# lmcinnes/enstop

Hardware: AMD Instinct MI355X
Metric: EM iterations/sec (higher is better)
Workload: dtype f32; 1 GPU; 1M x 100k, 100M nnz; corpus=independent Zipf tokens (SURVEY 8d), nnz=100435863, k=64, schedule=fused, parallelism=single fit

## Files before the change

enstop_amd/_lib.py:

```python
import ctypes as C
import os

import numpy as np

_HERE = os.path.dirname(os.path.abspath(__file__))
LIB_PATH = os.environ.get("ENSTOP_AMD_LIB", os.path.join(_HERE, "libplsa_hip.so"))

PLSA_FUSED = 1
PLSA_TRACE_LL = 4
PLSA_SW_LL_ONLY = 8
PLSA_STOP_NO_ZERO_ARM = 16
PLSA_SHARDED = 64
PLSA_GRAPH = 128
PLSA_REFERENCE_SUMS = 256
PLSA_REFERENCE_LL = 512

_i32p = np.ctypeslib.ndpointer(np.int32, flags="C_CONTIGUOUS")
_i64p = np.ctypeslib.ndpointer(np.int64, flags="C_CONTIGUOUS")
_f32p = np.ctypeslib.ndpointer(np.float32, flags="C_CONTIGUOUS")
_f64p = np.ctypeslib.ndpointer(np.float64, flags="C_CONTIGUOUS")
_ctx = C.c_void_p
_i64 = C.c_int64
_i32 = C.c_int32
_vp = C.c_void_p

SIGNATURES = {
    "plsa_device_count": (C.c_int, [C.POINTER(C.c_int)]),
    "plsa_hw_queues": (C.c_int, []),
    "plsa_create": (C.c_int, [C.c_int, C.POINTER(_ctx)]),
    "plsa_destroy": (None, [_ctx]),
    "plsa_last_error": (C.c_char_p, [_ctx]),
    "plsa_synchronize": (C.c_int, [_ctx]),
    "plsa_device_info": (C.c_int, [_ctx, C.c_char_p, C.c_char_p, C.POINTER(C.c_int), C.POINTER(_i64)]),
    "plsa_upload_csr": (C.c_int, [_ctx, _i32p, _i32p, _f32p, _i64, _i64, _i64]),
    "plsa_bootstrap": (C.c_int, [_ctx, _vp, _i64]),
    "plsa_active_shape": (C.c_int, [_ctx, C.POINTER(_i64), C.POINTER(_i64), C.POINTER(_i64)]),
    "plsa_download_active_csr": (C.c_int, [_ctx, _i32p, _i32p, _f32p]),
    "plsa_set_factors": (C.c_int, [_ctx, _vp, _vp, _i64, _i64, _i32]),
    "plsa_get_factors": (C.c_int, [_ctx, _vp, _vp]),
    "plsa_init_factors_device": (C.c_int, [_ctx, _i32, C.c_uint64]),
    "plsa_init_factors_mt19937": (C.c_int, [_ctx, _i32, np.ctypeslib.ndpointer(np.uint32, flags="C_CONTIGUOUS")]),
    "plsa_mt_marginals": (C.c_int, [_ctx, np.ctypeslib.ndpointer(np.float64, flags="C_CONTIGUOUS"), _i32]),
    "plsa_refit_init_mt19937": (C.c_int, [_ctx, C.c_void_p, _i64, _i32,
                                          np.ctypeslib.ndpointer(np.uint32, flags="C_CONTIGUOUS")]),
    "plsa_copy_components_to_device": (C.c_int, [_ctx, _vp]),
    "plsa_set_arithmetic": (C.c_int, [_ctx, _i32]),
    "plsa_e_step": (C.c_int, [_ctx, C.c_float, _vp]),
    "plsa_set_p": (C.c_int, [_ctx, _f32p]),
    "plsa_m_step": (C.c_int, [_ctx, _vp, _i32, _vp, _vp]),
    "plsa_log_likelihood": (C.c_int, [_ctx, _vp, C.POINTER(C.c_double)]),
    "plsa_fit": (C.c_int, [_ctx, _vp, _i32, _i32, C.c_double, C.c_float, _i32, C.POINTER(_i32), _vp,
                           C.POINTER(_i32)]),
    "plsa_refit": (C.c_int, [_ctx, _vp, _i32, _i32, C.c_double, C.c_float, _i32, C.POINTER(_i32), _vp,
                             C.POINTER(_i32)]),
    "plsa_em_accumulate": (C.c_int, [_ctx, _vp, C.c_float, _vp]),
    "plsa_em_accumulate_materialised": (C.c_int, [_ctx, _vp, C.c_float, _vp]),
    "plsa_p_reserve": (C.c_int, [_ctx, C.c_int64, C.POINTER(C.c_void_p)]),
    "plsa_p_borrow": (C.c_int, [_ctx, C.c_void_p, C.c_int64]),
    "plsa_em_finish": (C.c_int, [_ctx]),
    "plsa_set_sample_weight": (C.c_int, [_ctx, _vp]),
    "plsa_comm_last_error": (C.c_int, [_ctx, C.c_char_p, _i64]),
    "plsa_accumulator_device": (C.c_int, [_ctx, C.POINTER(C.c_void_p), C.POINTER(_i64)]),
    "plsa_accumulator_get": (C.c_int, [_ctx, _f32p]),
    "plsa_accumulator_set": (C.c_int, [_ctx, _f32p]),
    "plsa_comm_unique_id": (C.c_int, [C.c_void_p]),
    "plsa_comm_init": (C.c_int, [_ctx, C.c_char_p, _i32, _i32]),
    "plsa_comm_destroy": (C.c_int, [_ctx]),
    "plsa_comm_info": (C.c_int, [_ctx, C.POINTER(_i32), C.POINTER(_i32)]),
    "plsa_comm_barrier": (C.c_int, [_ctx]),
    "plsa_stack_reserve": (C.c_int, [_ctx, C.c_int64, C.c_int64, C.c_int32, C.POINTER(C.c_void_p)]),
    "plsa_comm_allgather_stack": (C.c_int, [_ctx, C.c_int64, C.c_int64, C.c_int32, C.POINTER(C.POINTER(C.c_float))]),
    "plsa_comm_allgather_stack_to": (C.c_int, [_ctx, _i64, _i64, _i32, _f32p]),
    "plsa_comm_allgather_host": (C.c_int, [_ctx, _vp, _i64, _vp]),
    "plsa_comm_allreduce_f64": (C.c_int, [_ctx, _f64p, _i64, _i32]),
    "plsa_comm_broadcast_host": (C.c_int, [_ctx, _vp, _i64, _i32]),
    "plsa_allreduce_accumulator": (C.c_int, [_ctx]),
    "plsa_reference_chain_info": (C.c_int, [_ctx, C.POINTER(_i64), C.POINTER(_i64), C.POINTER(_i32)]),
    "plsa_placement_info": (C.c_int, [_ctx, C.POINTER(_i32), C.POINTER(C.c_double), C.POINTER(C.c_double)]),
    "plsa_schedule_info": (C.c_int, [_ctx, C.POINTER(_i32), C.POINTER(C.c_double), C.POINTER(_i32), C.POINTER(_i32),
                                     C.POINTER(C.c_int64)]),
    "plsa_packed_info": (C.c_int, [_ctx, C.POINTER(_i32), C.POINTER(_i32)]),
    "plsa_pass_info": (C.c_int, [_ctx, _i32p, _i32p, _i32p]),
    "plsa_fit_info": (C.c_int, [_ctx, _i32p]),
    "plsa_release_scratch": (C.c_int, [_ctx]),
    "plsa_timing_enable": (C.c_int, [_ctx, _i32]),
    "plsa_timing_reset": (C.c_int, [_ctx]),
    "plsa_timing_get": (C.c_int, [_ctx, C.c_char_p, C.POINTER(C.c_double), C.POINTER(_i64)]),
    "plsa_timing_report": (C.c_int, [_ctx, C.c_char_p, _i64]),
    "plsa_measure_stream_bandwidth": (C.c_int, [_ctx, _i64, _i32, _i32, C.POINTER(C.c_double)]),
    "plsa_all_pairs_hellinger": (C.c_int, [_ctx, C.c_void_p, _i64, _i64, _f64p]),
    "plsa_all_pairs_kl": (C.c_int, [_ctx, C.c_void_p, _i64, _i64, _f64p]),
    "plsa_cluster_representatives": (C.c_int, [_ctx, C.c_void_p, _i64, _i64, _i32p, _vp, _i32, _f32p]),
    "plsa_host_normalize_rows": (None, [_f64p, _i64, _i64]),
    "plsa_host_mt19937_jump": (C.c_int, [C.POINTER(C.c_uint32), _i32]),
    "plsa_generate_synthetic": (C.c_int, [_ctx, _i64, _i64, _i64, C.c_double, C.c_uint64,
                                          C.POINTER(_i64)]),
    "plsa_generate_synthetic_topics": (C.c_int, [_ctx, _i64, _i64, _i64, C.c_double, C.c_uint64, _i32, C.c_double,
                                                 C.c_double, C.POINTER(_i64)]),
    "plsa_synthetic_dominant_topics": (C.c_int, [_ctx, _i32p]),
}

_members = C.c_void_p
MEMBERS_MAX = 64
MEMBER_SIGNATURES = {
    "plsa_members_create": (C.c_int, [_ctx, _i32, C.POINTER(_members)]),
    "plsa_members_destroy": (None, [_members]),
    "plsa_members_capacity": (C.c_int, [_ctx, _i32, C.POINTER(_i32)]),
    "plsa_members_prepare": (C.c_int, [_members, _i32, _vp, _i64, _i32, _vp, _vp, _vp]),
    "plsa_members_fit": (C.c_int, [_members, _i32, _i32, _i32, C.c_double, C.c_float, _i32, _i32p, _vp, _i32, _i32p,
                                   C.POINTER(_i32)]),
    "plsa_members_copy_components": (C.c_int, [_members, _i32, C.c_void_p]),
    "plsa_members_context": (C.c_int, [_members, _i32, C.POINTER(_ctx)]),
    "plsa_members_info": (C.c_int, [_members, _i32, _i32p]),
    "plsa_members_last_ll": (C.c_int, [_members, _i32, C.POINTER(C.c_double)]),
    "plsa_members_release": (C.c_int, [_members]),
}

METRIC_SIGNATURES = {
    "plsa_codocument_counts": (C.c_int, [_ctx, _i32p, _i64, _i32, _i32, _i64p, _i64p]),
}

_lib = None
HW_QUEUES = {"set_by": None, "hip_mapped_before_load": None}


def _default_hw_queues():
    want = os.environ.get("ENSTOP_AMD_HW_QUEUES", "8").strip()
    if "GPU_MAX_HW_QUEUES" in os.environ:
        HW_QUEUES["set_by"] = "user"
        return
    try:
        n_queues = int(want)
    except ValueError:
        raise ValueError("ENSTOP_AMD_HW_QUEUES=%r: expected a positive integer (hardware queues to ask the HIP runtime for) "
                         "or 0 to leave the runtime's default" % (want,)) from None
    if n_queues <= 0:
        HW_QUEUES["set_by"] = "opt-out"
        return
    try:
        with open("/proc/self/maps") as f:
            HW_QUEUES["hip_mapped_before_load"] = "libamdhip64" in f.read()
    except OSError:
        pass
    os.environ["GPU_MAX_HW_QUEUES"] = str(n_queues)
    HW_QUEUES["set_by"] = "enstop_amd"


def hw_queues():
    return dict(HW_QUEUES, value=int(load().plsa_hw_queues()))


def load():
    global _lib
    if _lib is not None:
        return _lib
    if not os.path.exists(LIB_PATH):
        raise ImportError(
            "enstop_amd: %s not found -- build the HIP extension first "
            "(python -m enstop_amd.build). There is no CPU fallback." % LIB_PATH)
    _default_hw_queues()
    lib = C.CDLL(LIB_PATH, mode=C.RTLD_GLOBAL)
    for name, (res, args) in list(SIGNATURES.items()) + list(MEMBER_SIGNATURES.items()) + list(METRIC_SIGNATURES.items()):
        fn = getattr(lib, name)
        fn.restype = res
        fn.argtypes = args
    _lib = lib
    return lib


def ptr(a):
    return None if a is None else a.ctypes.data
```

enstop_amd/csrc/plsa_hip.hip:

```cpp
#include <hip/hip_runtime.h>
#include <hipcub/hipcub.hpp>
#include <rccl/rccl.h>

#include <algorithm>
#include <cmath>
#include <cstdarg>
#include <cstdio>
#include <cstdlib>
#include <cstring>
#include <memory>
#include <mutex>
#include <string>
#include <thread>
#include <type_traits>
#include <vector>

#include "../../include/plsa_hip.h"
#include "../../include/plsa_hip_diag.h"
#include "../../include/plsa_hip_members.h"
#include "../../include/plsa_hip_metrics.h"
#include "mt_jump.hpp"
#include "plsa_kernels.hpp"
#include "plsa_member_kernels.hpp"
#include "plsa_metric_kernels.hpp"
#include "plsa_ref_kernels.hpp"
#include "plsa_synth.hpp"

using plsa::i64;

namespace {

thread_local std::string g_err;


struct DevBuf {
    void *p = nullptr;
    size_t cap = 0;
    bool borrowed = false;
    DevBuf() = default;
    DevBuf(DevBuf &&o) noexcept { swap(o); }
    DevBuf &operator=(DevBuf &&o) noexcept { DevBuf(std::move(o)).swap(*this); return *this; }
    void swap(DevBuf &o) noexcept { std::swap(p, o.p); std::swap(cap, o.cap); std::swap(borrowed, o.borrowed); }
    ~DevBuf() { if (p && !borrowed) (void)hipFree(p); }
    void release() { if (!borrowed) *this = DevBuf(); }
    void borrow(void *q, size_t bytes) { *this = DevBuf(); p = q; cap = q ? bytes : 0; borrowed = q != nullptr; }
    template <class T> T *as() const { return reinterpret_cast<T *>(p); }
};

template <class H, hipError_t (*Destroy)(H)>
struct Handle {
    H h = nullptr;
    Handle() = default;
    Handle(Handle &&o) noexcept { std::swap(h, o.h); }
    Handle &operator=(Handle &&o) noexcept { Handle(std::move(o)).swap(*this); return *this; }
    void swap(Handle &o) noexcept { std::swap(h, o.h); }
    ~Handle() { if (h) (void)Destroy(h); }
    operator H() const { return h; }
};
using Stream = Handle<hipStream_t, hipStreamDestroy>;
using Event = Handle<hipEvent_t, hipEventDestroy>;

struct HostFree { void operator()(void *p) const { (void)hipHostFree(p); } };
template <class T> using Pinned = std::unique_ptr<T[], HostFree>;
template <class T> hipError_t host_alloc(Pinned<T> &h, size_t count) {
    h.reset();
    void *q = nullptr;
    const hipError_t e = hipHostMalloc(&q, sizeof(T) * count, hipHostMallocDefault);
    h.reset(static_cast<T *>(q));
    return e;
}

template <class T> struct Derived {
    bool valid = false;
    void invalidate() { valid = false; }
    void drop() { static_cast<T &>(*this) = T{}; }
};

struct Timed {
    int name_id;
    Event a, b;
};

}

struct plsa_ctx {
    int device = 0;
    Stream stream;
    Stream stream2;
    hipStream_t ls = nullptr;
    Event ev_fork, ev_join;
    Event ev_row, ev_tail;
    bool overlap = true;
    double overlap_full_limit = 2e9;
    std::string err;
    hipDeviceProp_t prop;
    int grid_cap = 2048;

    i64 bn = 0, bm = 0, bnnz = 0;
    DevBuf b_indptr, b_col, b_val;
    bool active_is_base = true;
    i64 n = 0, m = 0, nnz = 0;
    DevBuf a_indptr, a_col, a_val;
    const int *indptr = nullptr, *col = nullptr;
    const float *val = nullptr;
    struct RowIndex : Derived<RowIndex> { DevBuf ids; } rowidx;

    struct Csc : Derived<Csc> {
        DevBuf colptr, row, val, pos, item_first, item_col, item_start, item_end, item_order, heavy_cols;
        DevBuf item_rec;
        DevBuf xcd_lo;
        bool balanced = false;
        int seg = 256, n_heavy = 0;
        i64 n_items = 0;
    } csc;
    int seg_override = 0, struct_lpn = 0;
    int struct_row_lpn = 0;
    DevBuf partial;
    bool use_item_order = true, xcd_split = true;
    bool packed = true;
    struct PackedStream : Derived<PackedStream> { DevBuf buf; bool ok = false; } pk_csr, pk_csc;
    DevBuf pk_count;
    int chunks_per_lane = 2;
    int row_lpn = 1, row_ch = 1;
    bool row_shape_8x2 = true;
    bool p_lent = false;
    int e_rows = -1;
    int mt_streams = 256;
    i64 mt_min_blocks = 4096;
    int heavy_items = 32;

    bool force_wide = false;
    struct RowItems : Derived<RowItems> {
        DevBuf first, row, start;
        bool use = false;
        int seg = 64;
        i64 n = 0;
    } ritems;
    int rseg_override = 0, ritems_mode = -1;
    DevBuf rpartial;

    struct EItems : Derived<EItems> { DevBuf row, start; int seg = 0; i64 n = 0; } eitems;
    int eseg_override = -1;

    bool sort_rows = true;
    struct RowOrder : Derived<RowOrder> {
        DevBuf ids;
        int range = 0;
    } roworder;
    i64 syn_n = 0; int syn_k0 = 0; double syn_alpha = 0.0; uint64_t syn_seed = 0;
    bool row_xcd = false;

    int k = 0, kp = 0, lpn = 1, ch = 1;
    DevBuf U[3], Vt[3], Vacc;
    bool rot3 = false;
    int speculate = -1;
    Event ev_ll;
    int cu = 0, cv = 0;
    i64 fac_n = 0, fac_m = 0;
    DevBuf P;
    struct PState : Derived<PState> {} p_state;
    bool ref_sums = false, ref_ll = false;
    DevBuf ref_terms;
    int ref_chain_mode = 0;
    bool ref_pairs_off = false;
    DevBuf ref_csum, ref_pairs, ref_exps, ref_pairs2, ref_exps2, ref_stats, ref_ll_neg;
    struct RefTileSums : Derived<RefTileSums> {
        DevBuf sums;
        const float *sw = nullptr;
        int tj = 0;
    } ref_tsum;
    const float *ref_e_sw = nullptr;
    bool ref_e_no_sums = false;
    struct RefHeavy : Derived<RefHeavy> { DevBuf cols; int n = 0, min = 0; } ref_heavy;
    Pinned<unsigned long long> h_ref_stats;
    Event ev_ref_stats;
    bool ref_stats_pending = false;
    unsigned long long ref_slow_total = 0, ref_chunks_total = 0;
    int placement_candidates = 4, placement_tried = 0;
    double placement_gbps[2] = {0.0, 0.0};
    size_t p_shift = 0;

    DevBuf sw, ll_partials, ll_out, colsum_partials, norm_pwz, norm_pdz, tmp0, tmp1, tmp2, cubtmp;
    DevBuf mt_seq;
    bool mt_chain = false;
    DevBuf mt_words, mt_state, mt_fin, mt_poly;
    Pinned<double> h_ll;

    DevBuf colsum_rows, colsum_rows2;
    DevBuf metric_mask, metric_small;
    DevBuf t_end;
    bool pipeline = true;
    bool graph = false;
    int order_band = -1;
    int balance = -1;
    bool bal_have_frac = false;
    double bal_frac[9] = {0, 0, 0, 0, 0, 0, 0, 0, 0};
    int bal_lo[9] = {0, 0, 0, 0, 0, 0, 0, 0, 0};
    i64 bal_chunks = -1;
    int bal_launches = 0;
    double bal_end_us[8] = {0, 0, 0, 0, 0, 0, 0, 0};
    int small_grid = 0;
    int colsum_rows_used = 0;
    struct FitInfo {
        int fused = 0, pipelined = 0, speculated = 0, graph_launches = 0;
        int tail = 0;
        int two_stage = 0;
        int xcd_split = 0;
    } fit_info;

    ncclComm_t comm = nullptr;
    int comm_rank = 0, comm_world = 1;
    bool sharded = false;
    bool sw_resident = false;
    i64 sw_n = 0;
    DevBuf sw_res;
    DevBuf comm_send, comm_recv, comm_small, comm_stack;
    Pinned<float> comm_host;
    size_t comm_host_cap = 0;

    bool timing = false;
    std::vector<std::string> names;
    std::vector<Timed> timed;
    std::vector<Event> pool;
    std::vector<double> acc_ms;
    std::vector<i64> acc_n;
};

namespace {

inline float *p_base(plsa_ctx *c) { return reinterpret_cast<float *>(reinterpret_cast<char *>(c->P.p) + c->p_shift); }

int fail(plsa_ctx *c, const char *fmt, ...) {
    char buf[512];
    va_list ap;
    va_start(ap, fmt);
    vsnprintf(buf, sizeof buf, fmt, ap);
    va_end(ap);
    if (c) c->err = buf; else g_err = buf;
    return 1;
}

#define HIPCHK(c, expr)                                                                            \
    do {                                                                                           \
        hipError_t e_ = (expr);                                                                    \
        if (e_ != hipSuccess)                                                                      \
            return fail((c), "%s failed: %s (%s:%d)", #expr, hipGetErrorString(e_), __FILE__,      \
                        __LINE__);                                                                 \
    } while (0)

#define CHK(expr)                                                                                  \
    do {                                                                                           \
        int r_ = (expr);                                                                           \
        if (r_) return r_;                                                                         \
    } while (0)

#define NCCLCHK(c, expr)                                                                           \
    do {                                                                                           \
        ncclResult_t n_ = (expr);                                                                  \
        if (n_ != ncclSuccess)                                                                     \
            return fail((c), "%s failed: %s (%s:%d)", #expr, ncclGetErrorString(n_), __FILE__,     \
                        __LINE__);                                                                 \
    } while (0)

int grid_for(plsa_ctx *c, i64 work_items, int items_per_block);
bool g_contig = false;

int ensure(plsa_ctx *c, DevBuf &b, size_t bytes) {
// ... 248 lines not shown
    if (c->row_lpn == 8 && c->row_ch == 2 && c->kp == 64) {
        if (wide) fn(plsa::Shape<8, 2, false, true>{}); else fn(plsa::Shape<8, 2, true>{});
        return 0;
    }
    return dispatch_shape_gather(c, wide, fn);
}

int launch_check(plsa_ctx *c, const char *what) {
    hipError_t e = hipGetLastError();
    if (e != hipSuccess) return fail(c, "launch of %s failed: %s", what, hipGetErrorString(e));
    return 0;
}

inline int out_u(const plsa_ctx *c) { return c->rot3 ? (c->cu + 1) % 3 : 1 - c->cu; }
inline int out_v(const plsa_ctx *c) { return c->rot3 ? (c->cv + 1) % 3 : 1 - c->cv; }

int grid_for(plsa_ctx *c, i64 work_items, int items_per_block) {
    i64 need = (work_items + items_per_block - 1) / items_per_block;
    if (need < 1) need = 1;
    return (int)std::min<i64>(need, c->grid_cap);
}

void set_active_pointers(plsa_ctx *c) {
    if (c->active_is_base) {
        c->indptr = c->b_indptr.as<int>(); c->col = c->b_col.as<int>(); c->val = c->b_val.as<float>();
        c->n = c->bn; c->m = c->bm; c->nnz = c->bnnz;
    } else {
        c->indptr = c->a_indptr.as<int>(); c->col = c->a_col.as<int>(); c->val = c->a_val.as<float>();
    }
    c->rowidx.invalidate(); c->csc.invalidate(); c->pk_csr.invalidate(); c->pk_csc.invalidate(); c->roworder.invalidate();
    c->ritems.invalidate(); c->eitems.invalidate(); c->p_state.invalidate(); c->ref_heavy.invalidate(); c->ref_tsum.invalidate();
    c->ref_pairs_off = false;
}

int ensure_rowidx(plsa_ctx *c) {
    if (c->rowidx.valid) return 0;
    CHK(ensure(c, c->rowidx.ids, sizeof(int) * (size_t)c->nnz));
    if (c->n > 0) {
        Scope s(c, "k_expand_rows");
        hipLaunchKernelGGL(plsa::k_expand_rows, dim3(grid_for(c, c->n, 4)), dim3(256), 0, c->stream,
                           c->indptr, (int)c->n, c->rowidx.ids.as<int>());
    }
    CHK(launch_check(c, "k_expand_rows"));
    c->rowidx.valid = true;
    return 0;
}

int row_xcd_range(const plsa_ctx *c) {
    const i64 gpb = 256 / std::max(1, c->row_lpn);
    if (!c->row_xcd || c->n < 64 * gpb) return 0;
    return (int)(((c->n + gpb - 1) / gpb + 7) / 8 * gpb);
}

int ensure_roworder(plsa_ctx *c, const int **out) {
    *out = nullptr;
    if (!c->sort_rows) return 0;
    const int range = row_xcd_range(c);
    if (!c->roworder.valid || c->roworder.range != range) {
        c->roworder.range = range;
        const i64 n = c->n;
        CHK(ensure(c, c->roworder.ids, sizeof(int) * (size_t)n));
        CHK(ensure(c, c->tmp0, sizeof(int) * (size_t)n * 2));
        CHK(ensure(c, c->tmp1, sizeof(int) * (size_t)n));
        int *len = c->tmp0.as<int>(), *len_sorted = c->tmp0.as<int>() + n, *ids = c->tmp1.as<int>();
        hipLaunchKernelGGL(plsa::k_row_lengths, dim3((unsigned)((n + 255) / 256)), dim3(256), 0, c->stream,
                           c->indptr, (int)n, len, ids, range);
        CHK(launch_check(c, "k_row_lengths"));
        size_t bytes = 0;
        HIPCHK(c, hipcub::DeviceRadixSort::SortPairsDescending(nullptr, bytes, len, len_sorted, ids,
                                                               c->roworder.ids.as<int>(), (int)n, 0, 32, c->stream));
        CHK(ensure(c, c->cubtmp, bytes));
        HIPCHK(c, hipcub::DeviceRadixSort::SortPairsDescending(c->cubtmp.p, bytes, len, len_sorted, ids,
                                                               c->roworder.ids.as<int>(), (int)n, 0, 32, c->stream));
        c->roworder.valid = true;
    }
    *out = c->roworder.ids.as<int>();
    return 0;
}

int exclusive_sum_int(plsa_ctx *c, const int *in, int *out, i64 count);

int ensure_ritems(plsa_ctx *c) {
    if (c->ritems.valid) return 0;
    const i64 n = c->n;
    const i64 group_slots = (i64)c->prop.multiProcessorCount * 32 * (64 / std::max(1, c->row_lpn));
    const double avg = (double)c->nnz / (double)std::max<i64>(n, 1);
    const int rseg_decide = c->rseg_override ? c->rseg_override : 64;
    c->ritems.use = c->ritems_mode == 1 || (c->ritems_mode < 0 && n < 2 * group_slots && avg > 2.0 * rseg_decide);
    if (c->rseg_override) c->ritems.seg = c->rseg_override;
    else {
        const i64 per_slot = c->nnz / std::max<i64>(group_slots, 1);
        int r = 16;
        while (r * 2 <= per_slot && r < 64) r *= 2;
        c->ritems.seg = r;
    }
    c->ritems.n = 0;
    if (c->ritems.use) {
        CHK(ensure(c, c->ritems.first, sizeof(int) * (size_t)(n + 1)));
        CHK(ensure(c, c->tmp0, sizeof(int) * (size_t)(n + 1)));
        HIPCHK(c, hipMemsetAsync(c->tmp0.p, 0, sizeof(int) * (size_t)(n + 1), c->stream));
        hipLaunchKernelGGL(plsa::k_item_counts, dim3((unsigned)((n + 255) / 256)), dim3(256), 0, c->stream,
                           c->indptr, (int)n, c->ritems.seg, c->tmp0.as<int>());
        CHK(exclusive_sum_int(c, c->tmp0.as<int>(), c->ritems.first.as<int>(), n + 1));
        int cnt = 0;
        HIPCHK(c, hipMemcpyAsync(&cnt, c->ritems.first.as<int>() + n, sizeof(int), hipMemcpyDeviceToHost, c->stream));
        HIPCHK(c, hipStreamSynchronize(c->stream));
        c->ritems.n = cnt;
        CHK(ensure(c, c->ritems.row, sizeof(int) * (size_t)std::max(cnt, 1)));
        CHK(ensure(c, c->ritems.start, sizeof(int) * (size_t)std::max(cnt, 1)));
        hipLaunchKernelGGL(plsa::k_ritem_fill, dim3((unsigned)((n + 255) / 256)), dim3(256), 0, c->stream,
                           c->indptr, c->ritems.first.as<int>(), (int)n, c->ritems.seg, c->ritems.row.as<int>(),
                           c->ritems.start.as<int>());
        CHK(launch_check(c, "k_ritem_fill"));
    }
    c->ritems.valid = true;
    return 0;
}

int ensure_eitems(plsa_ctx *c, int eseg) {
    if (c->eitems.valid && c->eitems.seg == eseg) return 0;
    const i64 n = c->n;
    c->eitems.seg = eseg;
    c->eitems.n = 0;
    if (eseg > 0) {
        CHK(ensure(c, c->tmp0, sizeof(int) * (size_t)(n + 1)));
        CHK(ensure(c, c->tmp1, sizeof(int) * (size_t)(n + 1)));
        HIPCHK(c, hipMemsetAsync(c->tmp0.p, 0, sizeof(int) * (size_t)(n + 1), c->stream));
        hipLaunchKernelGGL(plsa::k_item_counts, dim3((unsigned)((n + 255) / 256)), dim3(256), 0, c->stream,
                           c->indptr, (int)n, eseg, c->tmp0.as<int>());
        CHK(exclusive_sum_int(c, c->tmp0.as<int>(), c->tmp1.as<int>(), n + 1));
        int cnt = 0;
        HIPCHK(c, hipMemcpyAsync(&cnt, c->tmp1.as<int>() + n, sizeof(int), hipMemcpyDeviceToHost, c->stream));
        HIPCHK(c, hipStreamSynchronize(c->stream));
        c->eitems.n = cnt;
        CHK(ensure(c, c->eitems.row, sizeof(int) * (size_t)std::max(cnt, 1)));
        CHK(ensure(c, c->eitems.start, sizeof(int) * (size_t)std::max(cnt, 1)));
        hipLaunchKernelGGL(plsa::k_ritem_fill, dim3((unsigned)((n + 255) / 256)), dim3(256), 0, c->stream,
                           c->indptr, c->tmp1.as<int>(), (int)n, eseg, c->eitems.row.as<int>(), c->eitems.start.as<int>());
        CHK(launch_check(c, "k_ritem_fill"));
        HIPCHK(c, hipStreamSynchronize(c->stream));
    }
    c->eitems.valid = true;
    return 0;
}

int exclusive_sum_int(plsa_ctx *c, const int *in, int *out, i64 count) {
    size_t bytes = 0;
    HIPCHK(c, hipcub::DeviceScan::ExclusiveSum(nullptr, bytes, in, out, (int)count, c->stream));
    CHK(ensure(c, c->cubtmp, bytes));
    HIPCHK(c, hipcub::DeviceScan::ExclusiveSum(c->cubtmp.p, bytes, in, out, (int)count, c->stream));
    return 0;
}

int ensure_csc(plsa_ctx *c) {
    if (c->csc.valid) return 0;
    CHK(ensure_rowidx(c));
    {
        const i64 slots = (i64)c->prop.multiProcessorCount * 32 * (64 / std::max(1, c->lpn));
        i64 want = c->nnz / std::max<i64>(slots + slots / 4, 1);
        int seg = 16;
        const int cap = 64;
        while (seg * 2 <= want && seg < cap) seg *= 2;
        c->csc.seg = c->seg_override ? c->seg_override : seg;
    }
    const i64 nnz = c->nnz, m = c->m;
    CHK(ensure(c, c->csc.colptr, sizeof(int) * (size_t)(m + 1)));
    CHK(ensure(c, c->csc.row, sizeof(int) * (size_t)nnz));
    CHK(ensure(c, c->csc.val, sizeof(float) * (size_t)nnz));
    CHK(ensure(c, c->csc.pos, sizeof(int) * (size_t)nnz));
    CHK(ensure(c, c->tmp0, sizeof(int) * (size_t)std::max<i64>(nnz, m + 1)));
    CHK(ensure(c, c->tmp1, sizeof(int) * (size_t)nnz));
    const bool pack = c->packed && nnz > 0 && c->n <= plsa::PACK_MAX_IDS;
    c->pk_csc.invalidate();
    c->pk_csc.ok = false;
    if (pack) {
        CHK(ensure(c, c->pk_csc.buf, sizeof(unsigned) * (size_t)nnz));
        CHK(ensure(c, c->pk_count, sizeof(unsigned long long)));
        HIPCHK(c, hipMemsetAsync(c->pk_count.p, 0, sizeof(unsigned long long), c->stream));
    }
    if (nnz > 0) {
        hipLaunchKernelGGL(plsa::k_iota, dim3(grid_for(c, nnz, 256)), dim3(256), 0, c->stream,
                           c->tmp1.as<int>(), nnz);
        int bits = 1;
        while (((i64)1 << bits) < m) ++bits;
        size_t bytes = 0;
        HIPCHK(c, hipcub::DeviceRadixSort::SortPairs(nullptr, bytes, c->col, c->tmp0.as<int>(),
                                                     c->tmp1.as<int>(), c->csc.pos.as<int>(), nnz, 0,
                                                     bits, c->stream));
        CHK(ensure(c, c->cubtmp, bytes));
        HIPCHK(c, hipcub::DeviceRadixSort::SortPairs(c->cubtmp.p, bytes, c->col, c->tmp0.as<int>(),
                                                     c->tmp1.as<int>(), c->csc.pos.as<int>(), nnz, 0,
                                                     bits, c->stream));
        hipLaunchKernelGGL(plsa::k_colptr_from_sorted, dim3((unsigned)((m + 256) / 256)), dim3(256), 0, c->stream,
                           c->tmp0.as<int>(), nnz, (int)m, c->csc.colptr.as<int>());
        hipLaunchKernelGGL(plsa::k_csc_gather, dim3(grid_for(c, nnz, 256)), dim3(256), 0, c->stream,
                           c->csc.pos.as<int>(), c->rowidx.ids.as<int>(), c->val, nnz,
                           c->csc.row.as<int>(), c->csc.val.as<float>(), pack ? c->pk_csc.buf.as<unsigned>() : nullptr,
                           pack ? c->pk_count.as<unsigned long long>() : nullptr);
        CHK(launch_check(c, "k_csc_gather"));
    } else {
        HIPCHK(c, hipMemsetAsync(c->csc.colptr.p, 0, sizeof(int) * (size_t)(m + 1), c->stream));
    }
    CHK(ensure(c, c->csc.item_first, sizeof(int) * (size_t)(m + 1)));
    HIPCHK(c, hipMemsetAsync(c->tmp0.p, 0, sizeof(int) * (size_t)(m + 1), c->stream));
    hipLaunchKernelGGL(plsa::k_col_item_counts, dim3((unsigned)((m + 255) / 256)), dim3(256), 0, c->stream,
                       c->csc.colptr.as<int>(), (int)m, c->csc.seg, c->tmp0.as<int>());
    CHK(exclusive_sum_int(c, c->tmp0.as<int>(), c->csc.item_first.as<int>(), m + 1));
    int n_items = 0;
    HIPCHK(c, hipMemcpyAsync(&n_items, c->csc.item_first.as<int>() + m, sizeof(int), hipMemcpyDeviceToHost,
                             c->stream));
    HIPCHK(c, hipStreamSynchronize(c->stream));
    c->csc.n_items = n_items;
    const size_t ni = (size_t)std::max<i64>(n_items, 1);
    CHK(ensure(c, c->csc.item_col, sizeof(int) * ni));
    CHK(ensure(c, c->csc.item_start, sizeof(int) * ni));
    CHK(ensure(c, c->csc.item_end, sizeof(int) * ni));
    CHK(ensure(c, c->csc.item_order, sizeof(int) * ni));
    CHK(ensure(c, c->tmp2, sizeof(unsigned long long) * ni * 2));
    CHK(ensure(c, c->tmp1, sizeof(int) * ni));
    unsigned long long *d_key = c->tmp2.as<unsigned long long>();
    const int band_bytes = (c->kp >= 64 ? 2048 : 512) << 10;
    const int band = c->order_band >= 0 ? c->order_band : std::max(64, band_bytes / (c->kp > 0 ? c->kp * 4 : 256));
    int len_bits = 1;
    while (((i64)1 << len_bits) <= c->n) ++len_bits;
    int key_bits = len_bits;
    if (band > 0) { i64 n_bands = c->n / band + 1; int bb = 1; while (((i64)1 << bb) < n_bands) ++bb; key_bits = len_bits + bb; }
    if (n_items > 0)
        hipLaunchKernelGGL(plsa::k_item_fill, dim3((unsigned)((n_items + 255) / 256)), dim3(256), 0, c->stream,
                           c->csc.colptr.as<int>(), c->csc.item_first.as<int>(), (int)m, c->csc.seg, c->csc.row.as<int>(),
                           c->csc.item_col.as<int>(), c->csc.item_start.as<int>(), c->csc.item_end.as<int>(), band, len_bits, d_key,
                           c->tmp1.as<int>(), n_items);
    CHK(launch_check(c, "k_item_fill"));
    if (n_items > 0) {
        size_t bytes = 0;
        HIPCHK(c, hipcub::DeviceRadixSort::SortPairs(nullptr, bytes, d_key, d_key + ni,
                                                     c->tmp1.as<int>(), c->csc.item_order.as<int>(), n_items, 0, key_bits, c->stream));
        CHK(ensure(c, c->cubtmp, bytes));
        HIPCHK(c, hipcub::DeviceRadixSort::SortPairs(c->cubtmp.p, bytes, d_key, d_key + ni,
                                                     c->tmp1.as<int>(), c->csc.item_order.as<int>(), n_items, 0, key_bits, c->stream));
    }
    CHK(ensure(c, c->csc.item_rec, sizeof(int4) * ni));
    if (n_items > 0) {
        hipLaunchKernelGGL(plsa::k_item_records, dim3((unsigned)((n_items + 255) / 256)), dim3(256), 0, c->stream,
                           c->use_item_order ? c->csc.item_order.as<int>() : nullptr, c->csc.item_col.as<int>(),
                           c->csc.item_start.as<int>(), c->csc.item_end.as<int>(), (i64)n_items, c->csc.item_rec.as<int4>());
        CHK(launch_check(c, "k_item_records"));
    }
    c->csc.balanced = false;
    CHK(ensure(c, c->csc.heavy_cols, sizeof(int) * (size_t)(m + 1)));
    HIPCHK(c, hipMemsetAsync(c->csc.heavy_cols.as<int>() + m, 0, sizeof(int), c->stream));
    hipLaunchKernelGGL(plsa::k_heavy_list, dim3((unsigned)((m + 255) / 256)), dim3(256), 0, c->stream,
                       c->csc.item_first.as<int>(), (int)m, c->heavy_items, c->csc.heavy_cols.as<int>(),
                       c->csc.heavy_cols.as<int>() + m);
    CHK(launch_check(c, "k_heavy_list"));
    HIPCHK(c, hipMemcpyAsync(&c->csc.n_heavy, c->csc.heavy_cols.as<int>() + m, sizeof(int), hipMemcpyDeviceToHost, c->stream));
    unsigned long long escaped = 0;
    if (pack) HIPCHK(c, hipMemcpyAsync(&escaped, c->pk_count.p, sizeof escaped, hipMemcpyDeviceToHost, c->stream));
    HIPCHK(c, hipStreamSynchronize(c->stream));
    c->csc.valid = true;
    c->pk_csc.valid = c->packed;
    c->pk_csc.ok = pack && escaped * 16 <= (unsigned long long)nnz;
    if (!c->pk_csc.ok) c->pk_csc.buf.release();
    return 0;
}

int build_packed(plsa_ctx *c, DevBuf &out, const int *ids, const float *vals, i64 id_range, bool *ok) {
    *ok = false;
    const i64 nnz = c->nnz;
    if (nnz <= 0 || id_range > plsa::PACK_MAX_IDS) { out.release(); return 0; }
    CHK(ensure(c, out, sizeof(unsigned) * (size_t)nnz));
    CHK(ensure(c, c->pk_count, sizeof(unsigned long long)));
    HIPCHK(c, hipMemsetAsync(c->pk_count.p, 0, sizeof(unsigned long long), c->stream));
    hipLaunchKernelGGL(plsa::k_pack_entries, dim3(grid_for(c, nnz, 256)), dim3(256), 0, c->stream,
                       ids, vals, nnz, out.as<unsigned>(), c->pk_count.as<unsigned long long>());
    CHK(launch_check(c, "k_pack_entries"));
    unsigned long long escaped = 0;
    HIPCHK(c, hipMemcpyAsync(&escaped, c->pk_count.p, sizeof escaped, hipMemcpyDeviceToHost, c->stream));
    HIPCHK(c, hipStreamSynchronize(c->stream));
    *ok = escaped * 16 <= (unsigned long long)nnz;
    if (!*ok) out.release();
    return 0;
}

int ensure_packed_csr(plsa_ctx *c) {
    if (!c->packed || c->pk_csr.valid) return 0;
    CHK(build_packed(c, c->pk_csr.buf, c->col, c->val, c->m, &c->pk_csr.ok));
    c->pk_csr.valid = true;
    return 0;
}

int ensure_packed_csc(plsa_ctx *c) {
    CHK(ensure_csc(c));
    if (!c->packed || c->pk_csc.valid) return 0;
    CHK(build_packed(c, c->pk_csc.buf, c->csc.row.as<int>(), c->csc.val.as<float>(), c->n, &c->pk_csc.ok));
    c->pk_csc.valid = true;
    return 0;
}

int upload_sw(plsa_ctx *c, const float *sw, const float **d_sw) {
    *d_sw = nullptr;
    if (!sw) {
        if (c->sw_resident) {
            if (c->sw_n != c->n) return fail(c, "resident sample weights were set for %lld documents, the active matrix has %lld",
                                              (long long)c->sw_n, (long long)c->n);
            *d_sw = c->sw_res.as<float>();
        }
        return 0;
    }
    CHK(ensure(c, c->sw, sizeof(float) * (size_t)c->n));
    HIPCHK(c, hipMemcpyAsync(c->sw.p, sw, sizeof(float) * (size_t)c->n, hipMemcpyHostToDevice, c->stream));
    HIPCHK(c, hipStreamSynchronize(c->stream));
    *d_sw = c->sw.as<float>();
    return 0;
}

void set_shape(plsa_ctx *c, int k) {
    const int kp = (k + 3) / 4 * 4;
    c->k = k; c->kp = kp;
    const int prev_lpn = c->struct_lpn, prev_row_lpn = c->struct_row_lpn;
    int lpn = 1;
    while (lpn < kp / 4 && lpn < 64) lpn *= 2;
    if (lpn >= 32 && lpn * 4 >= kp && c->chunks_per_lane == 2) lpn /= 2;
    c->lpn = lpn;
    c->ch = (kp / 4 + lpn - 1) / lpn;
    if (c->ch == 3) c->ch = 4;
    c->row_lpn = c->lpn; c->row_ch = c->ch;
    if (c->row_shape_8x2 && c->lpn == 16 && c->ch == 1 && kp == 64) { c->row_lpn = 8; c->row_ch = 2; }
    if (c->row_lpn != prev_row_lpn) {
        c->ritems.invalidate();
        c->struct_row_lpn = c->row_lpn;
    }
    if (lpn != prev_lpn) {
        c->eitems.invalidate();
        if (!c->seg_override) c->csc.invalidate();
        c->struct_lpn = lpn;
    }
}

int need_factors(plsa_ctx *c) {
    if (c->k <= 0 || !c->U[0].p || !c->Vt[0].p) return fail(c, "factors not set (call plsa_set_factors)");
    if (c->n <= 0) return fail(c, "no corpus uploaded");
    if (c->fac_n != c->n || c->fac_m != c->m)
        return fail(c, "factors were set for a %lld x %lld matrix but the active matrix is %lld x %lld "
                       "(call plsa_set_factors after plsa_upload_csr / plsa_bootstrap)",
                    (long long)c->fac_n, (long long)c->fac_m, (long long)c->n, (long long)c->m);
    return 0;
}

int run_ref_e_step(plsa_ctx *c, float thresh);
int run_ref_norm_pwz(plsa_ctx *c, const float *d_sw);
int ensure_ref_heavy(plsa_ctx *c);
bool ref_pairs_now(const plsa_ctx *c);
int run_ref_m_step(plsa_ctx *c, const float *d_sw, bool update_v, float *d_norm_pdz);
int run_ref_loglik(plsa_ctx *c, const float *d_sw, double *out);

int run_e_step(plsa_ctx *c, float thresh) {
    c->ref_tsum.invalidate();
    {
        const size_t need = sizeof(float) * (size_t)(c->nnz + 64) * (size_t)c->kp;
        size_t free_b = 0, total_b = 0;
        if (!c->P.borrowed && c->P.cap < need && hipMemGetInfo(&free_b, &total_b) == hipSuccess && free_b + c->P.cap < need)
            return fail(c, c->ref_sums ? "the reference arithmetic (PLSA_REFERENCE_SUMS) stores P(z|w,d) like the reference does: %.1f GB needed, "
                                         "%.1f GB of HBM free -- at this size only the default arithmetic is available"
                                       : "materialising P(z|w,d) needs %.1f GB but only %.1f GB of HBM are free; use the fused "
                           "schedule (PLSA_FUSED), which never stores it, or tile the documents (plsa_em_accumulate_materialised)", need / 1e9, (free_b + c->P.cap) / 1e9);
    }
    if (c->P.borrowed || c->p_lent) {
        const size_t need = sizeof(float) * (size_t)(c->nnz + 64) * (size_t)c->kp;
        if (c->P.cap < need)
            return fail(c, c->P.borrowed ? "the borrowed P(z|w,d) buffer holds %.2f GB, this matrix needs %.2f GB (plsa_p_borrow)"
                                         : "the P(z|w,d) buffer lent out by plsa_p_reserve holds %.2f GB, this matrix needs %.2f GB: it cannot "
                                           "grow while other contexts hold its address (end the loans, then plsa_release_scratch)",
                        c->P.cap / 1e9, need / 1e9);
        c->p_shift = 0;
    } else
    {
        const char *s1 = getenv("PLSA_P_SLACK_MB"), *s2 = getenv("PLSA_P_OFFSET_KB");
        const size_t slack = s1 ? (size_t)atoll(s1) << 20 : 0;
        c->p_shift = s2 ? (size_t)atoll(s2) * 1024 : 0;
        CHK(ensure_best_placement(c, c->P, sizeof(float) * (size_t)(c->nnz + 64) * (size_t)c->kp + std::max(slack, c->p_shift),
                                  c->placement_candidates, c->placement_gbps, &c->placement_tried));
    }
    if (c->ref_sums) return run_ref_e_step(c, thresh);
    bool e_rows = c->e_rows < 0 ? (double)c->nnz * c->kp >= 1e8 : c->e_rows != 0;
    if (e_rows) {
        const int eseg = c->eseg_override >= 0 ? c->eseg_override : (c->lpn >= 16 ? 64 : (c->lpn == 8 ? 8 : 16));
        CHK(ensure_eitems(c, eseg));
        const bool items = eseg > 0 && c->eitems.n > 0;
        const int grid = grid_for(c, items ? c->eitems.n : c->n, 256 / c->lpn);
        const int *order = nullptr;
        if (!items) CHK(ensure_roworder(c, &order));
        CHK(dispatch_shape(c, [&](auto S) {
            Scope s(c, "k_e_step");
            auto go = [&](auto TN) {
                hipLaunchKernelGGL((plsa::k_e_step_rows<decltype(S), decltype(TN)::value>), dim3(grid), dim3(256), 0, c->stream,
                                   c->indptr, c->col, (int)c->n, order, c->U[c->cu].as<float>(), c->Vt[c->cv].as<float>(),
                                   p_base(c), c->kp, thresh, items ? c->eitems.row.as<int>() : nullptr,
                                   items ? c->eitems.start.as<int>() : nullptr, eseg, c->eitems.n);
            };
            if (thresh < plsa::TINY_THRESH) go(std::true_type{}); else go(std::false_type{});
        }));
    } else {
        CHK(ensure_rowidx(c));
        const i64 tiles = (c->nnz + 63) / 64;
        const int grid = grid_for(c, tiles, 4);
        CHK(dispatch_shape(c, [&](auto S) {
            Scope s(c, "k_e_step");
            auto go = [&](auto TN) {
                hipLaunchKernelGGL((plsa::k_e_step<decltype(S), decltype(TN)::value>), dim3(grid), dim3(256), 0, c->stream,
                                   c->rowidx.ids.as<int>(), c->col, c->nnz, c->U[c->cu].as<float>(),
                                   c->Vt[c->cv].as<float>(), p_base(c), c->kp, thresh);
            };
            if (thresh < plsa::TINY_THRESH) go(std::true_type{}); else go(std::false_type{});
        }));
    }
    CHK(launch_check(c, "k_e_step"));
    c->p_state.valid = true;
    return 0;
}

int run_row_pass(plsa_ctx *c, bool from_p, bool want_ll, const float *d_sw, float thresh,
                 float *d_norm_pdz, int *ll_blocks) {
    CHK(ensure_ritems(c));
    const bool items = c->ritems.use && c->ritems.n > 0;
    int grid = grid_for(c, items ? c->ritems.n : c->n, 256 / c->row_lpn);
    const int *order = nullptr;
    const int gpb_row = 256 / c->row_lpn;
    const bool xcd_rows = !items && !from_p && c->sort_rows && row_xcd_range(c) > 0;
    if (xcd_rows) grid = (int)(((c->n + gpb_row - 1) / gpb_row + 7) / 8 * 8);
    if (!items) CHK(ensure_roworder(c, &order));
    if (items) CHK(ensure(c, c->rpartial, sizeof(float) * (size_t)c->ritems.n * c->kp));
    const int *ri_row = items ? c->ritems.row.as<int>() : nullptr;
    const int *ri_start = items ? c->ritems.start.as<int>() : nullptr;
    float *rpart = items ? c->rpartial.as<float>() : nullptr;
    const int rseg = c->ritems.seg;
    const i64 n_ritems = c->ritems.n;
    if (want_ll) CHK(ensure(c, c->ll_partials, sizeof(double) * (size_t)grid));
    if (!from_p) CHK(ensure_packed_csr(c));
    const bool packed = !from_p && c->packed && c->pk_csr.ok;
    CHK(dispatch_shape_row(c, [&](auto S) {
        using Sh = decltype(S);
        const int *ip = c->indptr, *cl = packed ? c->pk_csr.buf.as<int>() : c->col;
        const float *vl = c->val, *U = c->U[c->cu].as<float>(), *Vt = c->Vt[c->cv].as<float>();
        const float *P = p_base(c);
        float *Un = c->U[out_u(c)].as<float>();
        double *llp = c->ll_partials.as<double>();
        const int n = (int)c->n, kp = c->kp;
        auto launch = [&](auto SS, auto FP, auto LL, auto TN, const char *name) {
            Scope s(c, name);
            hipLaunchKernelGGL((plsa::k_row_pass<decltype(SS), decltype(FP)::value, decltype(LL)::value, decltype(TN)::value>),
                               dim3(grid), dim3(256), 0, c->ls, ip, cl, vl, n, order, U, Vt, P, Un,
                               d_sw, d_norm_pdz, kp, thresh, llp, ri_row, ri_start, rseg, n_ritems, rpart, xcd_rows ? 1 : 0);
        };
        auto go = [&](auto FP, auto LL, auto TN, const char *name) {
            if constexpr (!decltype(FP)::value) {
                if (packed) { launch(plsa::Packed<Sh>{}, FP, LL, TN, name); return; }
            }
            launch(Sh{}, FP, LL, TN, name);
        };
        using T = std::true_type;
        using F = std::false_type;
        const bool tiny = thresh < plsa::TINY_THRESH;
        if (from_p) go(T{}, F{}, F{}, "k_row_pass<P>");
        else if (want_ll) { if (tiny) go(F{}, T{}, T{}, "k_row_pass<fused,LL>"); else go(F{}, T{}, F{}, "k_row_pass<fused,LL>"); }
        else { if (tiny) go(F{}, F{}, T{}, "k_row_pass<fused>"); else go(F{}, F{}, F{}, "k_row_pass<fused>"); }
        if (items) {
            Scope s(c, "k_row_reduce");
            hipLaunchKernelGGL((plsa::k_row_reduce<Sh>), dim3(grid_for(c, c->n, 256 / Sh::LPN)), dim3(256), 0, c->ls,
                               c->ritems.first.as<int>(), n, rpart, Un, d_norm_pdz, kp);
        }
    }));
    CHK(launch_check(c, "k_row_pass"));
    if (ll_blocks) *ll_blocks = grid;
    return 0;
}

void balance_set_lo(plsa_ctx *c, int n_chunks) {
    c->bal_lo[0] = 0;
    for (int x = 1; x < 8; ++x) {
        int v = (int)(c->bal_frac[x] * n_chunks + 0.5);
        c->bal_lo[x] = std::min(n_chunks, std::max(c->bal_lo[x - 1], v));
    }
    c->bal_lo[8] = n_chunks;
    c->bal_chunks = n_chunks;
}

int col_grid(plsa_ctx *c, int n_chunks, bool split) {
    i64 g = n_chunks;
    if (split) {
        int longest = 1;
        for (int x = 0; x < 8; ++x) longest = std::max(longest, c->bal_lo[x + 1] - c->bal_lo[x]);
        g = 8 * (i64)longest;
    }
    return (int)std::max<i64>(1, std::min<i64>(g, (i64)1 << 22));
}

template <class Launch>
int ensure_balance(plsa_ctx *c, int n_chunks, bool split, Launch &&launch) {
    if (c->csc.balanced && c->bal_chunks == n_chunks) return 0;
    CHK(ensure(c, c->csc.xcd_lo, sizeof(int) * 16));
    const bool warm = c->bal_have_frac;
    if (!warm) for (int x = 0; x <= 8; ++x) c->bal_frac[x] = x / 8.0;
    balance_set_lo(c, n_chunks);
    HIPCHK(c, hipMemcpyAsync(c->csc.xcd_lo.p, c->bal_lo, sizeof(int) * 9, hipMemcpyHostToDevice, c->ls));
    c->bal_launches = 0;
    const bool small_grid_active = c->small_grid > 0 && (double)c->nnz * c->kp < c->overlap_full_limit;
    const bool tune = split && n_chunks >= 64 && !small_grid_active &&
                      (c->balance > 0 || (c->balance < 0 && (double)c->nnz * c->kp >= 1e8));
    if (tune) {
        const size_t cap = (size_t)8 * (size_t)n_chunks + 16;
        CHK(ensure(c, c->t_end, sizeof(unsigned long long) * cap));
        std::vector<unsigned long long> te;
        const int max_launches = warm ? 1 : 8;
        if (!warm) CHK(launch(false));
        double best_spread = 1e300, best_frac[9];
        for (int x = 0; x <= 8; ++x) best_frac[x] = c->bal_frac[x];
        for (int it = 0; it < max_launches; ++it) {
            const int grid = col_grid(c, n_chunks, split);
            te.assign((size_t)grid + 1, 0);
            HIPCHK(c, hipMemsetAsync(c->t_end.p, 0, sizeof(unsigned long long) * ((size_t)grid + 1), c->ls));
            CHK(launch(true));
            HIPCHK(c, hipMemcpyAsync(te.data(), c->t_end.p, sizeof(unsigned long long) * ((size_t)grid + 1),
                                     hipMemcpyDeviceToHost, c->ls));
            HIPCHK(c, hipStreamSynchronize(c->ls));
            c->bal_launches++;
            unsigned long long t0 = ~0ull, last[8] = {0, 0, 0, 0, 0, 0, 0, 0};
            for (int b = 0; b <= grid; ++b) if (te[b]) t0 = std::min(t0, te[b]);
            for (int b = 0; b < grid; ++b) last[b & 7] = std::max(last[b & 7], te[b]);
            double T[8], mean = 0.0, lo_t = 1e300, hi_t = 0.0;
            for (int x = 0; x < 8; ++x) {
                T[x] = std::max(1.0, (double)(last[x] - t0) / 100.0);
                c->bal_end_us[x] = T[x];
                mean += T[x] / 8.0; lo_t = std::min(lo_t, T[x]); hi_t = std::max(hi_t, T[x]);
            }
            const double spread = (hi_t - lo_t) / mean;
            if (spread < best_spread) {
                best_spread = spread;
                for (int x = 0; x <= 8; ++x) best_frac[x] = c->bal_frac[x];
            }
            if (spread <= 0.02) break;
            if (it == max_launches - 1 && !warm) {
                for (int x = 0; x <= 8; ++x) c->bal_frac[x] = best_frac[x];
                balance_set_lo(c, n_chunks);
                HIPCHK(c, hipMemcpyAsync(c->csc.xcd_lo.p, c->bal_lo, sizeof(int) * 9, hipMemcpyHostToDevice, c->ls));
                break;
            }
            double size[8], tot = 0.0;
            for (int x = 0; x < 8; ++x) {
                size[x] = std::max(1e-6, (c->bal_frac[x + 1] - c->bal_frac[x]) * (1.0 + 0.8 * (mean / T[x] - 1.0)));
                tot += size[x];
            }
            double acc = 0.0;
            for (int x = 0; x < 8; ++x) { acc += size[x]; c->bal_frac[x + 1] = acc / tot; }
            c->bal_frac[8] = 1.0;
            balance_set_lo(c, n_chunks);
            HIPCHK(c, hipMemcpyAsync(c->csc.xcd_lo.p, c->bal_lo, sizeof(int) * 9, hipMemcpyHostToDevice, c->ls));
        }
        c->bal_have_frac = true;
    }
    c->csc.balanced = true;
    return 0;
}

int run_col_pass(plsa_ctx *c, bool from_p, const float *d_sw, float thresh, int parts = 3) {
    CHK(from_p ? ensure_csc(c) : ensure_packed_csc(c));
    const bool packed = !from_p && c->packed && c->pk_csc.ok;
    CHK(ensure(c, c->partial, sizeof(float) * (size_t)std::max<i64>(c->csc.n_items, 1) * c->kp));
    int rc = 0;
    CHK(dispatch_shape_gather(c, table_is_wide(c, c->n), [&](auto S) {
        using Sh = decltype(S);
        constexpr int LPN = Sh::LPN, GPB = 256 / LPN;
        const i64 n_visit = c->csc.n_items;
        const int n_chunks = (int)((n_visit + GPB - 1) / GPB);
        const int grid2 = grid_for(c, c->m, GPB);
        const bool u_fits_l2 = (double)c->n * c->kp * 4.0 <= 2.0 * 1024 * 1024;
        const int xcd_split = (c->xcd_split && n_chunks >= 64 && !u_fits_l2) ? 1 : 0;
        if (parts & 1) {
            c->fit_info.xcd_split = xcd_split;
            rc = ensure(c, c->colsum_rows, sizeof(double) * (size_t)std::max(n_chunks, 1) * c->kp);
            if (rc) return;
            const size_t smem = sizeof(double) * (size_t)GPB * c->kp;
            auto launch = [&](bool timed) -> int {
                int grid = col_grid(c, n_chunks, xcd_split != 0);
                if (c->small_grid > 0 && (double)c->nnz * c->kp < c->overlap_full_limit)
                    grid = std::min(grid, c->small_grid * c->prop.multiProcessorCount);
                Scope s(c, from_p ? "k_col_pass<P>" : "k_col_pass<fused>");
                const int4 *rec = c->csc.item_rec.as<int4>();
                const int *lo = c->csc.xcd_lo.as<int>(), *cp = c->csc.pos.as<int>();
                const int *cr = packed ? c->pk_csc.buf.as<int>() : c->csc.row.as<int>();
                const float *cvl = c->csc.val.as<float>(), *U = c->U[c->cu].as<float>(), *Vt = c->Vt[c->cv].as<float>();
                float *part = c->partial.as<float>();
                double *sums = c->colsum_rows.as<double>();
                unsigned long long *te = c->t_end.as<unsigned long long>();
                const int kp = c->kp;
                auto run = [&](auto SS, auto FP, auto TM, auto TN) {
                    hipLaunchKernelGGL((plsa::k_col_pass<decltype(SS), decltype(FP)::value, decltype(TM)::value, decltype(TN)::value>),
                                       dim3(grid), dim3(256), smem, c->ls, rec, n_visit, lo, cr, cvl, cp, U, Vt, p_base(c), d_sw,
                                       part, kp, thresh, xcd_split, sums, te);
                };
                auto go = [&](auto FP, auto TM, auto TN) {
                    if constexpr (!decltype(FP)::value) {
                        if (packed) { run(plsa::Packed<Sh>{}, FP, TM, TN); return; }
                    }
                    run(Sh{}, FP, TM, TN);
                };
                using T = std::true_type;
                using F = std::false_type;
                const bool tiny = !from_p && thresh < plsa::TINY_THRESH;
                if (from_p) { if (timed) go(T{}, T{}, F{}); else go(T{}, F{}, F{}); }
                else if (tiny) { if (timed) go(F{}, T{}, T{}); else go(F{}, F{}, T{}); }
                else { if (timed) go(F{}, T{}, F{}); else go(F{}, F{}, F{}); }
                return launch_check(c, "k_col_pass");
            };
            rc = ensure_balance(c, n_chunks, xcd_split != 0, launch);
            if (rc) return;
            rc = launch(false);
            if (rc) return;
            c->colsum_rows_used = n_chunks;
        }
        if (parts & 2) {
            Scope s(c, "k_col_reduce");
            hipLaunchKernelGGL((plsa::k_col_reduce<Sh>), dim3(grid2 + c->csc.n_heavy), dim3(256),
                               (256 / LPN) * c->kp * sizeof(float), c->ls,
                               c->csc.item_first.as<int>(), (int)c->m, c->heavy_items, c->csc.heavy_cols.as<int>(), c->csc.n_heavy,
                               c->partial.as<float>(), c->Vacc.as<float>(), c->kp);
        }
    }));
    if (rc) return rc;
    CHK(launch_check(c, "k_col_pass"));
    return 0;
}

int run_v_normalise(plsa_ctx *c) {
    if (c->sharded && c->comm) {
        Scope s(c, "rccl_allreduce_accumulator");
        NCCLCHK(c, ncclAllReduce(c->Vacc.p, c->Vacc.p, (size_t)c->m * c->kp, ncclFloat, ncclSum, c->comm, c->ls));
    }
    const int nb = (int)std::min<i64>(plsa::NORM_BLOCKS, std::max<i64>(1, c->m));
    CHK(ensure(c, c->colsum_partials, sizeof(double) * (size_t)nb * c->kp));
    {
        Scope s(c, "k_colsum_partial");
        hipLaunchKernelGGL(plsa::k_colsum_partial, dim3(nb), dim3(256), 256 * sizeof(double), c->ls,
                           c->Vacc.as<float>(), (int)c->m, c->kp, c->colsum_partials.as<double>());
    }
    CHK(ensure(c, c->norm_pwz, sizeof(float) * (size_t)c->kp));
    {
        Scope s(c, "k_colsum_final");
        hipLaunchKernelGGL(plsa::k_colsum_final, dim3(1), dim3(256), 0, c->ls,
                           c->colsum_partials.as<double>(), nb, c->kp, c->norm_pwz.as<float>());
    }
    {
        Scope s(c, "k_v_normalise");
        const i64 total4 = c->m * c->kp / 4;
        hipLaunchKernelGGL(plsa::k_v_normalise, dim3(grid_for(c, total4, 256)), dim3(256),
                           c->kp * sizeof(float), c->ls, c->Vacc.as<float>(),
                           c->Vt[out_v(c)].as<float>(), (int)c->m, c->kp, c->norm_pwz.as<float>());
    }
    CHK(launch_check(c, "k_v_normalise"));
    return 0;
}

int run_col_tail(plsa_ctx *c) {
    if (c->sharded) {
        c->fit_info.tail = 2;
        c->fit_info.two_stage = 0;
        CHK(run_col_pass(c, false, nullptr, 0.f, 2));
        return run_v_normalise(c);
    }
    c->fit_info.tail = 1;
    c->fit_info.two_stage = c->colsum_rows_used > 2048;
    const int rows = c->colsum_rows_used;
    if (rows <= 0) return fail(c, "internal: column tail without a column pass");
    CHK(ensure(c, c->norm_pwz, sizeof(float) * (size_t)c->kp));
    const double *rows_in = c->colsum_rows.as<double>();
    int n_rows = rows;
    if (rows > 2048) {
        const int nb = std::max(64, std::min(1024, rows / 64));
        CHK(ensure(c, c->colsum_rows2, sizeof(double) * (size_t)nb * c->kp));
        Scope s(c, "k_norm_reduce");
        hipLaunchKernelGGL(plsa::k_norm_reduce, dim3(nb), dim3(256), 0, c->ls, rows_in, rows, c->kp,
                           c->colsum_rows2.as<double>());
        rows_in = c->colsum_rows2.as<double>();
        n_rows = nb;
    }
    {
        Scope s(c, "k_colsum_final");
        hipLaunchKernelGGL(plsa::k_colsum_final, dim3(1), dim3(256), 0, c->ls, rows_in, n_rows, c->kp,
                           c->norm_pwz.as<float>());
    }
    CHK(dispatch_shape(c, [&](auto S) {
        using Sh = decltype(S);
        constexpr int GPB = 256 / Sh::LPN;
        const int grid2 = grid_for(c, c->m, GPB);
        Scope s(c, "k_col_reduce_norm");
        hipLaunchKernelGGL((plsa::k_col_reduce_norm<Sh>), dim3(grid2 + c->csc.n_heavy), dim3(256),
                           sizeof(float) * (size_t)(GPB + 1) * c->kp, c->ls, c->csc.item_first.as<int>(), (int)c->m,
                           c->heavy_items, c->csc.heavy_cols.as<int>(), c->csc.n_heavy, c->partial.as<float>(),
                           c->norm_pwz.as<float>(), c->Vt[out_v(c)].as<float>(), c->kp);
    }));
    return launch_check(c, "k_col_reduce_norm");
}

int finish_ll(plsa_ctx *c, int blocks, double *out) {
    CHK(ensure(c, c->ll_out, sizeof(double)));
    {
        Scope s(c, "k_ll_final");
        hipLaunchKernelGGL(plsa::k_ll_final, dim3(1), dim3(256), 0, c->stream,
                           c->ll_partials.as<double>(), blocks, c->ll_out.as<double>());
    }
    CHK(launch_check(c, "k_ll_final"));
    if (c->sharded && c->comm)
        NCCLCHK(c, ncclAllReduce(c->ll_out.p, c->ll_out.p, 1, ncclDouble, ncclSum, c->comm, c->stream));
    HIPCHK(c, hipMemcpyAsync(c->h_ll.get(), c->ll_out.p, sizeof(double), hipMemcpyDeviceToHost, c->stream));
    if (!out) return hipEventRecord(c->ev_ll, c->stream) == hipSuccess ? 0 : fail(c, "event record failed");
    HIPCHK(c, hipStreamSynchronize(c->stream));
    *out = c->h_ll[0];
    return 0;
}

int wait_ll(plsa_ctx *c, double *out) {
    HIPCHK(c, hipEventSynchronize(c->ev_ll));
    *out = c->h_ll[0];
    return 0;
}

int run_loglik(plsa_ctx *c, const float *d_sw, double *out) {
    if (c->ref_ll) return run_ref_loglik(c, d_sw, out);
    const int grid = grid_for(c, c->n, 256 / c->lpn);
    const int *order = nullptr;
    CHK(ensure_roworder(c, &order));
    CHK(ensure(c, c->ll_partials, sizeof(double) * (size_t)grid));
    CHK(dispatch_shape(c, [&](auto S) {
        Scope s(c, "k_loglik");
        hipLaunchKernelGGL((plsa::k_loglik<decltype(S)>), dim3(grid), dim3(256), 0, c->stream, c->indptr,
                           c->col, c->val, (int)c->n, order, c->U[c->cu].as<float>(),
                           c->Vt[c->cv].as<float>(), d_sw, c->kp, c->ll_partials.as<double>());
    }));
    CHK(launch_check(c, "k_loglik"));
    return finish_ll(c, grid, out);
}

int run_m_step_from_p(plsa_ctx *c, const float *d_sw, bool update_v, float *d_norm_pdz) {
    if (!c->p_state.valid) return fail(c, "plsa_m_step: no P(z|w,d) on the device (run plsa_e_step or plsa_set_p)");
    if (c->ref_sums) return run_ref_m_step(c, d_sw, update_v, d_norm_pdz);
    CHK(run_row_pass(c, true, false, nullptr, 0.f, d_norm_pdz, nullptr));
    if (update_v) {
        CHK(run_col_pass(c, true, d_sw, 0.f, 1));
        CHK(run_col_tail(c));
    }
    c->cu ^= 1;
    if (update_v) c->cv ^= 1;
    return 0;
}

template <class Fn>
int dispatch_ref_group(plsa_ctx *c, Fn &&fn) {
    using std::integral_constant;
    const int kp = c->kp;
    if (kp <= 8) fn(integral_constant<int, 8>{}, integral_constant<int, 1>{});
    else if (kp <= 16) fn(integral_constant<int, 16>{}, integral_constant<int, 1>{});
    else if (kp <= 32) fn(integral_constant<int, 32>{}, integral_constant<int, 1>{});
    else if (kp <= 64) fn(integral_constant<int, 64>{}, integral_constant<int, 1>{});
    else if (kp <= 128) fn(integral_constant<int, 64>{}, integral_constant<int, 2>{});
    else if (kp <= 256) fn(integral_constant<int, 64>{}, integral_constant<int, 4>{});
    else if (kp <= 512) fn(integral_constant<int, 64>{}, integral_constant<int, 8>{});
    else if (kp <= 1024) fn(integral_constant<int, 64>{}, integral_constant<int, 16>{});
    else return fail(c, "unsupported topic count k=%d (max 1024)", c->k);
    return 0;
}

int run_ref_e_step(plsa_ctx *c, float thresh) {
    CHK(ensure_rowidx(c));
    static const bool tiled = [] { const char *e = getenv("PLSA_REF_E_TILED"); return !e || atoi(e) != 0; }();
    if (tiled && c->nnz > 0) {
        Scope s(c, "k_ref_e_step");
        const int kp = c->kp;
        const char *fe = getenv("PLSA_REF_FUSE_SUMS");
        const bool fuse = (!fe || atoi(fe) != 0) && ref_pairs_now(c) && !c->ref_e_no_sums;
        int rc_alloc = 0;
        auto go = [&](auto NZ) {
            constexpr int nz = decltype(NZ)::value;
            const i64 tiles = (c->nnz + 64 / nz - 1) / (64 / nz);
            if (fuse && (rc_alloc = ensure(c, c->ref_tsum.sums, sizeof(float) * (size_t)tiles * kp)) == 0) {
                hipLaunchKernelGGL((plsa::ref::k_ref_e_step_tiled<nz, true>), dim3(grid_for(c, tiles, 2)), dim3(128),
                                   sizeof(float) * 2 * (64 / nz) * (size_t)(kp + 1), c->stream, c->rowidx.ids.as<int>(), c->col, c->nnz,
                                   c->U[c->cu].as<float>(), c->Vt[c->cv].as<float>(), p_base(c), kp, thresh, c->val, c->ref_e_sw,
                                   c->ref_tsum.sums.as<float>());
                c->ref_tsum.valid = true; c->ref_tsum.sw = c->ref_e_sw; c->ref_tsum.tj = 64 / nz;
            } else if (!rc_alloc) {
                hipLaunchKernelGGL((plsa::ref::k_ref_e_step_tiled<nz, false>), dim3(grid_for(c, tiles, 2)), dim3(128),
                                   sizeof(float) * 2 * (64 / nz) * (size_t)(kp + 1), c->stream, c->rowidx.ids.as<int>(), c->col, c->nnz,
                                   c->U[c->cu].as<float>(), c->Vt[c->cv].as<float>(), p_base(c), kp, thresh, nullptr, nullptr, nullptr);
            }
        };
        using std::integral_constant;
        if (kp <= 64) go(integral_constant<int, 1>{});
        else if (kp <= 128) go(integral_constant<int, 2>{});
        else if (kp <= 256) go(integral_constant<int, 4>{});
        else if (kp <= 512) go(integral_constant<int, 8>{});
        else go(integral_constant<int, 16>{});
        if (rc_alloc) return rc_alloc;
    } else {
        Scope s(c, "k_ref_e_step");
        hipLaunchKernelGGL(plsa::ref::k_ref_e_step, dim3(grid_for(c, c->nnz, 256)), dim3(256), 0, c->stream,
                           c->rowidx.ids.as<int>(), c->col, c->nnz, c->U[c->cu].as<float>(), c->Vt[c->cv].as<float>(),
                           p_base(c), c->kp, thresh);
    }
    CHK(launch_check(c, "k_ref_e_step"));
    c->p_state.valid = true;
    return 0;
}

int ensure_ref_heavy(plsa_ctx *c) {
    if (c->ref_heavy.valid) return 0;
    const char *e = getenv("PLSA_REF_HEAVY_MIN");
    c->ref_heavy.min = e ? atoi(e) : 2048;
    c->ref_heavy.n = 0;
    if (c->ref_heavy.min > 0 && c->nnz > 0) {
        CHK(ensure(c, c->ref_heavy.cols, sizeof(int) * (size_t)(c->m + 1)));
        HIPCHK(c, hipMemsetAsync(c->ref_heavy.cols.p, 0, sizeof(int), c->stream));
        hipLaunchKernelGGL(plsa::ref::k_ref_heavy_cols, dim3((unsigned)((c->m + 255) / 256)), dim3(256), 0, c->stream,
                           c->csc.colptr.as<int>(), (int)c->m, c->ref_heavy.min, c->ref_heavy.cols.as<int>() + 1, c->ref_heavy.cols.as<int>());
        CHK(launch_check(c, "k_ref_heavy_cols"));
        int n = 0;
        HIPCHK(c, hipMemcpyAsync(&n, c->ref_heavy.cols.p, sizeof(int), hipMemcpyDeviceToHost, c->stream));
        HIPCHK(c, hipStreamSynchronize(c->stream));
        c->ref_heavy.n = n;
    }
    c->ref_heavy.valid = true;
    return 0;
}

int run_ref_pair_chain(plsa_ctx *c, int kind, const float *P, int kp, const float *d_sw, float *out, unsigned long long *stats) {
    const int *ri = c->rowidx.ids.as<int>();
    const bool ll = kind == plsa::ref::PAIR_NEG_TERMS;
    bool two = true;
    if (const char *e = getenv("PLSA_REF_LEVELS")) two = atoi(e) != 1;
    int L = !two && c->nnz >= plsa::ref::PAIR_L_LARGE_FROM ? plsa::ref::PAIR_L_LARGE : plsa::ref::PAIR_L_SMALL;
    if (const char *e = getenv("PLSA_REF_CHUNK")) { const int v = atoi(e); if (v >= 64 && v <= 4096 && v % 64 == 0) L = v; }
    const i64 n_chunks = (c->nnz + L - 1) / L;
    const i64 n_groups = (n_chunks + plsa::ref::PAIR_R - 1) / plsa::ref::PAIR_R;
    if (two) {
        CHK(ensure(c, c->ref_pairs2, sizeof(uint4) * (size_t)n_groups * kp));
        CHK(ensure(c, c->ref_exps2, sizeof(unsigned) * (size_t)n_groups * kp));
    }
    const i64 n_super = (n_chunks + plsa::ref::PAIR_SC - 1) / plsa::ref::PAIR_SC, n_pad = n_super * plsa::ref::PAIR_SC;
    CHK(ensure(c, c->ref_csum, sizeof(double) * (size_t)n_pad * kp));
    CHK(ensure(c, c->ref_pairs, sizeof(uint4) * (size_t)n_chunks * kp));
    CHK(ensure(c, c->ref_exps, sizeof(unsigned) * (size_t)n_chunks * kp));
    const int grid = grid_for(c, n_super, 4);
// ... 100 lines not shown
    unsigned long long *stats = c->ref_stats.as<unsigned long long>();
    HIPCHK(c, hipMemsetAsync(stats, 0, 16, c->ls));
    CHK(run_ref_pair_chain(c, d_sw ? plsa::ref::PAIR_WEIGHTED : plsa::ref::PAIR_PLAIN, p_base(c), kp, d_sw, out, stats));
    CHK(launch_check(c, "k_ref_pair_walk"));
    if (!c->ref_stats_pending) {
        HIPCHK(c, hipMemcpyAsync(c->h_ref_stats.get(), stats, 16, hipMemcpyDeviceToHost, c->ls));
        HIPCHK(c, hipEventRecord(c->ev_ref_stats, c->ls));
        c->ref_stats_pending = true;
    }
    return 0;
}

int run_ref_m_step(plsa_ctx *c, const float *d_sw, bool update_v, float *d_norm_pdz) {
    if (c->sharded) return fail(c, "the reference arithmetic has no doc-sharded form (norm_pwz is ONE chain over all non-zeros)");
    const int *order = nullptr;
    CHK(ensure_roworder(c, &order));
    int heavy_min = INT32_MAX;
    if (update_v) {
        CHK(ensure_csc(c));
        CHK(ensure_rowidx(c));
        CHK(ensure_ref_heavy(c));
        if (c->ref_heavy.n > 0) heavy_min = c->ref_heavy.min;
        CHK(ensure(c, c->norm_pwz, sizeof(float) * (size_t)c->kp));
        HIPCHK(c, hipEventRecord(c->ev_fork, c->stream));
        HIPCHK(c, hipStreamWaitEvent(c->stream2, c->ev_fork, 0));
        {
            LaunchOn on2(c, c->stream2);
            CHK(run_ref_norm_pwz(c, d_sw));
        }
        CHK(launch_check(c, "k_ref_norm_chain"));
        HIPCHK(c, hipEventRecord(c->ev_join, c->stream2));
    }
    const char *row_tiled_env = getenv("PLSA_REF_ROW_TILED");
    const bool row_tiled = row_tiled_env ? atoi(row_tiled_env) != 0 : c->n >= 300000;
    CHK(dispatch_ref_group(c, [&](auto G, auto NZ) {
        constexpr int g = decltype(G)::value, nz = decltype(NZ)::value;
        if (row_tiled) {
            Scope s(c, "k_ref_row_pass");
            constexpr int tj = 64 / nz;
            hipLaunchKernelGGL((plsa::ref::k_ref_row_pass_tiled<nz>), dim3(grid_for(c, (c->n + tj - 1) / tj, 2)), dim3(128),
                               sizeof(float) * 2 * tj * (size_t)(c->kp + 1), c->stream, c->indptr, c->val, (int)c->n, order,
                               p_base(c), c->U[out_u(c)].as<float>(), d_norm_pdz, c->kp);
        } else {
            Scope s(c, "k_ref_row_pass");
            hipLaunchKernelGGL((plsa::ref::k_ref_row_pass<g, nz>), dim3(grid_for(c, c->n, 256 / g)), dim3(256),
                               sizeof(float) * (size_t)(256 / g) * c->kp, c->stream, c->indptr, c->val, (int)c->n, order,
                               p_base(c), c->U[out_u(c)].as<float>(), d_norm_pdz, c->kp);
        }
        if (update_v) {
            Scope s(c, "k_ref_col_pass");
            hipLaunchKernelGGL((plsa::ref::k_ref_col_pass<g, nz>), dim3(grid_for(c, c->m, 256 / g)), dim3(256), 0, c->stream,
                               c->csc.colptr.as<int>(), c->csc.row.as<int>(), c->csc.val.as<float>(), c->csc.pos.as<int>(),
                               (int)c->m, p_base(c), d_sw, c->Vacc.as<float>(), c->kp, heavy_min);
        }
    }));
    if (update_v && c->ref_heavy.n > 0) {
        Scope s(c, "k_ref_col_heavy");
        const int kp = c->kp;
        auto go = [&](auto NZ) {
            constexpr int nz = decltype(NZ)::value;
            if (d_sw)
                hipLaunchKernelGGL((plsa::ref::k_ref_norm_chain<nz, true, true>), dim3(c->ref_heavy.n), dim3(plsa::ref::CHAIN_THREADS), 0,
                                   c->stream, c->csc.row.as<int>(), c->csc.val.as<float>(), (i64)0, p_base(c), d_sw, kp, c->Vacc.as<float>(),
                                   c->csc.pos.as<int>(), c->ref_heavy.cols.as<int>() + 1, c->csc.colptr.as<int>());
            else
                hipLaunchKernelGGL((plsa::ref::k_ref_norm_chain<nz, false, true>), dim3(c->ref_heavy.n), dim3(plsa::ref::CHAIN_THREADS), 0,
                                   c->stream, c->csc.row.as<int>(), c->csc.val.as<float>(), (i64)0, p_base(c), d_sw, kp, c->Vacc.as<float>(),
                                   c->csc.pos.as<int>(), c->ref_heavy.cols.as<int>() + 1, c->csc.colptr.as<int>());
        };
        using std::integral_constant;
        if (kp <= 64) go(integral_constant<int, 1>{});
        else if (kp <= 128) go(integral_constant<int, 2>{});
        else if (kp <= 256) go(integral_constant<int, 4>{});
        else if (kp <= 512) go(integral_constant<int, 8>{});
        else go(integral_constant<int, 16>{});
    }
    CHK(launch_check(c, "k_ref_row_pass / k_ref_col_pass"));
    if (update_v) {
        HIPCHK(c, hipStreamWaitEvent(c->stream, c->ev_join, 0));
        Scope s(c, "k_v_normalise");
        const i64 total4 = c->m * c->kp / 4;
        hipLaunchKernelGGL(plsa::k_v_normalise, dim3(grid_for(c, total4, 256)), dim3(256), c->kp * sizeof(float), c->stream,
                           c->Vacc.as<float>(), c->Vt[out_v(c)].as<float>(), (int)c->m, c->kp, c->norm_pwz.as<float>());
        CHK(launch_check(c, "k_v_normalise"));
    }
    c->cu ^= 1;
    if (update_v) c->cv ^= 1;
    return 0;
}

int run_ref_loglik(plsa_ctx *c, const float *d_sw, double *out) {
    if (c->sharded) return fail(c, "the reference arithmetic has no doc-sharded form");
    CHK(ensure_rowidx(c));
    CHK(ensure(c, c->ref_terms, sizeof(float) * (size_t)std::max<i64>(c->nnz, 1)));
    CHK(ensure(c, c->ll_out, sizeof(double)));
    {
        Scope s(c, "k_ref_ll_terms");
        hipLaunchKernelGGL(plsa::ref::k_ref_ll_terms, dim3(grid_for(c, c->nnz, 256)), dim3(256), 0, c->stream,
                           c->rowidx.ids.as<int>(), c->col, c->val, c->nnz, c->U[c->cu].as<float>(), c->Vt[c->cv].as<float>(),
                           d_sw, c->kp, c->ref_terms.as<float>());
    }
    if (ref_pairs_now(c)) {
        CHK(ensure(c, c->ref_stats, 32));
        CHK(ensure(c, c->ref_ll_neg, sizeof(float)));
        unsigned long long *stats = c->ref_stats.as<unsigned long long>();
        CHK(run_ref_pair_chain(c, plsa::ref::PAIR_NEG_TERMS, c->ref_terms.as<float>(), 1, nullptr, c->ref_ll_neg.as<float>(), stats + 2));
        hipLaunchKernelGGL(plsa::ref::k_ref_ll_from_walk, dim3(1), dim3(1), 0, c->stream, c->ref_ll_neg.as<float>(), c->ll_out.as<double>());
    } else {
        Scope s(c, "k_ref_ll_chain");
        hipLaunchKernelGGL(plsa::ref::k_ref_ll_chain, dim3(1), dim3(64), 0, c->stream, c->ref_terms.as<float>(), c->nnz,
                           c->ll_out.as<double>());
    }
    CHK(launch_check(c, "k_ref_ll_chain"));
    HIPCHK(c, hipMemcpyAsync(c->h_ll.get(), c->ll_out.p, sizeof(double), hipMemcpyDeviceToHost, c->stream));
    HIPCHK(c, hipStreamSynchronize(c->stream));
    *out = c->h_ll[0];
    return 0;
}

struct ArithmeticScope {
    plsa_ctx *c;
    bool sums, ll;
    ArithmeticScope(plsa_ctx *c_, int flags) : c(c_), sums(c_->ref_sums), ll(c_->ref_ll) {
        if (flags & PLSA_REFERENCE_SUMS) c->ref_sums = true;
        if (flags & PLSA_REFERENCE_LL) c->ref_ll = true;
    }
    ~ArithmeticScope() { c->ref_sums = sums; c->ref_ll = ll; }
};

bool stop_test(float cur, float &prev, double tol, bool zero_arm = true) {
    const float change = fabsf(cur - prev);
    if ((zero_arm && change == 0.0f) || (double)(change / fabsf(cur)) < tol) return true;
    prev = cur;
    return false;
}

void read_knobs(plsa_ctx *c) {
    if (const char *s = getenv("PLSA_OVERLAP")) c->overlap = atoi(s) != 0;
    if (const char *s = getenv("PLSA_OVERLAP_FULL_LIMIT")) c->overlap_full_limit = atof(s);
    if (const char *s = getenv("PLSA_ROW_ITEMS")) c->ritems_mode = atoi(s);
    if (const char *s = getenv("PLSA_PACKED")) c->packed = atoi(s) != 0;
    if (const char *s = getenv("PLSA_ROW_SEG")) c->rseg_override = std::max(1, atoi(s));
    int mult = 128;
    if (const char *s = getenv("PLSA_GRID_MULT")) mult = std::max(1, atoi(s));
    c->grid_cap = c->prop.multiProcessorCount * mult;
    if (const char *s = getenv("PLSA_CONTIG")) g_contig = atoi(s) != 0;
    if (const char *s = getenv("PLSA_PLACEMENT_CANDIDATES")) c->placement_candidates = std::max(1, atoi(s));
    if (const char *s = getenv("PLSA_COL_SEG")) c->seg_override = std::max(1, atoi(s));
    if (const char *s = getenv("PLSA_HEAVY_ITEMS")) c->heavy_items = std::max(1, atoi(s));
    if (const char *s = getenv("PLSA_SORT_ROWS")) c->sort_rows = atoi(s) != 0;
    if (const char *s = getenv("PLSA_ROW_XCD")) c->row_xcd = atoi(s) != 0;
    if (const char *s = getenv("PLSA_ITEM_ORDER")) c->use_item_order = atoi(s) != 0;
    if (const char *s = getenv("PLSA_XCD_SPLIT")) c->xcd_split = atoi(s) != 0;
    if (const char *s = getenv("PLSA_BALANCE")) c->balance = atoi(s);
    if (const char *s = getenv("PLSA_ORDER_BAND")) c->order_band = atoi(s);
    if (const char *s = getenv("PLSA_GRAPH")) c->graph = atoi(s) != 0;
    if (const char *s = getenv("PLSA_PIPELINE")) c->pipeline = atoi(s) != 0;
    if (const char *s = getenv("PLSA_CHUNKS_PER_LANE")) c->chunks_per_lane = atoi(s);
    if (const char *s = getenv("PLSA_E_ROWS")) c->e_rows = atoi(s);
    if (const char *s = getenv("PLSA_E_SEG")) c->eseg_override = atoi(s);
    if (const char *s = getenv("PLSA_MT_STREAMS")) c->mt_streams = std::max(1, std::min(4096, atoi(s)));
    if (const char *s = getenv("PLSA_MT_MIN_BLOCKS")) c->mt_min_blocks = std::max(1, atoi(s));
    if (const char *s = getenv("PLSA_SMALL_GRID")) c->small_grid = std::max(0, atoi(s));
    if (const char *s = getenv("PLSA_ROW_SHAPE")) c->row_shape_8x2 = atoi(s) != 0;
    if (const char *s = getenv("PLSA_FORCE_WIDE")) c->force_wide = atoi(s) != 0;
    if (const char *s = getenv("PLSA_MT_CHAIN")) c->mt_chain = atoi(s) != 0;
    if (const char *s = getenv("PLSA_SPECULATE")) c->speculate = atoi(s);
    if (const char *s = getenv("PLSA_REF_CHAIN"))
        c->ref_chain_mode = !strcmp(s, "pairs") ? 1 : (!strcmp(s, "serial") ? 2 : 0);
}

}

extern "C" {

int plsa_device_count(int *count) {
    hipError_t e = hipGetDeviceCount(count);
    if (e != hipSuccess) { *count = 0; return fail(nullptr, "hipGetDeviceCount: %s", hipGetErrorString(e)); }
    return 0;
}

const char *plsa_last_error(const plsa_ctx *ctx) { return ctx ? ctx->err.c_str() : g_err.c_str(); }

int plsa_create(int device, plsa_ctx **out) {
    *out = nullptr;
    int cnt = 0;
    hipError_t e = hipGetDeviceCount(&cnt);
    if (e != hipSuccess || cnt <= 0)
        return fail(nullptr, "no HIP device available (%s)", hipGetErrorString(e));
    if (device < 0 || device >= cnt) return fail(nullptr, "device %d out of range [0,%d)", device, cnt);
    std::unique_ptr<plsa_ctx> owner(new plsa_ctx());
    plsa_ctx *c = owner.get();
    c->device = device;
    if (hipSetDevice(device) != hipSuccess || hipGetDeviceProperties(&c->prop, device) != hipSuccess)
        return fail(nullptr, "hipSetDevice(%d) failed", device);
    if (strncmp(c->prop.gcnArchName, "gfx950", 6) != 0)
        return fail(nullptr, "libplsa_hip is built for gfx950 (MI355X) only; device %d is %s", device,
                    c->prop.gcnArchName);
    int prio_lo = 0, prio_hi = 0;
    (void)hipDeviceGetStreamPriorityRange(&prio_lo, &prio_hi);
    const char *prio_env = getenv("PLSA_TAIL_PRIORITY");
    const bool tail_prio = !prio_env || atoi(prio_env) != 0;
    if (hipStreamCreateWithFlags(&c->stream.h, hipStreamNonBlocking) != hipSuccess ||
        (tail_prio ? hipStreamCreateWithPriority(&c->stream2.h, hipStreamNonBlocking, prio_hi)
                   : hipStreamCreateWithFlags(&c->stream2.h, hipStreamNonBlocking)) != hipSuccess ||
        hipEventCreateWithFlags(&c->ev_fork.h, hipEventDisableTiming) != hipSuccess ||
        hipEventCreateWithFlags(&c->ev_join.h, hipEventDisableTiming) != hipSuccess ||
        hipEventCreateWithFlags(&c->ev_row.h, hipEventDisableTiming) != hipSuccess ||
        hipEventCreateWithFlags(&c->ev_tail.h, hipEventDisableTiming) != hipSuccess ||
        hipEventCreateWithFlags(&c->ev_ll.h, hipEventDisableTiming) != hipSuccess ||
        host_alloc(c->h_ll, 2) != hipSuccess)
        return fail(nullptr, "stream / pinned buffer creation failed");
    c->ls = c->stream;
    read_knobs(c);
    *out = owner.release();
    return 0;
}

void plsa_destroy(plsa_ctx *c) {
    if (!c) return;
    (void)hipSetDevice(c->device);
    (void)hipStreamSynchronize(c->stream);
    if (c->comm) (void)ncclCommDestroy(c->comm);
    delete c;
}

int plsa_synchronize(plsa_ctx *c) {
    HIPCHK(c, hipSetDevice(c->device));
    HIPCHK(c, hipStreamSynchronize(c->stream));
    return 0;
}

int plsa_hw_queues(void) {
    const char *s = getenv("GPU_MAX_HW_QUEUES");
    return s && atoi(s) > 0 ? atoi(s) : 4;
}

int plsa_device_info(plsa_ctx *c, char *name64, char *arch64, int *cus, int64_t *hbm_bytes) {
    if (name64) { strncpy(name64, c->prop.name, 63); name64[63] = 0; }
    if (arch64) { strncpy(arch64, c->prop.gcnArchName, 63); arch64[63] = 0; }
    if (cus) *cus = c->prop.multiProcessorCount;
    if (hbm_bytes) *hbm_bytes = (int64_t)c->prop.totalGlobalMem;
    return 0;
}

int plsa_upload_csr(plsa_ctx *c, const int32_t *indptr, const int32_t *indices, const float *data,
                    int64_t n, int64_t m, int64_t nnz) {
    HIPCHK(c, hipSetDevice(c->device));
    if (n <= 0 || m <= 0 || nnz < 0) return fail(c, "plsa_upload_csr: bad shape n=%lld m=%lld nnz=%lld",
                                                 (long long)n, (long long)m, (long long)nnz);
    if (n >= INT32_MAX || m >= INT32_MAX || nnz >= INT32_MAX)
        return fail(c, "plsa_upload_csr: n, m and nnz must each be < 2^31");
    if (indptr[0] != 0 || indptr[n] != nnz) return fail(c, "plsa_upload_csr: indptr[0] != 0 or indptr[n] != nnz");
    CHK(ensure(c, c->b_indptr, sizeof(int) * (size_t)(n + 1)));
    CHK(ensure(c, c->b_col, sizeof(int) * (size_t)nnz));
    CHK(ensure(c, c->b_val, sizeof(float) * (size_t)nnz));
    HIPCHK(c, hipMemcpyAsync(c->b_indptr.p, indptr, sizeof(int) * (size_t)(n + 1), hipMemcpyHostToDevice, c->stream));
    if (nnz) {
        CHK(copy_to_device(c, c->b_col.p, indices, sizeof(int) * (size_t)nnz));
        CHK(copy_to_device(c, c->b_val.p, data, sizeof(float) * (size_t)nnz));
    }
    CHK(ensure(c, c->tmp2, 16));
    int bad = 0;
    HIPCHK(c, hipMemsetAsync(c->tmp2.p, 0, sizeof(int), c->stream));
    hipLaunchKernelGGL(plsa::k_validate_csr, dim3(grid_for(c, std::max<i64>(n, nnz), 256)), dim3(256), 0, c->stream,
                       c->b_indptr.as<int>(), c->b_col.as<int>(), (i64)n, (i64)m, (i64)nnz, c->tmp2.as<int>());
    CHK(launch_check(c, "k_validate_csr"));
    HIPCHK(c, hipMemcpyAsync(&bad, c->tmp2.p, sizeof(int), hipMemcpyDeviceToHost, c->stream));
    HIPCHK(c, hipStreamSynchronize(c->stream));
    if (bad) {
        c->bn = c->bm = c->bnnz = 0;
        c->n = c->m = c->nnz = 0;
        c->active_is_base = true;
        return fail(c, "plsa_upload_csr: %s%s%s", (bad & 1) ? "indptr is not non-decreasing within [0, nnz]" : "",
                    bad == 3 ? "; " : "", (bad & 2) ? "column index outside [0, m)" : "");
    }
    c->bn = n; c->bm = m; c->bnnz = nnz;
    c->syn_n = 0;
    c->active_is_base = true;
    set_active_pointers(c);
    return 0;
}

int plsa_bootstrap(plsa_ctx *c, const int64_t *idx, int64_t n_out) {
    HIPCHK(c, hipSetDevice(c->device));
    if (c->bn <= 0) return fail(c, "plsa_bootstrap: no corpus uploaded");
    if (!idx) {
        c->active_is_base = true;
        set_active_pointers(c);
        return 0;
    }
    if (n_out <= 0 || n_out >= INT32_MAX) return fail(c, "plsa_bootstrap: bad n_out");
    CHK(ensure(c, c->tmp0, sizeof(i64) * (size_t)n_out));
    CHK(ensure(c, c->tmp1, sizeof(i64) * (size_t)(n_out + 1)));
    CHK(ensure(c, c->tmp2, sizeof(i64) * (size_t)(n_out + 1) + 16));
    i64 *d_idx = c->tmp0.as<i64>();
    int *d_len = c->tmp1.as<int>();
    i64 *d_ptr = c->tmp2.as<i64>();
    int *d_bad = reinterpret_cast<int *>(d_ptr + n_out + 1);
    HIPCHK(c, hipMemcpyAsync(d_idx, idx, sizeof(i64) * (size_t)n_out, hipMemcpyHostToDevice, c->stream));
    HIPCHK(c, hipMemsetAsync(d_bad, 0, sizeof(int), c->stream));
    HIPCHK(c, hipMemsetAsync(d_len, 0, sizeof(int) * (size_t)(n_out + 1), c->stream));
    hipLaunchKernelGGL(plsa::k_boot_lengths, dim3((unsigned)((n_out + 255) / 256)), dim3(256), 0, c->stream,
                       c->b_indptr.as<int>(), d_idx, (i64)n_out, c->bn, d_len, d_bad);
    CHK(launch_check(c, "k_boot_lengths"));
    {
// ... 756 lines not shown
    HIPCHK(c, hipSetDevice(c->device));
    if (c->comm) {
        HIPCHK(c, hipStreamSynchronize(c->stream));
        HIPCHK(c, hipStreamSynchronize(c->stream2));
        NCCLCHK(c, ncclCommDestroy(c->comm));
        c->comm = nullptr;
    }
    c->comm_rank = 0; c->comm_world = 1;
    return 0;
}

int plsa_comm_info(plsa_ctx *c, int32_t *rank, int32_t *world) {
    if (rank) *rank = c->comm_rank;
    if (world) *world = c->comm_world;
    return 0;
}

int plsa_comm_barrier(plsa_ctx *c) {
    HIPCHK(c, hipSetDevice(c->device));
    if (c->comm) {
        HIPCHK(c, hipMemsetAsync(c->comm_small.p, 0, sizeof(int), c->stream));
        NCCLCHK(c, ncclAllReduce(c->comm_small.p, c->comm_small.p, 1, ncclInt32, ncclSum, c->comm, c->stream));
    }
    HIPCHK(c, hipStreamSynchronize(c->stream));
    return 0;
}

int plsa_stack_reserve(plsa_ctx *c, int64_t slots, int64_t m, int32_t k, void **base_device) {
    HIPCHK(c, hipSetDevice(c->device));
    if (slots < 1 || m < 1 || k < 1 || !base_device) return fail(c, "plsa_stack_reserve: bad arguments");
    CHK(ensure(c, c->comm_stack, sizeof(float) * (size_t)slots * (size_t)k * (size_t)m));
    *base_device = c->comm_stack.p;
    return 0;
}

static int allgather_stack_impl(plsa_ctx *c, int64_t slots, int64_t m, int32_t k, float *dst, float **host_view) {
    HIPCHK(c, hipSetDevice(c->device));
    if (slots < 1 || m < 1 || k < 1 || (!dst && !host_view)) return fail(c, "plsa_comm_allgather_stack: bad arguments");
    const size_t km = (size_t)k * (size_t)m, world = (size_t)c->comm_world;
    if (c->comm_stack.cap < sizeof(float) * (size_t)slots * km)
        return fail(c, "plsa_comm_allgather_stack: no stack of %lld slots reserved (plsa_stack_reserve)", (long long)slots);
    const size_t bytes = sizeof(float) * (size_t)slots * km * world;
    if (!dst && c->comm_host_cap < bytes) {
        c->comm_host_cap = 0;
        HIPCHK(c, host_alloc(c->comm_host, bytes / sizeof(float)));
        c->comm_host_cap = bytes;
    }
    const float *src = c->comm_stack.as<float>();
    if (c->comm) {
        CHK(ensure(c, c->comm_recv, bytes));
        Scope s(c, "rccl_allgather_stack");
        NCCLCHK(c, ncclGroupStart());
        for (int64_t sl = 0; sl < slots; ++sl)
            NCCLCHK(c, ncclAllGather(c->comm_stack.as<float>() + (size_t)sl * km,
                                     c->comm_recv.as<float>() + (size_t)sl * world * km, km, ncclFloat, c->comm, c->stream));
        NCCLCHK(c, ncclGroupEnd());
        src = c->comm_recv.as<float>();
    }
    float *to = dst ? dst : c->comm_host.get();
    HIPCHK(c, hipMemcpyAsync(to, src, bytes, hipMemcpyDeviceToHost, c->stream));
    HIPCHK(c, hipStreamSynchronize(c->stream));
    if (host_view) *host_view = to;
    return 0;
}

int plsa_comm_allgather_stack(plsa_ctx *c, int64_t slots, int64_t m, int32_t k, float **host) {
    return allgather_stack_impl(c, slots, m, k, nullptr, host);
}

int plsa_comm_allgather_stack_to(plsa_ctx *c, int64_t slots, int64_t m, int32_t k, float *dst) {
    if (!dst) return fail(c, "plsa_comm_allgather_stack_to: dst is NULL");
    return allgather_stack_impl(c, slots, m, k, dst, nullptr);
}

int plsa_comm_allgather_host(plsa_ctx *c, const void *send, int64_t bytes, void *recv) {
    HIPCHK(c, hipSetDevice(c->device));
    if (!send || !recv || bytes <= 0) return fail(c, "plsa_comm_allgather_host: bad arguments");
    if (!c->comm) { memmove(recv, send, (size_t)bytes); return 0; }
    CHK(ensure(c, c->comm_send, (size_t)bytes));
    CHK(ensure(c, c->comm_recv, (size_t)bytes * (size_t)c->comm_world));
    HIPCHK(c, hipMemcpyAsync(c->comm_send.p, send, (size_t)bytes, hipMemcpyHostToDevice, c->stream));
    NCCLCHK(c, ncclAllGather(c->comm_send.p, c->comm_recv.p, (size_t)bytes, ncclUint8, c->comm, c->stream));
    HIPCHK(c, hipMemcpyAsync(recv, c->comm_recv.p, (size_t)bytes * (size_t)c->comm_world, hipMemcpyDeviceToHost, c->stream));
    HIPCHK(c, hipStreamSynchronize(c->stream));
    return 0;
}

int plsa_comm_allreduce_f64(plsa_ctx *c, double *inout, int64_t count, int32_t op) {
    HIPCHK(c, hipSetDevice(c->device));
    if (!inout || count <= 0 || (op != 0 && op != 1)) return fail(c, "plsa_comm_allreduce_f64: bad arguments");
    if (!c->comm) return 0;
    CHK(ensure(c, c->comm_send, sizeof(double) * (size_t)count));
    HIPCHK(c, hipMemcpyAsync(c->comm_send.p, inout, sizeof(double) * (size_t)count, hipMemcpyHostToDevice, c->stream));
    NCCLCHK(c, ncclAllReduce(c->comm_send.p, c->comm_send.p, (size_t)count, ncclDouble, op == 0 ? ncclSum : ncclMax,
                             c->comm, c->stream));
    HIPCHK(c, hipMemcpyAsync(inout, c->comm_send.p, sizeof(double) * (size_t)count, hipMemcpyDeviceToHost, c->stream));
    HIPCHK(c, hipStreamSynchronize(c->stream));
    return 0;
}

int plsa_comm_broadcast_host(plsa_ctx *c, void *buf, int64_t bytes, int32_t root) {
    HIPCHK(c, hipSetDevice(c->device));
    if (!buf || bytes <= 0 || root < 0 || root >= c->comm_world) return fail(c, "plsa_comm_broadcast_host: bad arguments");
    if (!c->comm) return 0;
    CHK(ensure(c, c->comm_send, (size_t)bytes));
    if (c->comm_rank == root)
        HIPCHK(c, hipMemcpyAsync(c->comm_send.p, buf, (size_t)bytes, hipMemcpyHostToDevice, c->stream));
    NCCLCHK(c, ncclBroadcast(c->comm_send.p, c->comm_send.p, (size_t)bytes, ncclUint8, root, c->comm, c->stream));
    HIPCHK(c, hipMemcpyAsync(buf, c->comm_send.p, (size_t)bytes, hipMemcpyDeviceToHost, c->stream));
    HIPCHK(c, hipStreamSynchronize(c->stream));
    return 0;
}

int plsa_allreduce_accumulator(plsa_ctx *c) {
    HIPCHK(c, hipSetDevice(c->device));
    CHK(need_factors(c));
    if (!c->comm) return 0;
    NCCLCHK(c, ncclAllReduce(c->Vacc.p, c->Vacc.p, (size_t)c->m * c->kp, ncclFloat, ncclSum, c->comm, c->stream));
    return 0;
}

int plsa_reference_chain_info(plsa_ctx *c, int64_t *slow_chunks, int64_t *chunks, int32_t *serial_now) {
    HIPCHK(c, hipSetDevice(c->device));
    HIPCHK(c, hipStreamSynchronize(c->stream));
    HIPCHK(c, hipStreamSynchronize(c->stream2));
    if (c->ref_stats_pending) {
        c->ref_stats_pending = false;
        c->ref_slow_total += c->h_ref_stats[0]; c->ref_chunks_total += c->h_ref_stats[1];
        if (c->ref_chain_mode == 0 && c->h_ref_stats[1] > 0 && c->h_ref_stats[0] * 4 > c->h_ref_stats[1]) c->ref_pairs_off = true;
    }
    if (slow_chunks) *slow_chunks = (int64_t)c->ref_slow_total;
    if (chunks) *chunks = (int64_t)c->ref_chunks_total;
    if (serial_now) *serial_now = (c->ref_chain_mode == 2 || (c->ref_chain_mode == 0 && c->ref_pairs_off)) ? 1 : 0;
    return 0;
}

int plsa_placement_info(plsa_ctx *c, int32_t *candidates, double *best_gbps, double *worst_gbps) {
    if (candidates) *candidates = c->placement_tried;
    if (best_gbps) *best_gbps = c->placement_gbps[0];
    if (worst_gbps) *worst_gbps = c->placement_gbps[1];
    return 0;
}

int plsa_schedule_info(plsa_ctx *c, int32_t *xcd_lo, double *xcd_end_us, int32_t *timed_launches, int32_t *item_len,
                       int64_t *n_items) {
    if (xcd_lo) for (int x = 0; x <= 8; ++x) xcd_lo[x] = c->csc.balanced ? c->bal_lo[x] : 0;
    if (xcd_end_us) for (int x = 0; x < 8; ++x) xcd_end_us[x] = c->bal_launches > 0 ? c->bal_end_us[x] : 0.0;
    if (timed_launches) *timed_launches = c->bal_launches;
    if (item_len) *item_len = c->csc.valid ? c->csc.seg : 0;
    if (n_items) *n_items = c->csc.valid ? c->csc.n_items : 0;
    return 0;
}

int plsa_packed_info(plsa_ctx *c, int32_t *csr, int32_t *csc) {
    if (csr) *csr = !c->packed ? 0 : (c->pk_csr.valid ? (c->pk_csr.ok ? 1 : 0) : -1);
    if (csc) *csc = !c->packed ? 0 : (c->csc.valid && c->pk_csc.valid ? (c->pk_csc.ok ? 1 : 0) : -1);
    return 0;
}

int plsa_pass_info(plsa_ctx *c, int32_t *col, int32_t *row, int32_t *wide) {
    if (c->k <= 0) return fail(c, "plsa_pass_info: factors not set (call plsa_set_factors)");
    if (col) { col[0] = c->lpn; col[1] = c->ch; col[2] = c->kp == 4 * c->lpn * c->ch; }
    if (row) { row[0] = c->row_lpn; row[1] = c->row_ch; row[2] = c->kp == 4 * c->row_lpn * c->row_ch; }
    if (wide) { wide[0] = table_is_wide(c, c->m); wide[1] = table_is_wide(c, c->n); }
    return 0;
}

int plsa_fit_info(plsa_ctx *c, int32_t *info) {
    if (!info) return fail(c, "plsa_fit_info: NULL argument");
    const plsa_ctx::FitInfo &f = c->fit_info;
    info[0] = f.fused; info[1] = f.pipelined; info[2] = f.speculated; info[3] = f.graph_launches;
    info[4] = f.tail; info[5] = f.two_stage; info[6] = f.xcd_split;
    return 0;
}

int plsa_release_scratch(plsa_ctx *c) {
    HIPCHK(c, hipSetDevice(c->device));
    HIPCHK(c, hipStreamSynchronize(c->stream));
    c->P.release();
    c->p_lent = false;
    c->p_state.drop();
    c->p_shift = 0;
    c->ref_heavy.drop(); c->ref_tsum.drop(); c->pk_csr.drop(); c->pk_csc.drop();
    for (DevBuf *b : {&c->ref_terms, &c->ref_csum, &c->ref_pairs, &c->ref_exps, &c->ref_ll_neg, &c->ref_pairs2, &c->ref_exps2,
                      &c->partial, &c->tmp0, &c->tmp1, &c->tmp2, &c->cubtmp, &c->pk_count,
                      &c->mt_words, &c->mt_state, &c->mt_fin, &c->mt_poly, &c->mt_seq,
                      &c->comm_stack, &c->comm_recv, &c->comm_send, &c->metric_mask, &c->metric_small})
        b->release();
    return 0;
}

int plsa_timing_enable(plsa_ctx *c, int32_t on) {
    if (!on) CHK(timing_flush(c));
    c->timing = on != 0;
    return 0;
}

int plsa_timing_reset(plsa_ctx *c) {
    CHK(timing_flush(c));
    std::fill(c->acc_ms.begin(), c->acc_ms.end(), 0.0);
    std::fill(c->acc_n.begin(), c->acc_n.end(), 0);
    return 0;
}

int plsa_timing_get(plsa_ctx *c, const char *prefix, double *total_ms, int64_t *launches) {
    CHK(timing_flush(c));
    double t = 0.0;
    i64 n = 0;
    const size_t pl = strlen(prefix);
    for (size_t i = 0; i < c->names.size(); ++i)
        if (c->names[i].compare(0, pl, prefix) == 0) { t += c->acc_ms[i]; n += c->acc_n[i]; }
    if (total_ms) *total_ms = t;
    if (launches) *launches = n;
    return 0;
}

int plsa_timing_report(plsa_ctx *c, char *buf, int64_t cap) {
    CHK(timing_flush(c));
    std::string s;
    char line[256];
    for (size_t i = 0; i < c->names.size(); ++i) {
        if (!c->acc_n[i]) continue;
        snprintf(line, sizeof line, "%s %lld %.6f\n", c->names[i].c_str(), (long long)c->acc_n[i], c->acc_ms[i]);
        s += line;
    }
    if (cap > 0) { strncpy(buf, s.c_str(), (size_t)cap - 1); buf[cap - 1] = 0; }
    return 0;
}

int plsa_measure_stream_bandwidth(plsa_ctx *c, int64_t bytes, int32_t kind, int32_t reps, double *gbps) {
    HIPCHK(c, hipSetDevice(c->device));
    if (bytes < (1 << 20) || reps < 1 || kind < 0 || kind > 6) return fail(c, "plsa_measure_stream_bandwidth: bad arguments");
    DevBuf a, b;
    const i64 n4 = bytes / 16;
    CHK(ensure(c, a, (size_t)n4 * 16));
    if (kind == 2) CHK(ensure(c, b, (size_t)n4 * 16));
    Event e0, e1;
    (void)hipEventCreate(&e0.h); (void)hipEventCreate(&e1.h);
    const int grid = grid_for(c, n4, 256);
    for (int r = -1; r < reps; ++r) {
        if (r == 0) (void)hipEventRecord(e0, c->stream);
        if (kind == 0) hipLaunchKernelGGL((plsa::k_probe_fill<true>), dim3(grid), dim3(256), 0, c->stream, a.as<float>(), n4);
        else if (kind == 1) hipLaunchKernelGGL((plsa::k_probe_fill<false>), dim3(grid), dim3(256), 0, c->stream, a.as<float>(), n4);
        else if (kind >= 4) hipLaunchKernelGGL(plsa::k_probe_fill_tiled, dim3(grid_for(c, n4, 256 * (kind == 4 ? 16 : kind == 5 ? 4 : 64))), dim3(256), 0, c->stream, a.as<float>(), n4, kind == 4 ? 16 : kind == 5 ? 4 : 64);
        else if (kind == 3) hipLaunchKernelGGL(plsa::k_probe_read, dim3(grid), dim3(256), 0, c->stream, a.as<float>(), a.as<float>(), n4);
        else hipLaunchKernelGGL(plsa::k_probe_copy, dim3(grid), dim3(256), 0, c->stream, a.as<float>(), b.as<float>(), n4);
    }
    (void)hipEventRecord(e1, c->stream);
    hipError_t e = hipStreamSynchronize(c->stream);
    float ms = 0.f;
    (void)hipEventElapsedTime(&ms, e0, e1);
    if (e != hipSuccess) return fail(c, "stream probe failed: %s", hipGetErrorString(e));
    const double moved = (double)n4 * 16.0 * (kind == 2 ? 2.0 : 1.0) * reps;
    *gbps = moved / 1e9 / (ms / 1e3);
    return 0;
}

void plsa_host_normalize_rows(double *a, int64_t rows, int64_t cols) {
    for (int64_t i = 0; i < rows; ++i) {
        double *r = a + i * cols;
        double marginal = 0.0;
        for (int64_t j = 0; j < cols; ++j) marginal += r[j];
        if (marginal > 0.0)
            for (int64_t j = 0; j < cols; ++j) r[j] /= marginal;
    }
}

int plsa_all_pairs_hellinger(plsa_ctx *c, const float *topics, int64_t t, int64_t m, double *D) {
    HIPCHK(c, hipSetDevice(c->device));
    if (!topics || !D || t <= 0 || m <= 0 || t > 65536) return fail(c, "plsa_all_pairs_hellinger: bad arguments");
    const int nt = (int)((t + plsa::HELL_TILE - 1) / plsa::HELL_TILE);
    std::vector<int> ti, tj;
    for (int i = 0; i < nt; ++i) for (int j = i; j < nt; ++j) { ti.push_back(i); tj.push_back(j); }
    int slices = (int)std::max<i64>(1, std::min<i64>(64, (4 * (i64)c->prop.multiProcessorCount + (i64)ti.size() - 1) / (i64)ti.size()));
    i64 slice = ((m + slices - 1) / slices + plsa::HELL_KSTEP - 1) / plsa::HELL_KSTEP * plsa::HELL_KSTEP;
    slices = (int)((m + slice - 1) / slice);
    DevBuf R, l1, part, dD, dt;
    CHK(ensure(c, R, sizeof(float) * (size_t)t * m));
    CHK(ensure(c, l1, sizeof(double) * (size_t)t));
    CHK(ensure(c, part, sizeof(double) * (size_t)slices * t * t));
    CHK(ensure(c, dD, sizeof(double) * (size_t)t * t));
    CHK(ensure(c, dt, sizeof(int) * 2 * ti.size()));
    hipError_t e = hipMemcpyAsync(R.p, topics, sizeof(float) * (size_t)t * m, hipMemcpyHostToDevice, c->stream);
    if (e == hipSuccess) e = hipMemcpyAsync(dt.p, ti.data(), sizeof(int) * ti.size(), hipMemcpyHostToDevice, c->stream);
    if (e == hipSuccess) e = hipMemcpyAsync(dt.as<int>() + ti.size(), tj.data(), sizeof(int) * tj.size(), hipMemcpyHostToDevice, c->stream);
    if (e == hipSuccess) {
        hipLaunchKernelGGL(plsa::k_hell_prepare, dim3((unsigned)t), dim3(256), 0, c->stream, R.as<float>(), (int)t, (i64)m, l1.as<double>());
        { Scope s(c, "k_hell_gram");
          hipLaunchKernelGGL(plsa::k_hell_gram, dim3((unsigned)ti.size(), (unsigned)slices), dim3(256), 0, c->stream,
                             R.as<float>(), (int)t, (i64)m, slice, dt.as<int>(), dt.as<int>() + ti.size(), part.as<double>()); }
        hipLaunchKernelGGL(plsa::k_hell_finish, dim3((unsigned)((t * t + 255) / 256)), dim3(256), 0, c->stream,
                           part.as<double>(), slices, (int)t, l1.as<double>(), dD.as<double>());
        e = hipGetLastError();
    }
    if (e == hipSuccess) e = hipMemcpyAsync(D, dD.p, sizeof(double) * (size_t)t * t, hipMemcpyDeviceToHost, c->stream);
    if (e == hipSuccess) e = hipStreamSynchronize(c->stream);
    if (e != hipSuccess) return fail(c, "plsa_all_pairs_hellinger: %s", hipGetErrorString(e));
    return 0;
}

int plsa_codocument_counts(plsa_ctx *c, const int32_t *words, int64_t sets, int32_t nw, int32_t max_sets_per_pass,
                           int64_t *co, int64_t *positive) {
    if (!c) return fail(c, "plsa_codocument_counts: ctx is NULL");
    HIPCHK(c, hipSetDevice(c->device));
    if (nw < 2 || nw > plsa::METRIC_MAX_WORDS)
        return fail(c, "plsa_codocument_counts: nw=%d outside [2,%d]", nw, plsa::METRIC_MAX_WORDS);
// ... 267 lines not shown
```

enstop_amd/csrc/plsa_kernels.hpp:

```cpp
#pragma once
#include <hip/hip_runtime.h>
#include <stdint.h>

#ifndef PLSA_UNR
#define PLSA_UNR 4
#endif
#ifndef PLSA_NT_STREAMS
#define PLSA_NT_STREAMS 0
#endif
#ifndef PLSA_UNR_E
#define PLSA_UNR_E 16
#endif
#ifndef PLSA_WAVES
#define PLSA_WAVES 1
#endif
#ifndef PLSA_UNR_COL
#define PLSA_UNR_COL 8
#endif
#ifndef PLSA_WAVES_COL
#define PLSA_WAVES_COL PLSA_WAVES
#endif

namespace plsa {

// ... 408 lines not shown
                                                float *__restrict__ U_new,
                                                float *__restrict__ norm_pdz_out, int kp_rt, unsigned block, unsigned nblocks) {
    constexpr int LPN = S::LPN, CH = S::CH;
    constexpr int GPB = 256 / LPN;
    const int kp = S::kp(kp_rt);
    const int li = threadIdx.x % LPN;
    const int gid = threadIdx.x / LPN;
    for (i64 d = (i64)block * GPB + gid; d < n; d += (i64)nblocks * GPB) {
        const int i0 = ritem_first[d], i1 = ritem_first[d + 1];
        float4 acc[CH];
#pragma unroll
        for (int j = 0; j < CH; ++j) acc[j] = zero4();
        for (int it = i0; it < i1; ++it) {
            float4 p[CH];
            load_row<S, true>(rpartial + (i64)it * kp, li, kp, p);
#pragma unroll
            for (int j = 0; j < CH; ++j) {
                acc[j].x += p[j].x; acc[j].y += p[j].y; acc[j].z += p[j].z; acc[j].w += p[j].w;
            }
        }
        float part = 0.f;
#pragma unroll
        for (int j = 0; j < CH; ++j) part += hsum(acc[j]);
        const float rown = group_sum<LPN>(part);
        if (norm_pdz_out && li == 0) norm_pdz_out[d] = rown;
#pragma unroll
        for (int j = 0; j < CH; ++j) {
            if (S::ok(li, j, kp)) {
                float4 o = acc[j];
                if (rown > 0.f) { o.x /= rown; o.y /= rown; o.z /= rown; o.w /= rown; }
                st4(U_new + d * kp + S::c4(li, j), o);
            }
        }
    }
}

template <class S>
__global__ __launch_bounds__(256) void k_row_reduce(const int *__restrict__ ritem_first, int n,
                                                    const float *__restrict__ rpartial,
                                                    float *__restrict__ U_new,
                                                    float *__restrict__ norm_pdz_out, int kp_rt) {
    row_reduce_body<S>(ritem_first, n, rpartial, U_new, norm_pdz_out, kp_rt, blockIdx.x, gridDim.x);
}

__global__ void k_ritem_fill(const int *__restrict__ indptr, const int *__restrict__ ritem_first, int n,
                             int seg, int *__restrict__ ritem_row, int *__restrict__ ritem_start) {
    const i64 d = (i64)blockIdx.x * blockDim.x + threadIdx.x;
    if (d < n) {
        const int i0 = ritem_first[d], i1 = ritem_first[d + 1];
        for (int i = i0; i < i1; ++i) {
            ritem_row[i] = (int)d;
            ritem_start[i] = indptr[d] + (i - i0) * seg;
        }
    }
}

template <class S, int THREADS = 256>
__device__ __forceinline__ void block_colsum(const float4 (&csum)[S::CH], int li, int gid, int kp,
                                             double *sred , double *__restrict__ out_row) {
    constexpr int GPB = THREADS / S::LPN;
#pragma unroll
    for (int j = 0; j < S::CH; ++j) {
        if (S::ok(li, j, kp)) {
            double *p = sred + gid * kp + S::c4(li, j);
            p[0] = (double)csum[j].x; p[1] = (double)csum[j].y; p[2] = (double)csum[j].z; p[3] = (double)csum[j].w;
        }
    }
    __syncthreads();
    for (int z = threadIdx.x; z < kp; z += THREADS) {
        double t = 0.0;
        for (int g = 0; g < GPB; ++g) t += sred[g * kp + z];
        out_row[z] = t;
    }
}

template <class S, bool FROM_P, int UN, bool TINY>
__device__ __forceinline__ void col_batch(int s0, int d_l, float x_l, int p_l, int li, int kp, float thresh,
                                          const float *__restrict__ U, const float *__restrict__ P,
                                          const float4 (&vt)[S::CH], float4 (&acc)[S::CH]) {
    constexpr int LPN = S::LPN, CH = S::CH;
    constexpr bool OWNER = !FROM_P && UN >= 4;
    float4 a[UN][CH];
    float x[UN];
#pragma unroll
    for (int q = 0; q < UN; ++q) {
        if (!OWNER) x[q] = __shfl(x_l, s0 + q, LPN);
        if (FROM_P) {
            const int pos = __shfl(p_l, s0 + q, LPN);
            load_row<S, false>(P + (i64)pos * kp, li, kp, a[q]);
        } else {
            const int d = __shfl(d_l, s0 + q, LPN);
            gather_row<S>(U, d, li, kp, a[q]);
        }
    }
    if (OWNER) {
        float nmine = 0.f;
#pragma unroll
        for (int q = 0; q < UN; ++q) {
            float unth;
            float norm = group_sum<LPN>(products<CH, false>(a[q], vt, thresh, a[q], unth));
            rescue_tiny(TINY, norm, a[q]);
            nmine = (li == s0 + q) ? norm : nmine;
        }
        const float xs_mine = x_l * inv_norm(nmine);
#pragma unroll
        for (int q = 0; q < UN; ++q) {
            const float xs = __shfl(xs_mine, s0 + q, LPN);
#pragma unroll
            for (int j = 0; j < CH; ++j) {
                acc[j].x += xs * a[q][j].x; acc[j].y += xs * a[q][j].y;
                acc[j].z += xs * a[q][j].z; acc[j].w += xs * a[q][j].w;
            }
        }
        return;
    }
#pragma unroll
    for (int q = 0; q < UN; ++q) {
        float4 pz[CH];
        if (FROM_P) {
#pragma unroll
            for (int j = 0; j < CH; ++j) pz[j] = S::ok(li, j, kp) ? a[q][j] : zero4();
        } else {
            float unth;
            float norm = group_sum<LPN>(products<CH, false>(a[q], vt, thresh, pz, unth));
            rescue_tiny(TINY, norm, pz);
            x[q] *= inv_norm(norm);
        }
#pragma unroll
        for (int j = 0; j < CH; ++j) {
            acc[j].x += x[q] * pz[j].x; acc[j].y += x[q] * pz[j].y;
            acc[j].z += x[q] * pz[j].z; acc[j].w += x[q] * pz[j].w;
        }
    }
}

template <class S, bool FROM_P, bool TIMED, bool TINY>
__device__ __forceinline__ void col_pass_body(const int4 *__restrict__ item_rec, i64 n_items,
                                                  const int *__restrict__ xcd_lo,
                                                  const int *__restrict__ csc_row,
                                                  const float *__restrict__ csc_val,
                                                  const int *__restrict__ csc_pos,
                                                  const float *__restrict__ U,
                                                  const float *__restrict__ Vt,
                                                  const float *__restrict__ P,
                                                  const float *__restrict__ sw,
                                                  float *__restrict__ partial, int kp_rt, float thresh,
                                                  int xcd_split, double *__restrict__ chunk_sums,
                                                  unsigned long long *__restrict__ t_end, double *scol , unsigned block, unsigned nblocks) {
    constexpr int LPN = S::LPN, CH = S::CH, UNR = S::UNR_COL;
    constexpr int GPB = 256 / LPN;
    const int kp = S::kp(kp_rt);
    const int li = threadIdx.x % LPN;
    const int gid = threadIdx.x / LPN;
    const int n_chunks = (int)((n_items + GPB - 1) / GPB);
    const int xcd = xcd_split ? (int)(block & 7) : 0;
    const int nq = xcd_split ? (int)((nblocks + 7 - xcd) / 8) : (int)nblocks;
    const int q = xcd_split ? (int)(block >> 3) : (int)block;
    const int c_lo = xcd_split ? xcd_lo[xcd] : 0, c_hi = xcd_split ? xcd_lo[xcd + 1] : n_chunks;
    if (TIMED && block == 0 && threadIdx.x == 0) t_end[nblocks] = wall_clock64();
    for (int chunk = c_lo + q; chunk < c_hi; chunk += nq) {
        const i64 io = (i64)chunk * GPB + gid;
        float4 acc[CH];
#pragma unroll
        for (int j = 0; j < CH; ++j) acc[j] = zero4();
        if (io < n_items) {
            const int4 rec = item_rec[io];
            const int w = rec.x, j0 = rec.y, j1 = rec.z;
            float4 vt[CH];
            load_row<S, true, PLSA_NT_STREAMS>(Vt + (i64)w * kp, li, kp, vt);
            int d_n = (j0 + li < j1) ? ldi(csc_row + j0 + li) : 0;
            float x_n = (!S::PACKED && j0 + li < j1) ? ldf(csc_val + j0 + li) : 0.f;
            int p_n = (FROM_P && j0 + li < j1) ? ldi(csc_pos + j0 + li) : 0;
            for (int jb = j0; jb < j1; jb += LPN) {
                int d_l = d_n;
                const int p_l = p_n;
                float x_l = x_n;
                if (S::PACKED) unpack_entry(d_l, x_l, csc_val, jb + li, j1);
                const int jn = jb + LPN + li;
                d_n = jn < j1 ? ldi(csc_row + jn) : 0;
                if (!S::PACKED) x_n = jn < j1 ? ldf(csc_val + jn) : 0.f;
                if (FROM_P) p_n = jn < j1 ? ldi(csc_pos + jn) : 0;
                if (sw) x_l *= sw[d_l];
                const int cnt = min(LPN, j1 - jb);
                int s0 = 0;
                for (; s0 + UNR <= cnt; s0 += UNR)
                    col_batch<S, FROM_P, UNR, TINY>(s0, d_l, x_l, p_l, li, kp, thresh, U, P, vt, acc);
                constexpr int TAIL = (UNR >= 2 && LPN >= 2) ? 2 : 1;
                for (; s0 < cnt; s0 += TAIL)
                    col_batch<S, FROM_P, TAIL, TINY>(s0, d_l, x_l, p_l, li, kp, thresh, U, P, vt, acc);
            }
#pragma unroll
            for (int j = 0; j < CH; ++j)
                if (S::ok(li, j, kp)) st4(partial + (i64)rec.w * kp + S::c4(li, j), acc[j]);
        }
        block_colsum<S>(acc, li, gid, kp, scol, chunk_sums + (i64)chunk * kp);
        __syncthreads();
    }
    if (TIMED && threadIdx.x == 0) t_end[block] = wall_clock64();
}

template <class S, bool FROM_P, bool TIMED, bool TINY = false>
__global__ __launch_bounds__(256, PLSA_WAVES_COL) void k_col_pass(const int4 *__restrict__ item_rec, i64 n_items,
                                                  const int *__restrict__ xcd_lo,
                                                  const int *__restrict__ csc_row,
                                                  const float *__restrict__ csc_val,
                                                  const int *__restrict__ csc_pos,
                                                  const float *__restrict__ U,
                                                  const float *__restrict__ Vt,
                                                  const float *__restrict__ P,
                                                  const float *__restrict__ sw,
                                                  float *__restrict__ partial, int kp_rt, float thresh,
                                                  int xcd_split, double *__restrict__ chunk_sums,
                                                  unsigned long long *__restrict__ t_end) {
    extern __shared__ double scol[];
    col_pass_body<S, FROM_P, TIMED, TINY>(item_rec, n_items, xcd_lo, csc_row, csc_val, csc_pos, U, Vt, P, sw, partial, kp_rt, thresh,
                                          xcd_split, chunk_sums, t_end, scol, blockIdx.x, gridDim.x);
}

__global__ void k_item_records(const int *__restrict__ item_order, const int *__restrict__ item_col,
                               const int *__restrict__ item_start, const int *__restrict__ item_end, i64 n_items,
                               int4 *__restrict__ rec) {
    const i64 io = (i64)blockIdx.x * blockDim.x + threadIdx.x;
    if (io < n_items) {
        const int it = item_order ? item_order[io] : (int)io;
        rec[io] = make_int4(item_col[it], item_start[it], item_end[it], it);
    }
}

__device__ __forceinline__ float div_pos(float v, float n) { return n > 0.f ? v / n : v; }

template <class S, bool NORMALISE>
__device__ __forceinline__ void col_reduce_body(const int *__restrict__ item_first, int m, int heavy_items,
                                                const int *__restrict__ heavy_cols, int n_heavy,
                                                const float *__restrict__ partial, float *__restrict__ Vt_new,
                                                int kp, int block, int nblocks, float *sacc ,
                                                const float *snorm ) {
    constexpr int LPN = S::LPN, CH = S::CH;
    constexpr int GPB = 256 / LPN;
    const int li = threadIdx.x % LPN;
    const int gid = threadIdx.x / LPN;
    float4 acc[CH];
    for (int h = block; h < n_heavy; h += nblocks) {
        const int c = heavy_cols[h];
        const int i0 = item_first[c], i1 = item_first[c + 1];
#pragma unroll
        for (int j = 0; j < CH; ++j) acc[j] = zero4();
        constexpr int B = 4;
        for (int it = i0 + gid; it < i1; it += GPB * B) {
            float4 p[B][CH];
#pragma unroll
            for (int u = 0; u < B; ++u) {
                const int iu = it + u * GPB;
                if (iu < i1) {
                    load_row<S, true>(partial + (i64)iu * kp, li, kp, p[u]);
                } else {
#pragma unroll
                    for (int j = 0; j < CH; ++j) p[u][j] = zero4();
                }
            }
#pragma unroll
            for (int u = 0; u < B; ++u)
#pragma unroll
                for (int j = 0; j < CH; ++j) {
                    acc[j].x += p[u][j].x; acc[j].y += p[u][j].y; acc[j].z += p[u][j].z; acc[j].w += p[u][j].w;
                }
        }
#pragma unroll
        for (int j = 0; j < CH; ++j)
            if (S::ok(li, j, kp)) st4(sacc + gid * kp + S::c4(li, j), acc[j]);
        __syncthreads();
        for (int z = threadIdx.x; z < kp; z += 256) {
            float t = 0.f;
            for (int g = 0; g < GPB; ++g) t += sacc[g * kp + z];
            Vt_new[(i64)c * kp + z] = NORMALISE ? div_pos(t, snorm[z]) : t;
        }
        __syncthreads();
    }
    for (i64 c = (i64)block * GPB + gid; c < m; c += (i64)nblocks * GPB) {
        const int i0 = item_first[c], i1 = item_first[c + 1];
        if (i1 - i0 > heavy_items) continue;
#pragma unroll
        for (int j = 0; j < CH; ++j) acc[j] = zero4();
        int it = i0;
        for (; it + 4 <= i1; it += 4) {
            float4 p[4][CH];
#pragma unroll
            for (int u = 0; u < 4; ++u) load_row<S, true>(partial + (i64)(it + u) * kp, li, kp, p[u]);
#pragma unroll
            for (int u = 0; u < 4; ++u)
#pragma unroll
                for (int j = 0; j < CH; ++j) {
                    acc[j].x += p[u][j].x; acc[j].y += p[u][j].y; acc[j].z += p[u][j].z; acc[j].w += p[u][j].w;
                }
        }
        for (; it < i1; ++it) {
            float4 p[CH];
            load_row<S, true>(partial + (i64)it * kp, li, kp, p);
#pragma unroll
            for (int j = 0; j < CH; ++j) {
                acc[j].x += p[j].x; acc[j].y += p[j].y; acc[j].z += p[j].z; acc[j].w += p[j].w;
            }
        }
#pragma unroll
        for (int j = 0; j < CH; ++j) {
            if (S::ok(li, j, kp)) {
                float4 o = acc[j];
                if (NORMALISE) {
                    const float *nn = snorm + S::c4(li, j);
                    o.x = div_pos(o.x, nn[0]); o.y = div_pos(o.y, nn[1]); o.z = div_pos(o.z, nn[2]); o.w = div_pos(o.w, nn[3]);
                }
                st4(Vt_new + c * kp + S::c4(li, j), o);
            }
        }
    }
}

template <class S>
__global__ __launch_bounds__(256) void k_col_reduce(const int *__restrict__ item_first, int m,
                                                    int heavy_items, const int *__restrict__ heavy_cols,
                                                    int n_heavy, const float *__restrict__ partial,
                                                    float *__restrict__ Vt_new, int kp_rt) {
    extern __shared__ float sacc[];
    col_reduce_body<S, false>(item_first, m, heavy_items, heavy_cols, n_heavy, partial, Vt_new, S::kp(kp_rt),
                              (int)blockIdx.x, (int)gridDim.x, sacc, nullptr);
}

template <class S>
__global__ __launch_bounds__(256) void k_col_reduce_norm(const int *__restrict__ item_first, int m,
                                                         int heavy_items, const int *__restrict__ heavy_cols,
                                                         int n_heavy, const float *__restrict__ partial,
                                                         const float *__restrict__ norm_pwz,
                                                         float *__restrict__ Vt_out, int kp_rt) {
    extern __shared__ float sdyn[];
    const int kp = S::kp(kp_rt);
    constexpr int GPB = 256 / S::LPN;
    float *snorm = sdyn + GPB * kp;
    for (int z = threadIdx.x; z < kp; z += 256) snorm[z] = norm_pwz[z];
    __syncthreads();
    col_reduce_body<S, true>(item_first, m, heavy_items, heavy_cols, n_heavy, partial, Vt_out, kp,
                             (int)blockIdx.x, (int)gridDim.x, sdyn, snorm);
}

__global__ void k_heavy_list(const int *__restrict__ item_first, int m, int heavy_items,
                             int *__restrict__ heavy_cols, int *__restrict__ n_heavy) {
    const i64 c = (i64)blockIdx.x * blockDim.x + threadIdx.x;
    if (c < m && item_first[c + 1] - item_first[c] > heavy_items)
        heavy_cols[atomicAdd(n_heavy, 1)] = (int)c;
}

constexpr int NORM_BLOCKS = 256;

__device__ __forceinline__ void colsum_slab_body(const float *__restrict__ Vt_new, int m, int kp, int slab,
                                                 int n_slabs, double *__restrict__ partials, double *sred ) {
    const i64 per = ((i64)m + n_slabs - 1) / n_slabs;
    const i64 w0 = (i64)slab * per, w1 = min((i64)m, w0 + per);
    for (int zb = 0; zb < kp; zb += 256) {
        const int span = min(256, kp - zb);
        const int rpp = 256 / span;
        const int z = zb + (int)threadIdx.x % span;
        const int ro = (int)threadIdx.x / span;
        float s = 0.f;
        if (ro < rpp)
            for (i64 w = w0 + ro; w < w1; w += rpp) s += Vt_new[w * kp + z];
        sred[threadIdx.x] = (ro < rpp) ? (double)s : 0.0;
        __syncthreads();
        if ((int)threadIdx.x < span) {
            double tot = 0.0;
            for (int r = 0; r < rpp; ++r) tot += sred[r * span + threadIdx.x];
            partials[(i64)slab * kp + zb + threadIdx.x] = tot;
        }
        __syncthreads();
    }
}

__global__ __launch_bounds__(256) void k_colsum_partial(const float *__restrict__ Vt_new, int m,
                                                        int kp, double *__restrict__ partials) {
    extern __shared__ double sred_dyn[];
    colsum_slab_body(Vt_new, m, kp, (int)blockIdx.x, (int)gridDim.x, partials, sred_dyn);
}

__device__ __forceinline__ void colsum_final_body(const double *__restrict__ partials, int n_partials, int kp,
                                                  float *out, double *sred ) {
    for (int zb = 0; zb < kp; zb += 256) {
        const int span = min(256, kp - zb);
        const int rpp = 256 / span;
        const int z = zb + (int)threadIdx.x % span;
        const int ro = (int)threadIdx.x / span;
        double tot = 0.0;
        if (ro < rpp) {
#pragma unroll 8
            for (int b = ro; b < n_partials; b += rpp) tot += partials[(i64)b * kp + z];
        }
        sred[threadIdx.x] = tot;
        __syncthreads();
        if ((int)threadIdx.x < span) {
            double t2 = 0.0;
            for (int r = 0; r < rpp; ++r) t2 += sred[r * span + threadIdx.x];
            out[zb + threadIdx.x] = (float)t2;
        }
        __syncthreads();
    }
}

__global__ __launch_bounds__(256) void k_colsum_final(const double *__restrict__ partials, int n_partials,
                                                      int kp, float *__restrict__ norm_pwz) {
    __shared__ double sred[256];
    colsum_final_body(partials, n_partials, kp, norm_pwz, sred);
}

__device__ __forceinline__ void norm_reduce_body(const double *__restrict__ in, int rows, int kp,
                                                 double *__restrict__ out, double *sred , unsigned block,
                                                 unsigned nblocks) {
    const i64 per = ((i64)rows + nblocks - 1) / nblocks;
    const i64 r0 = (i64)block * per, r1 = min((i64)rows, r0 + per);
    for (int zb = 0; zb < kp; zb += 256) {
        const int span = min(256, kp - zb);
        const int rpp = 256 / span;
        const int z = zb + (int)threadIdx.x % span;
        const int ro = (int)threadIdx.x / span;
        double s = 0.0;
        if (ro < rpp) {
#pragma unroll 8
            for (i64 r = r0 + ro; r < r1; r += rpp) s += in[r * kp + z];
        }
        sred[threadIdx.x] = (ro < rpp) ? s : 0.0;
        __syncthreads();
        if ((int)threadIdx.x < span) {
            double tot = 0.0;
            for (int r = 0; r < rpp; ++r) tot += sred[r * span + threadIdx.x];
            out[(i64)block * kp + zb + threadIdx.x] = tot;
        }
        __syncthreads();
    }
}

__global__ __launch_bounds__(256) void k_norm_reduce(const double *__restrict__ in, int rows, int kp,
                                                     double *__restrict__ out) {
    __shared__ double sred[256];
    norm_reduce_body(in, rows, kp, out, sred, blockIdx.x, gridDim.x);
}

__device__ __forceinline__ void v_normalise_body(const float *__restrict__ Vt_new, float *__restrict__ Vt, int m,
                                                 int kp, const float *snorm, int block, int nblocks) {
    const i64 total4 = (i64)m * kp / 4;
    const int kq = kp / 4;
    for (i64 i = (i64)block * 256 + threadIdx.x; i < total4; i += (i64)nblocks * 256) {
        const int z4 = (int)(i % kq) * 4;
        float4 v = ld4(Vt_new + i * 4);
        const float n0 = snorm[z4], n1 = snorm[z4 + 1], n2 = snorm[z4 + 2], n3 = snorm[z4 + 3];
        if (n0 > 0.f) v.x /= n0;
        if (n1 > 0.f) v.y /= n1;
        if (n2 > 0.f) v.z /= n2;
        if (n3 > 0.f) v.w /= n3;
        st4(Vt + i * 4, v);
    }
}

__global__ __launch_bounds__(256) void k_v_normalise(const float *__restrict__ Vt_new,
                                                     float *__restrict__ Vt, int m, int kp,
                                                     const float *__restrict__ norm_pwz) {
    extern __shared__ float snorm[];
    for (int z = threadIdx.x; z < kp; z += 256) snorm[z] = norm_pwz[z];
    __syncthreads();
    v_normalise_body(Vt_new, Vt, m, kp, snorm, (int)blockIdx.x, (int)gridDim.x);
}

__device__ __forceinline__ void ll_final_body(const double *__restrict__ partials, int nb, double *__restrict__ out,
                                              double *red ) {
    double s = 0.0;
    for (int i = threadIdx.x; i < nb; i += 256) s += partials[i];
    red[threadIdx.x] = s;
    __syncthreads();
    for (int st = 128; st > 0; st >>= 1) {
        if ((int)threadIdx.x < st) red[threadIdx.x] += red[threadIdx.x + st];
        __syncthreads();
    }
    if (threadIdx.x == 0) out[0] = red[0];
}

__global__ void k_ll_final(const double *__restrict__ partials, int nb, double *__restrict__ out) {
    __shared__ double red[256];
    ll_final_body(partials, nb, out, red);
}

template <class S>
__global__ __launch_bounds__(256, PLSA_WAVES) void k_loglik(const int *__restrict__ indptr,
                                                const int *__restrict__ colidx,
                                                const float *__restrict__ vals, int n,
                                                const int *__restrict__ row_order,
                                                const float *__restrict__ U,
                                                const float *__restrict__ Vt,
                                                const float *__restrict__ sw, int kp_rt,
                                                double *__restrict__ ll_partials) {
    constexpr int LPN = S::LPN, CH = S::CH, UNR = S::UNR;
    constexpr int GPB = 256 / LPN;
    const int kp = S::kp(kp_rt);
    const int li = threadIdx.x % LPN;
    const int gid = threadIdx.x / LPN;
    double ll = 0.0;
// ... 789 lines not shown
```

enstop_amd/csrc/plsa_member_kernels.hpp:

```cpp
#pragma once

#include "plsa_kernels.hpp"

namespace plsa {

constexpr int MEMBERS_MAX = 64;

struct MemberArgs {
    const int4 *item_rec;
    const int *csc_row;
    const float *csc_val;
    float *partial;
    double *chunk_sums;
    i64 n_items;
    double *chunk_sums2;
    float *norm_pwz;
    const int *item_first, *heavy_cols;
    int n_chunks, norm_blocks;
    int m, n_heavy, heavy_items, reduce_grid;
    const int *indptr, *colidx;
    const float *vals;
    const int *row_order, *ritem_row, *ritem_start, *ritem_first;
    float *rpartial;
    double *ll_partials, *ll_out;
    i64 n_ritems;
    int n, rseg, row_grid, row_reduce_grid;
    float *U[2], *Vt[2];
};

__device__ __forceinline__ bool member_live(u64 live, unsigned r) { return (live >> r) & 1ull; }

template <class S, bool WANT_LL, bool TINY>
__global__ __launch_bounds__(256, PLSA_WAVES) void k_row_pass_members(const MemberArgs *__restrict__ args, u64 live, u64 cu,
                                                                      u64 cv, int kp_rt, float thresh) {
    const unsigned r = blockIdx.y;
    if (!member_live(live, r)) return;
    const MemberArgs &a = args[r];
    if (blockIdx.x >= (unsigned)a.row_grid) return;
    const int pu = (int)((cu >> r) & 1ull), pv = (int)((cv >> r) & 1ull);
    row_pass_body<S, false, WANT_LL, TINY>(a.indptr, a.colidx, a.vals, a.n, a.row_order, a.U[pu], a.Vt[pv], nullptr, a.U[1 - pu],
                                           nullptr, nullptr, kp_rt, thresh, a.ll_partials, a.ritem_row, a.ritem_start, a.rseg,
                                           a.n_ritems, a.rpartial, 0, blockIdx.x, (unsigned)a.row_grid);
}

template <class S>
__global__ __launch_bounds__(256) void k_row_reduce_members(const MemberArgs *__restrict__ args, u64 live, u64 cu, int kp_rt) {
    const unsigned r = blockIdx.y;
    if (!member_live(live, r)) return;
    const MemberArgs &a = args[r];
    if (!a.ritem_row || blockIdx.x >= (unsigned)a.row_reduce_grid) return;
    const int pu = (int)((cu >> r) & 1ull);
    row_reduce_body<S>(a.ritem_first, a.n, a.rpartial, a.U[1 - pu], nullptr, kp_rt, blockIdx.x, (unsigned)a.row_reduce_grid);
}

__global__ __launch_bounds__(256) void k_ll_final_members(const MemberArgs *__restrict__ args, u64 live) {
    __shared__ double red[256];
    const unsigned r = blockIdx.x;
    if (!member_live(live, r)) return;
    const MemberArgs &a = args[r];
    ll_final_body(a.ll_partials, a.row_grid, a.ll_out, red);
}

template <class S, bool TINY>
__global__ __launch_bounds__(256, PLSA_WAVES_COL) void k_col_pass_members(const MemberArgs *__restrict__ args, u64 live, u64 cu,
                                                                          u64 cv, int kp_rt, float thresh) {
    extern __shared__ double scol[];
    const unsigned r = blockIdx.y;
    if (!member_live(live, r)) return;
    const MemberArgs &a = args[r];
    if (blockIdx.x >= (unsigned)a.n_chunks) return;
    const int pu = (int)((cu >> r) & 1ull), pv = (int)((cv >> r) & 1ull);
    const unsigned nblocks = min((unsigned)a.n_chunks, gridDim.x);
    col_pass_body<S, false, false, TINY>(a.item_rec, a.n_items, nullptr, a.csc_row, a.csc_val, nullptr, a.U[pu], a.Vt[pv], nullptr,
                                         nullptr, a.partial, kp_rt, thresh, 0, a.chunk_sums, nullptr, scol, blockIdx.x, nblocks);
}

__global__ __launch_bounds__(256) void k_norm_reduce_members(const MemberArgs *__restrict__ args, u64 live, int kp) {
    __shared__ double sred[256];
    const unsigned r = blockIdx.y;
    if (!member_live(live, r)) return;
    const MemberArgs &a = args[r];
    if (blockIdx.x >= (unsigned)a.norm_blocks) return;
    norm_reduce_body(a.chunk_sums, a.n_chunks, kp, a.chunk_sums2, sred, blockIdx.x, (unsigned)a.norm_blocks);
}

__global__ __launch_bounds__(256) void k_colsum_final_members(const MemberArgs *__restrict__ args, u64 live, int kp) {
    __shared__ double sred[256];
    const unsigned r = blockIdx.x;
    if (!member_live(live, r)) return;
    const MemberArgs &a = args[r];
    if (a.norm_blocks > 0) colsum_final_body(a.chunk_sums2, a.norm_blocks, kp, a.norm_pwz, sred);
    else colsum_final_body(a.chunk_sums, a.n_chunks, kp, a.norm_pwz, sred);
}

template <class S>
__global__ __launch_bounds__(256) void k_col_reduce_norm_members(const MemberArgs *__restrict__ args, u64 live, u64 cv,
                                                                 int kp_rt) {
    extern __shared__ float sdyn[];
    const unsigned r = blockIdx.y;
    if (!member_live(live, r)) return;
    const MemberArgs &a = args[r];
    if (blockIdx.x >= (unsigned)a.reduce_grid) return;
    const int kp = S::kp(kp_rt);
    constexpr int GPB = 256 / S::LPN;
    float *snorm = sdyn + GPB * kp;
    for (int z = threadIdx.x; z < kp; z += 256) snorm[z] = a.norm_pwz[z];
    __syncthreads();
    const int pv = (int)((cv >> r) & 1ull);
    col_reduce_body<S, true>(a.item_first, a.m, a.heavy_items, a.heavy_cols, a.n_heavy, a.partial, a.Vt[1 - pv], kp,
                             (int)blockIdx.x, a.reduce_grid, sdyn, snorm);
}

}
```

enstop_amd/csrc/plsa_members.hpp:

```cpp
#pragma once

struct plsa_members {
    struct MemberDelete {
        void operator()(plsa_ctx *m) const {
            if (!m) return;
            m->stream.h = nullptr; m->stream2.h = nullptr;
            delete m;
        }
    };
    using Member = std::unique_ptr<plsa_ctx, MemberDelete>;
    plsa_ctx *leader = nullptr;
    std::vector<Member> ctx;
    std::vector<char> prepared;
    struct Info { int group = -1, group_size = 0, items = 0, rseg = 0, n_chunks = 0, n_heavy = 0, row_grid = 0, norm_blocks = 0; };
    std::vector<Info> info;
    std::vector<double> last_ll;
    DevBuf table, ll_out;
    Pinned<double> h_ll;
};

namespace {

int new_member(plsa_ctx *leader, plsa_members::Member &out) {
    plsa_members::Member m(new plsa_ctx());
    m->device = leader->device;
    m->prop = leader->prop;
    m->stream.h = leader->stream.h;
    m->stream2.h = leader->stream2.h;
    m->ls = m->stream;
    if (hipEventCreateWithFlags(&m->ev_fork.h, hipEventDisableTiming) != hipSuccess ||
        hipEventCreateWithFlags(&m->ev_join.h, hipEventDisableTiming) != hipSuccess ||
        hipEventCreateWithFlags(&m->ev_row.h, hipEventDisableTiming) != hipSuccess ||
        hipEventCreateWithFlags(&m->ev_tail.h, hipEventDisableTiming) != hipSuccess ||
        hipEventCreateWithFlags(&m->ev_ll.h, hipEventDisableTiming) != hipSuccess ||
        host_alloc(m->h_ll, 2) != hipSuccess)
        return fail(leader, "plsa_members: event / pinned buffer creation failed");
    read_knobs(m.get());
    out = std::move(m);
    return 0;
}

struct ScratchLoan {
    plsa_ctx *l, *m;
    void swap_all() {
        for (auto p : {&plsa_ctx::tmp0, &plsa_ctx::tmp1, &plsa_ctx::tmp2, &plsa_ctx::cubtmp, &plsa_ctx::pk_count, &plsa_ctx::mt_words,
                       &plsa_ctx::mt_state, &plsa_ctx::mt_fin, &plsa_ctx::mt_poly, &plsa_ctx::mt_seq})
            (l->*p).swap(m->*p);
    }
    ScratchLoan(plsa_ctx *l_, plsa_ctx *m_) : l(l_), m(m_) { swap_all(); }
    ~ScratchLoan() { swap_all(); }
};

int member_rc(plsa_ctx *leader, plsa_ctx *m, int rc) {
    if (rc) leader->err = m->err;
    return rc;
}

int members_check(plsa_members *b, int32_t member) {
    if (!b) return fail(nullptr, "plsa_members: NULL batch");
    if (member < 0 || member >= (int32_t)b->ctx.size())
        return fail(b->leader, "plsa_members: member %d outside [0, %d)", member, (int)b->ctx.size());
    return 0;
}

int member_args(plsa_ctx *c, double *ll_out, plsa::MemberArgs &a, plsa_members::Info &inf) {
    CHK(ensure_packed_csc(c));
    CHK(ensure_packed_csr(c));
    CHK(ensure_ritems(c));
    const bool items = c->ritems.use && c->ritems.n > 0;
    const int *order = nullptr;
    if (!items) CHK(ensure_roworder(c, &order));
    const int row_grid = grid_for(c, items ? c->ritems.n : c->n, 256 / c->row_lpn);
    if (items) CHK(ensure(c, c->rpartial, sizeof(float) * (size_t)c->ritems.n * c->kp));
    CHK(ensure(c, c->ll_partials, sizeof(double) * (size_t)row_grid));
    CHK(ensure(c, c->partial, sizeof(float) * (size_t)std::max<i64>(c->csc.n_items, 1) * c->kp));
    const int gpb = 256 / c->lpn;
    const int n_chunks = (int)((c->csc.n_items + gpb - 1) / gpb);
    CHK(ensure(c, c->colsum_rows, sizeof(double) * (size_t)std::max(n_chunks, 1) * c->kp));
    CHK(ensure(c, c->norm_pwz, sizeof(float) * (size_t)c->kp));
    int norm_blocks = 0;
    if (n_chunks > 2048) {
        norm_blocks = std::max(64, std::min(1024, n_chunks / 64));
        CHK(ensure(c, c->colsum_rows2, sizeof(double) * (size_t)norm_blocks * c->kp));
    }
    const bool pk_col = c->packed && c->pk_csc.ok, pk_row = c->packed && c->pk_csr.ok;
    a = plsa::MemberArgs{};
    a.item_rec = c->csc.item_rec.as<int4>();
    a.csc_row = pk_col ? c->pk_csc.buf.as<int>() : c->csc.row.as<int>();
    a.csc_val = c->csc.val.as<float>();
    a.partial = c->partial.as<float>();
    a.chunk_sums = c->colsum_rows.as<double>();
    a.n_items = c->csc.n_items;
    a.chunk_sums2 = c->colsum_rows2.as<double>();
    a.norm_pwz = c->norm_pwz.as<float>();
    a.item_first = c->csc.item_first.as<int>();
    a.heavy_cols = c->csc.heavy_cols.as<int>();
    a.n_chunks = n_chunks;
    a.norm_blocks = norm_blocks;
    a.m = (int)c->m;
    a.n_heavy = c->csc.n_heavy;
    a.heavy_items = c->heavy_items;
    a.reduce_grid = grid_for(c, c->m, gpb) + c->csc.n_heavy;
    a.indptr = c->indptr;
    a.colidx = pk_row ? c->pk_csr.buf.as<int>() : c->col;
    a.vals = c->val;
    a.row_order = order;
    a.ritem_row = items ? c->ritems.row.as<int>() : nullptr;
    a.ritem_start = items ? c->ritems.start.as<int>() : nullptr;
    a.ritem_first = items ? c->ritems.first.as<int>() : nullptr;
    a.rpartial = items ? c->rpartial.as<float>() : nullptr;
    a.ll_partials = c->ll_partials.as<double>();
    a.ll_out = ll_out;
    a.n_ritems = c->ritems.n;
    a.n = (int)c->n;
    a.rseg = c->ritems.seg;
    a.row_grid = row_grid;
    a.row_reduce_grid = grid_for(c, c->n, 256 / c->row_lpn);
    for (int i = 0; i < 2; ++i) { a.U[i] = c->U[i].as<float>(); a.Vt[i] = c->Vt[i].as<float>(); }
    inf.items = items; inf.rseg = c->ritems.seg; inf.n_chunks = n_chunks; inf.n_heavy = c->csc.n_heavy;
    inf.row_grid = row_grid; inf.norm_blocks = norm_blocks;
    c->colsum_rows_used = n_chunks;
    return 0;
}

template <class Fn>
int dispatch_narrow_row(plsa_ctx *c, Fn &&fn) {
    if (c->row_lpn == 8 && c->row_ch == 2 && c->kp == 64) { fn(plsa::Shape<8, 2, true>{}); return 0; }
    return dispatch_shape(c, fn);
}

int fit_group(plsa_members *b, const std::vector<int> &who, const std::vector<plsa::MemberArgs> &rows, int n_iter,
              int n_iter_per_test, double tolerance, float thresh, int flags, int32_t *iters_done, float *ll_trace, int ll_cap,
              int32_t *n_ll) {
    plsa_ctx *L = b->leader, *c0 = b->ctx[who[0]].get();
    const int G = (int)who.size();
    const bool trace = flags & PLSA_TRACE_LL, zero_arm = !(flags & PLSA_STOP_NO_ZERO_ARM);
    HIPCHK(L, hipMemcpyAsync(b->table.p, rows.data(), sizeof(plsa::MemberArgs) * (size_t)G, hipMemcpyHostToDevice, L->stream));
    HIPCHK(L, hipStreamSynchronize(L->stream));
    const plsa::MemberArgs *table = b->table.as<plsa::MemberArgs>();
    int row_x = 1, reduce_x = 1, chunks_x = 1, norm_x = 0, rr_x = 0;
    for (const auto &a : rows) {
        row_x = std::max(row_x, a.row_grid);
        reduce_x = std::max(reduce_x, a.reduce_grid);
        chunks_x = std::max(chunks_x, a.n_chunks);
        norm_x = std::max(norm_x, a.norm_blocks);
        if (a.ritem_row) rr_x = std::max(rr_x, a.row_reduce_grid);
    }
    const bool pk_row = c0->packed && c0->pk_csr.ok, pk_col = c0->packed && c0->pk_csc.ok;
    const bool tiny = thresh < plsa::TINY_THRESH;
    const int kp = c0->kp;
    using u64 = unsigned long long;
    u64 live = G == 64 ? ~0ull : ((1ull << G) - 1ull), cu = 0, cv = 0;
    for (int g = 0; g < G; ++g) {
        plsa_ctx *c = b->ctx[who[g]].get();
        if (c->cu) cu |= 1ull << g;
        if (c->cv) cv |= 1ull << g;
    }
    using T = std::true_type;
    using F = std::false_type;
    const bool two_streams = L->overlap;
    hipStream_t col_stream = two_streams ? L->stream2.h : L->stream.h;
    auto row_pass = [&](bool want_ll) -> int {
        CHK(dispatch_narrow_row(c0, [&](auto S) {
            using Sh = decltype(S);
            auto launch = [&](auto SS, auto LL, auto TN) {
                hipLaunchKernelGGL((plsa::k_row_pass_members<decltype(SS), decltype(LL)::value, decltype(TN)::value>),
                                   dim3(row_x, G), dim3(256), 0, L->stream, table, live, cu, cv, kp, thresh);
            };
            auto go = [&](auto LL, auto TN) { if (pk_row) launch(plsa::Packed<Sh>{}, LL, TN); else launch(Sh{}, LL, TN); };
            if (want_ll) { if (tiny) go(T{}, T{}); else go(T{}, F{}); }
            else { if (tiny) go(F{}, T{}); else go(F{}, F{}); }
            if (rr_x > 0)
                hipLaunchKernelGGL((plsa::k_row_reduce_members<Sh>), dim3(rr_x, G), dim3(256), 0, L->stream, table, live, cu, kp);
        }));
        if (want_ll) {
            hipLaunchKernelGGL(plsa::k_ll_final_members, dim3(G), dim3(256), 0, L->stream, table, live);
            HIPCHK(L, hipMemcpyAsync(b->h_ll.get(), b->ll_out.p, sizeof(double) * (size_t)G, hipMemcpyDeviceToHost, L->stream));
        }
        return launch_check(L, "k_row_pass_members");
    };
    auto col_chain = [&]() -> int {
        CHK(dispatch_shape(c0, [&](auto S) {
            using Sh = decltype(S);
            constexpr int GPB = 256 / Sh::LPN;
            const size_t smem = sizeof(double) * (size_t)GPB * kp;
            auto launch = [&](auto SS, auto TN) {
                hipLaunchKernelGGL((plsa::k_col_pass_members<decltype(SS), decltype(TN)::value>), dim3(chunks_x, G), dim3(256),
                                   smem, col_stream, table, live, cu, cv, kp, thresh);
            };
            auto go = [&](auto TN) { if (pk_col) launch(plsa::Packed<Sh>{}, TN); else launch(Sh{}, TN); };
            if (tiny) go(T{}); else go(F{});
            if (norm_x > 0)
                hipLaunchKernelGGL(plsa::k_norm_reduce_members, dim3(norm_x, G), dim3(256), 0, col_stream, table, live, kp);
            hipLaunchKernelGGL(plsa::k_colsum_final_members, dim3(G), dim3(256), 0, col_stream, table, live, kp);
            hipLaunchKernelGGL((plsa::k_col_reduce_norm_members<Sh>), dim3(reduce_x, G), dim3(256),
                               sizeof(float) * (size_t)(GPB + 1) * kp, col_stream, table, live, cv, kp);
        }));
        return launch_check(L, "k_col_pass_members");
    };
    std::vector<float> prev(G, 0.f);
    std::vector<int> nll(G, 0), iters(G, 0);
    auto record = [&](int g, float v) {
        if (ll_trace && nll[g] < ll_cap) ll_trace[(size_t)who[g] * ll_cap + nll[g]] = v;
        nll[g]++;
    };
    bool pending = false, first = true;
    for (int i = 0; i < n_iter && live; ++i) {
        const bool want_ll = pending || first;
        if (two_streams) {
            HIPCHK(L, hipEventRecord(L->ev_fork, L->stream));
            HIPCHK(L, hipStreamWaitEvent(L->stream2, L->ev_fork, 0));
        }
        CHK(col_chain());
        if (two_streams) HIPCHK(L, hipEventRecord(L->ev_join, L->stream2));
        CHK(row_pass(want_ll));
        if (two_streams) HIPCHK(L, hipStreamWaitEvent(L->stream, L->ev_join, 0));
        if (want_ll) {
            HIPCHK(L, hipStreamSynchronize(L->stream));
            for (int g = 0; g < G; ++g) {
                if (!((live >> g) & 1ull)) continue;
                const float cur = (float)b->h_ll[g];
                b->last_ll[who[g]] = b->h_ll[g];
                if (first) { prev[g] = cur; record(g, cur); continue; }
                record(g, cur);
                if (stop_test(cur, prev[g], tolerance, zero_arm)) live &= ~(1ull << g);
            }
            first = false;
        }
        cu ^= live; cv ^= live;
        for (int g = 0; g < G; ++g) if ((live >> g) & 1ull) iters[g]++;
        pending = (i % n_iter_per_test == 0);
    }
    HIPCHK(L, hipStreamSynchronize(L->stream));
    for (int g = 0; g < G; ++g) {
        plsa_ctx *c = b->ctx[who[g]].get();
        c->cu = (int)((cu >> g) & 1ull); c->cv = (int)((cv >> g) & 1ull);
        c->p_state.invalidate();
        if (((live >> g) & 1ull) && pending && trace) {
            ScratchLoan loan(L, c);
            double ll = 0.0;
            CHK(member_rc(L, c, run_loglik(c, nullptr, &ll)));
            b->last_ll[who[g]] = ll;
            record(g, (float)ll);
        }
        iters_done[who[g]] = iters[g];
        n_ll[who[g]] = nll[g];
    }
    return 0;
}

}

extern "C" {

int plsa_members_create(plsa_ctx *ctx, int32_t n_members, plsa_members **out) {
    if (!out) return fail(ctx, "plsa_members_create: out is NULL");
    *out = nullptr;
    if (!ctx) return fail(nullptr, "plsa_members_create: NULL context");
    if (n_members < 1 || n_members > PLSA_MEMBERS_MAX)
        return fail(ctx, "plsa_members_create: n_members=%d outside [1, %d]", n_members, (int)PLSA_MEMBERS_MAX);
    static_assert(PLSA_MEMBERS_MAX == plsa::MEMBERS_MAX, "the live mask is one 64-bit word");
    HIPCHK(ctx, hipSetDevice(ctx->device));
    std::unique_ptr<plsa_members> b(new plsa_members());
    b->leader = ctx;
    b->ctx.resize(n_members);
    b->prepared.assign(n_members, 0);
    b->info.assign(n_members, plsa_members::Info{});
    b->last_ll.assign(n_members, 0.0);
    for (auto &m : b->ctx) CHK(new_member(ctx, m));
    CHK(ensure(ctx, b->table, sizeof(plsa::MemberArgs) * (size_t)n_members));
    CHK(ensure(ctx, b->ll_out, sizeof(double) * (size_t)n_members));
    if (host_alloc(b->h_ll, (size_t)n_members) != hipSuccess) return fail(ctx, "plsa_members_create: pinned buffer allocation failed");
    *out = b.release();
    return 0;
}

void plsa_members_destroy(plsa_members *b) {
    if (!b) return;
    (void)hipSetDevice(b->leader->device);
    (void)hipStreamSynchronize(b->leader->stream);
    (void)hipStreamSynchronize(b->leader->stream2);
    delete b;
}

int plsa_members_release(plsa_members *b) {
    if (!b) return fail(nullptr, "plsa_members: NULL batch");
    plsa_ctx *L = b->leader;
    HIPCHK(L, hipSetDevice(L->device));
    HIPCHK(L, hipStreamSynchronize(L->stream));
    HIPCHK(L, hipStreamSynchronize(L->stream2));
    for (size_t r = 0; r < b->ctx.size(); ++r) {
        plsa_members::Member fresh;
        CHK(new_member(L, fresh));
        b->ctx[r] = std::move(fresh);
        b->prepared[r] = 0;
        b->info[r] = plsa_members::Info{};
    }
    return 0;
}

int plsa_members_prepare(plsa_members *b, int32_t member, const int64_t *idx, int64_t n_out, int32_t k,
                         uint32_t *mt_state_io, const float *U, const float *V) {
    CHK(members_check(b, member));
    plsa_ctx *L = b->leader, *c = b->ctx[member].get();
    HIPCHK(L, hipSetDevice(L->device));
    if (L->bn <= 0) return fail(L, "plsa_members_prepare: no corpus uploaded");
    if (!mt_state_io && (!U || !V)) return fail(L, "plsa_members_prepare: neither a generator state nor host factors");
    b->prepared[member] = 0;
    if (c->bn != L->bn || c->bm != L->bm || c->bnnz != L->bnnz) c->bal_have_frac = false;
    c->b_indptr.borrow(L->b_indptr.p, L->b_indptr.cap);
    c->b_col.borrow(L->b_col.p, L->b_col.cap);
    c->b_val.borrow(L->b_val.p, L->b_val.cap);
    c->bn = L->bn; c->bm = L->bm; c->bnnz = L->bnnz;
    ScratchLoan loan(L, c);
    CHK(member_rc(L, c, plsa_bootstrap(c, idx, n_out)));
    if (mt_state_io) CHK(member_rc(L, c, mt_init(c, k, mt_state_io, nullptr)));
    else CHK(member_rc(L, c, plsa_set_factors(c, U, V, c->n, c->m, k)));
    b->prepared[member] = 1;
    return 0;
}

int plsa_members_fit(plsa_members *b, int32_t n_active, int32_t n_iter, int32_t n_iter_per_test, double tolerance,
                     float thresh, int32_t flags, int32_t *iters_done, float *ll_trace, int32_t ll_cap, int32_t *n_ll,
                     int32_t *n_batched) {
    if (!b) return fail(nullptr, "plsa_members: NULL batch");
    plsa_ctx *L = b->leader;
    HIPCHK(L, hipSetDevice(L->device));
    if (n_active < 1 || n_active > (int32_t)b->ctx.size()) return fail(L, "plsa_members_fit: n_active=%d outside [1, %d]", n_active, (int)b->ctx.size());
    if (n_iter < 0 || n_iter_per_test <= 0) return fail(L, "plsa_members_fit: bad n_iter / n_iter_per_test");
    if (!iters_done || !n_ll) return fail(L, "plsa_members_fit: iters_done / n_ll is NULL");
    if (ll_trace && ll_cap < n_iter + 2) return fail(L, "plsa_members_fit: ll_cap=%d below n_iter + 2", ll_cap);
    for (int r = 0; r < n_active; ++r) {
        if (!b->prepared[r]) return fail(L, "plsa_members_fit: member %d is not prepared", r);
        if (b->ctx[r]->k != b->ctx[0]->k) return fail(L, "plsa_members_fit: members differ in k");
        b->info[r] = plsa_members::Info{};
    }
    if (n_batched) *n_batched = 0;
    const bool call_ok = (flags & PLSA_FUSED) && !(flags & (PLSA_REFERENCE_SUMS | PLSA_REFERENCE_LL | PLSA_SHARDED | PLSA_GRAPH)) &&
// ... 91 lines not shown
```

enstop_amd/engine.py:

```python
import ctypes as C
import os
import threading

import numpy as np

from . import _lib
from ._lib import (PLSA_FUSED, PLSA_REFERENCE_LL, PLSA_REFERENCE_SUMS, PLSA_SHARDED, PLSA_STOP_NO_ZERO_ARM, PLSA_SW_LL_ONLY,
                   PLSA_TRACE_LL, ptr)


class DeviceError(RuntimeError):
    pass


def default_device():
    if "ENSTOP_AMD_DEVICE" in os.environ:
        return int(os.environ["ENSTOP_AMD_DEVICE"])
    dev = int(os.environ.get("LOCAL_RANK", "0"))
    if dev > 0:
        cnt = C.c_int(0)
        if _lib.load().plsa_device_count(C.byref(cnt)) == 0 and 0 < cnt.value <= dev:
            if cnt.value != 1:
                raise RuntimeError("LOCAL_RANK=%d but only %d GPUs are visible: start one rank per visible GPU, "
                                   "narrow the devices to one per rank (HIP_VISIBLE_DEVICES), or set "
# ... 235 lines not shown
        return ll.value if want_ll else None

    def p_bytes(self):
        n, m, nnz = self.shape
        return 4 * (nnz + 64) * ((self.k + 3) // 4 * 4)

    def p_reserve(self, nbytes):
        out = C.c_void_p()
        self._ok(self._L.plsa_p_reserve(self._h, int(nbytes), C.byref(out)))
        return out.value

    def p_borrow(self, device_ptr, nbytes=0):
        self._ok(self._L.plsa_p_borrow(self._h, device_ptr, int(nbytes)))

    def em_finish(self):
        self._ok(self._L.plsa_em_finish(self._h))

    def set_sample_weight(self, sample_weight=None):
        sw = None if sample_weight is None else _f32(sample_weight)
        self._ok(self._L.plsa_set_sample_weight(self._h, ptr(sw)))

    def accumulator_device(self):
        p, n = C.c_void_p(), C.c_int64(0)
        self._ok(self._L.plsa_accumulator_device(self._h, C.byref(p), C.byref(n)))
        return p.value, n.value

    def accumulator_get(self):
        _, n = self.accumulator_device()
        out = np.empty(n, np.float32)
        self._ok(self._L.plsa_accumulator_get(self._h, out))
        return out

    def accumulator_set(self, a):
        self._ok(self._L.plsa_accumulator_set(self._h, _f32(a)))

    def comm_init(self, id_bytes, rank, world):
        if len(id_bytes) != 128:
            raise ValueError("the RCCL unique id has 128 bytes")
        self._ok(self._L.plsa_comm_init(self._h, bytes(id_bytes), int(rank), int(world)))

    def comm_destroy(self):
        self._ok(self._L.plsa_comm_destroy(self._h))

    def comm_info(self):
        r, w = C.c_int32(0), C.c_int32(1)
        self._ok(self._L.plsa_comm_info(self._h, C.byref(r), C.byref(w)))
        return r.value, w.value

    def comm_barrier(self):
        self._ok(self._L.plsa_comm_barrier(self._h))

    def stack_reserve(self, slots, k, m):
        base = C.c_void_p()
        self._ok(self._L.plsa_stack_reserve(self._h, int(slots), int(m), int(k), C.byref(base)))
        return int(base.value)

    def comm_allgather_stack(self, slots, k, m, copy=True, out=None):
        _, world = self.comm_info()
        shape = (int(slots) * world, int(k), int(m))
        if out is None and copy:
            out = np.empty(shape, np.float32)
        if out is not None:
            if out.dtype != np.float32 or not out.flags.c_contiguous or out.size != shape[0] * shape[1] * shape[2]:
                raise ValueError("out must be a C-contiguous float32 array of %d elements" % (shape[0] * shape[1] * shape[2]))
            self._ok(self._L.plsa_comm_allgather_stack_to(self._h, int(slots), int(m), int(k), out.reshape(-1)))
            return out.reshape(shape)
        p = C.POINTER(C.c_float)()
        self._ok(self._L.plsa_comm_allgather_stack(self._h, int(slots), int(m), int(k), C.byref(p)))
        return np.ctypeslib.as_array(p, shape=shape)

    def comm_allgather_host(self, a):
        a = np.ascontiguousarray(a)
        _, world = self.comm_info()
        out = np.empty((world,) + a.shape, a.dtype)
        self._ok(self._L.plsa_comm_allgather_host(self._h, a.ctypes.data, a.nbytes, out.ctypes.data))
        return out

    def comm_allreduce_f64(self, values, op="sum"):
        a = np.atleast_1d(np.array(values, dtype=np.float64))
        self._ok(self._L.plsa_comm_allreduce_f64(self._h, a, a.size, {"sum": 0, "max": 1}[op]))
        return a

    def comm_broadcast_host(self, a, root=0):
        a = np.array(a, copy=True, order="C")
        self._ok(self._L.plsa_comm_broadcast_host(self._h, a.ctypes.data, a.nbytes, int(root)))
        return a

    def allreduce_accumulator(self):
        self._ok(self._L.plsa_allreduce_accumulator(self._h))

    def all_pairs_hellinger(self, topics):
        T = _f32(topics)
        if T.ndim != 2:
            raise ValueError("topics must be a 2-D array")
        t, m = T.shape
        D = np.empty((t, t), np.float64)
        self._ok(self._L.plsa_all_pairs_hellinger(self._h, ptr(T), t, m, D))
        return D

    def all_pairs_kl(self, topics):
        T = _f32(topics)
        if T.ndim != 2:
            raise ValueError("topics must be a 2-D array")
        t, m = T.shape
        D = np.empty((t, t), np.float64)
        self._ok(self._L.plsa_all_pairs_kl(self._h, ptr(T), t, m, D))
        return D

    def cluster_representatives(self, topics, labels, weights=None):
        T = _f32(topics)
        lab = np.ascontiguousarray(labels, dtype=np.int32)
        t, m = T.shape
        if lab.shape != (t,):
            raise ValueError("labels must have one entry per topic")
        n_clusters = int(lab.max()) + 1 if lab.size and lab.max() >= 0 else 0
        out = np.empty((n_clusters, m), np.float32)
        w = None if weights is None else np.ascontiguousarray(weights, dtype=np.float64)
        self._ok(self._L.plsa_cluster_representatives(self._h, ptr(T), t, m, lab, ptr(w), n_clusters, out))
        return out

    def codocument_counts(self, words, max_sets_per_pass=0):
        W = np.ascontiguousarray(words, dtype=np.int32)
        if W.ndim != 2:
            raise ValueError("words must be a 2-D array [sets, nw]")
        sets, nw = W.shape
        co = np.zeros((sets, nw, nw), np.int64)
        positive = np.zeros((sets, nw), np.int64)
        self._ok(self._L.plsa_codocument_counts(self._h, W.reshape(-1), sets, nw, int(max_sets_per_pass), co.reshape(-1),
                                                positive.reshape(-1)))
        return co, positive

    def reference_chain_info(self):
        a, b, c_ = C.c_int64(0), C.c_int64(0), C.c_int32(0)
        self._ok(self._L.plsa_reference_chain_info(self._h, C.byref(a), C.byref(b), C.byref(c_)))
        return dict(slow_chunks=a.value, chunks=b.value, serial_chain_now=bool(c_.value))

    def placement_info(self):
        n, a, b = C.c_int32(0), C.c_double(0.0), C.c_double(0.0)
        self._ok(self._L.plsa_placement_info(self._h, C.byref(n), C.byref(a), C.byref(b)))
        return dict(candidates=n.value, kept_fill_GBps=round(a.value, 1), worst_fill_GBps=round(b.value, 1))

    def balance_info(self):
        lo = (C.c_int32 * 9)(); t = (C.c_double * 8)()
        n, seg, items = C.c_int32(0), C.c_int32(0), C.c_int64(0)
        self._ok(self._L.plsa_schedule_info(self._h, lo, t, C.byref(n), C.byref(seg), C.byref(items)))
        return dict(xcd_chunk_boundaries=list(lo), xcd_finish_us=[round(v, 1) for v in t], timed_launches=n.value,
                    item_entries=seg.value, n_items=items.value)

    def packed_info(self):
        a, b = C.c_int32(0), C.c_int32(0)
        self._ok(self._L.plsa_packed_info(self._h, C.byref(a), C.byref(b)))
        name = {1: "packed", 0: "arrays", -1: None}
        return dict(csr=name[a.value], csc=name[b.value])

    def pass_info(self):
        col, row, wide = np.zeros(3, np.int32), np.zeros(3, np.int32), np.zeros(2, np.int32)
        self._ok(self._L.plsa_pass_info(self._h, col, row, wide))
        return dict(col=(int(col[0]), int(col[1]), bool(col[2])), row=(int(row[0]), int(row[1]), bool(row[2])),
                    row_wide=bool(wide[0]), col_wide=bool(wide[1]))

    def fit_info(self):
        a = np.zeros(7, np.int32)
        self._ok(self._L.plsa_fit_info(self._h, a))
        return dict(fused=bool(a[0]), pipelined=bool(a[1]), speculated=bool(a[2]), graph_launches=int(a[3]),
                    col_tail={0: None, 1: "sweep", 2: "four_kernels"}[int(a[4])], two_stage_norm=bool(a[5]),
                    xcd_split=bool(a[6]))

    def release_scratch(self):
        if self._member_batch is not None:
            self._member_batch.release()
        self._ok(self._L.plsa_release_scratch(self._h))

    def member_capacity(self, k):
        out = C.c_int32(0)
        self._ok(self._L.plsa_members_capacity(self._h, int(k), C.byref(out)))
        return out.value

    def member_batch(self, n_members):
        b = self._member_batch
        if b is None or b.n_members < n_members:
            if b is not None:
                b.close()
            b = self._member_batch = MemberBatch(self, n_members)
        return b

    def timing(self, on=True):
        self._ok(self._L.plsa_timing_enable(self._h, int(on)))
        self.timing_on = bool(on)

    def timing_reset(self):
        self._ok(self._L.plsa_timing_reset(self._h))

    def timing_get(self, prefix):
        ms, n = C.c_double(0.0), C.c_int64(0)
        self._ok(self._L.plsa_timing_get(self._h, prefix.encode(), C.byref(ms), C.byref(n)))
        return ms.value, n.value

    def stream_bandwidth(self, nbytes=1 << 32, kind=0, reps=5):
        out = C.c_double(0.0)
        self._ok(self._L.plsa_measure_stream_bandwidth(self._h, int(nbytes), int(kind), int(reps), C.byref(out)))
        return out.value

    def timing_report(self):
        buf = C.create_string_buffer(8192)
        self._ok(self._L.plsa_timing_report(self._h, buf, 8192))
        out = {}
        for line in buf.value.decode().splitlines():
            name, cnt, ms = line.rsplit(" ", 2)
            out[name] = (int(cnt), float(ms))
        return out


class _MemberView(Engine):

    def __init__(self, leader, handle):
        self._L = leader._L
        self._h = handle
        self.device = leader.device
        self.k = 0
        self.base_rows = leader.base_rows
        self.lock = leader.lock
        self._member_batch = None

    def close(self):
        self._h = C.c_void_p()


class MemberBatch:

    def __init__(self, eng, n_members):
        if not 1 <= int(n_members) <= _lib.MEMBERS_MAX:
            raise ValueError("a batch holds 1 to %d members, not %r" % (_lib.MEMBERS_MAX, n_members))
        self.eng = eng
        self._L = eng._L
        self._b = C.c_void_p()
        self.n_members = int(n_members)
        self.k = 0
        self.last_batched = 0
        eng._ok(self._L.plsa_members_create(eng._h, self.n_members, C.byref(self._b)))

    def close(self):
        if getattr(self, "_b", None) is not None and self._b.value:
            if self.eng._h.value:
                self._L.plsa_members_destroy(self._b)
            self._b = C.c_void_p()

    def __del__(self):
        try:
            self.close()
        except Exception:
            pass

    def release(self):
        self.eng._ok(self._L.plsa_members_release(self._b))

    def prepare(self, member, k, idx=None, rng=None, U=None, V=None):
        ip = None
        n_out = 0
        if idx is not None:
            idx = np.ascontiguousarray(idx, dtype=np.int64)
            ip, n_out = idx.ctypes.data, idx.shape[0]
        if rng is not None:
            kind, key, pos, has_gauss, cached = rng.get_state()
            if kind != "MT19937":
                raise ValueError("not an MT19937 RandomState")
            state = np.empty(625, np.uint32)
            state[:624] = key
            state[624] = pos
            self.eng._ok(self._L.plsa_members_prepare(self._b, int(member), ip, n_out, int(k), state.ctypes.data, None, None))
            rng.set_state((kind, state[:624].copy(), int(state[624]), has_gauss, cached))
        else:
            U, V = _f32(U), _f32(V)
            if U.ndim != 2 or V.ndim != 2 or U.shape[1] != int(k) or V.shape[0] != int(k):
                raise ValueError("host factors must be U [n, k] and V [k, m]")
            self.eng._ok(self._L.plsa_members_prepare(self._b, int(member), ip, n_out, int(k), None, ptr(U), ptr(V)))
        self.k = int(k)

    def fit(self, n_active=None, n_iter=100, n_iter_per_test=10, tolerance=0.001, e_step_thresh=1e-32, flags=None, trace=False):
        n_active = self.n_members if n_active is None else int(n_active)
        flags = default_flags() if flags is None else int(flags)
        if trace:
            flags |= PLSA_TRACE_LL
        cap = int(n_iter) + 2
        iters, nll = np.zeros(n_active, np.int32), np.zeros(n_active, np.int32)
        ll = np.zeros((n_active, cap), np.float32)
        nb = C.c_int32(0)
        self.eng._ok(self._L.plsa_members_fit(self._b, n_active, int(n_iter), int(n_iter_per_test), float(tolerance),
                                              np.float32(e_step_thresh), flags, iters, ll.ctypes.data, cap, nll, C.byref(nb)))
        self.last_batched = nb.value
        return iters, [ll[r, :nll[r]].copy() for r in range(n_active)]

    def copy_components(self, member, device_ptr):
        self.eng._ok(self._L.plsa_members_copy_components(self._b, int(member), int(device_ptr)))

    def member(self, member):
        h = C.c_void_p()
        self.eng._ok(self._L.plsa_members_context(self._b, int(member), C.byref(h)))
        view = _MemberView(self.eng, h)
        view.k = self.k
        return view

    def components(self, member):
        return self.member(member).get_factors(want_u=False)[1]

    def last_ll(self, member):
        out = C.c_double(0.0)
# ... 50 lines not shown
```

include/plsa_hip_diag.h:

```cpp
#ifndef PLSA_HIP_DIAG_H
#define PLSA_HIP_DIAG_H

#include "plsa_hip.h"

#ifdef __cplusplus
extern "C" {
#endif

int plsa_hw_queues(void);
int plsa_device_info(plsa_ctx *ctx, char *name64, char *arch64, int *cus, int64_t *hbm_bytes);

int plsa_download_active_csr(plsa_ctx *ctx, int32_t *indptr, int32_t *indices, float *data);

int plsa_init_factors_device(plsa_ctx *ctx, int32_t k, uint64_t seed);

int plsa_mt_marginals(plsa_ctx *ctx, double *out, int32_t k);

int plsa_set_p(plsa_ctx *ctx, const float *P);

int plsa_accumulator_get(plsa_ctx *ctx, float *host);
int plsa_accumulator_set(plsa_ctx *ctx, const float *host);

int plsa_comm_last_error(plsa_ctx *ctx, char *buf, int64_t cap);

int plsa_comm_barrier(plsa_ctx *ctx);
int plsa_comm_allreduce_f64(plsa_ctx *ctx, double *inout, int64_t count, int32_t op);

int plsa_reference_chain_info(plsa_ctx *ctx, int64_t *slow_chunks, int64_t *chunks, int32_t *serial_now);

int plsa_placement_info(plsa_ctx *ctx, int32_t *candidates, double *best_gbps, double *worst_gbps);

int plsa_schedule_info(plsa_ctx *ctx, int32_t *xcd_lo , double *xcd_end_us , int32_t *timed_launches,
                       int32_t *item_len, int64_t *n_items);

int plsa_packed_info(plsa_ctx *ctx, int32_t *csr, int32_t *csc);

int plsa_pass_info(plsa_ctx *ctx, int32_t *col , int32_t *row , int32_t *wide );

int plsa_fit_info(plsa_ctx *ctx, int32_t *info );

int plsa_timing_enable(plsa_ctx *ctx, int32_t on);
int plsa_timing_reset(plsa_ctx *ctx);
int plsa_timing_get(plsa_ctx *ctx, const char *prefix, double *total_ms, int64_t *launches);
int plsa_timing_report(plsa_ctx *ctx, char *buf, int64_t cap);
int plsa_measure_stream_bandwidth(plsa_ctx *ctx, int64_t bytes, int32_t kind, int32_t reps, double *gbps);

void plsa_host_normalize_rows(double *a, int64_t rows, int64_t cols);

int plsa_host_mt19937_jump(uint32_t *key , int32_t log2_blocks);

int plsa_generate_synthetic(plsa_ctx *ctx, int64_t n, int64_t m, int64_t nnz_target, double zipf_s,
                            uint64_t seed, int64_t *nnz_out);
int plsa_generate_synthetic_topics(plsa_ctx *ctx, int64_t n, int64_t m, int64_t nnz_target, double zipf_s,
                                   uint64_t seed, int32_t k0, double alpha, double background, int64_t *nnz_out);
int plsa_synthetic_dominant_topics(plsa_ctx *ctx, int32_t *out );

#ifdef __cplusplus
}
#endif
#endif
```

Baseline: 348.9 iter/s.

## Merge consecutive same-column items in a chunk into one partial row

```diff
diff --git a/enstop_amd/_lib.py b/enstop_amd/_lib.py
--- a/enstop_amd/_lib.py
+++ b/enstop_amd/_lib.py
@@ -80,6 +80,7 @@
     "plsa_schedule_info": (C.c_int, [_ctx, C.POINTER(_i32), C.POINTER(C.c_double), C.POINTER(_i32), C.POINTER(_i32),
                                      C.POINTER(C.c_int64)]),
     "plsa_packed_info": (C.c_int, [_ctx, C.POINTER(_i32), C.POINTER(_i32)]),
+    "plsa_partial_info": (C.c_int, [_ctx, _i64p]),
     "plsa_pass_info": (C.c_int, [_ctx, _i32p, _i32p, _i32p]),
     "plsa_fit_info": (C.c_int, [_ctx, _i32p]),
     "plsa_release_scratch": (C.c_int, [_ctx]),
diff --git a/enstop_amd/csrc/plsa_hip.hip b/enstop_amd/csrc/plsa_hip.hip
--- a/enstop_amd/csrc/plsa_hip.hip
+++ b/enstop_amd/csrc/plsa_hip.hip
@@ -106,13 +106,19 @@
     struct RowIndex : Derived<RowIndex> { DevBuf ids; } rowidx;
 
     struct Csc : Derived<Csc> {
-        DevBuf colptr, row, val, pos, item_first, item_col, item_start, item_end, item_order, heavy_cols;
+        DevBuf colptr, row, val, pos, item_first, item_col, item_start, item_end, item_order;
         DevBuf item_rec;
         DevBuf xcd_lo;
         bool balanced = false;
-        int seg = 256, n_heavy = 0;
+        int seg = 256;
         i64 n_items = 0;
     } csc;
+    struct Runs : Derived<Runs> {
+        DevBuf first, heavy_cols;
+        i64 n = 0;
+        int gpb = 0, n_heavy = 0;
+    } runs;
+    bool partial_runs = true;
     int seg_override = 0, struct_lpn = 0;
     int struct_row_lpn = 0;
     DevBuf partial;
@@ -667,8 +673,19 @@
     return 0;
 }
 
+int ensure_runs(plsa_ctx *c);
+
+inline size_t col_pass_smem(int gpb, int kp) { return sizeof(double) * (size_t)gpb * kp + sizeof(int) * (size_t)gpb; }
+
+int build_csc(plsa_ctx *c);
+
 int ensure_csc(plsa_ctx *c) {
-    if (c->csc.valid) return 0;
+    if (!c->csc.valid) CHK(build_csc(c));
+    return ensure_runs(c);
+}
+
+int build_csc(plsa_ctx *c) {
+    c->runs.invalidate();
     CHK(ensure_rowidx(c));
     {
         const i64 slots = (i64)c->prop.multiProcessorCount * 32 * (64 / std::max(1, c->lpn));
@@ -754,21 +771,7 @@
         HIPCHK(c, hipcub::DeviceRadixSort::SortPairs(c->cubtmp.p, bytes, d_key, d_key + ni,
                                                      c->tmp1.as<int>(), c->csc.item_order.as<int>(), n_items, 0, key_bits, c->stream));
     }
-    CHK(ensure(c, c->csc.item_rec, sizeof(int4) * ni));
-    if (n_items > 0) {
-        hipLaunchKernelGGL(plsa::k_item_records, dim3((unsigned)((n_items + 255) / 256)), dim3(256), 0, c->stream,
-                           c->use_item_order ? c->csc.item_order.as<int>() : nullptr, c->csc.item_col.as<int>(),
-                           c->csc.item_start.as<int>(), c->csc.item_end.as<int>(), (i64)n_items, c->csc.item_rec.as<int4>());
-        CHK(launch_check(c, "k_item_records"));
-    }
     c->csc.balanced = false;
-    CHK(ensure(c, c->csc.heavy_cols, sizeof(int) * (size_t)(m + 1)));
-    HIPCHK(c, hipMemsetAsync(c->csc.heavy_cols.as<int>() + m, 0, sizeof(int), c->stream));
-    hipLaunchKernelGGL(plsa::k_heavy_list, dim3((unsigned)((m + 255) / 256)), dim3(256), 0, c->stream,
-                       c->csc.item_first.as<int>(), (int)m, c->heavy_items, c->csc.heavy_cols.as<int>(),
-                       c->csc.heavy_cols.as<int>() + m);
-    CHK(launch_check(c, "k_heavy_list"));
-    HIPCHK(c, hipMemcpyAsync(&c->csc.n_heavy, c->csc.heavy_cols.as<int>() + m, sizeof(int), hipMemcpyDeviceToHost, c->stream));
     unsigned long long escaped = 0;
     if (pack) HIPCHK(c, hipMemcpyAsync(&escaped, c->pk_count.p, sizeof escaped, hipMemcpyDeviceToHost, c->stream));
     HIPCHK(c, hipStreamSynchronize(c->stream));
@@ -776,6 +779,46 @@
     c->pk_csc.valid = c->packed;
     c->pk_csc.ok = pack && escaped * 16 <= (unsigned long long)nnz;
     if (!c->pk_csc.ok) c->pk_csc.buf.release();
+    return 0;
+}
+
+int ensure_runs(plsa_ctx *c) {
+    const int gpb = 256 / std::max(1, c->lpn);
+    if (c->runs.valid && c->runs.gpb == gpb) return 0;
+    const i64 n_items = c->csc.n_items, m = c->m;
+    const size_t ni = (size_t)std::max<i64>(n_items, 1);
+    CHK(ensure(c, c->runs.first, sizeof(int) * (size_t)(m + 1)));
+    CHK(ensure(c, c->csc.item_rec, sizeof(int4) * ni));
+    CHK(ensure(c, c->tmp0, sizeof(int) * (ni + 1)));
+    CHK(ensure(c, c->tmp1, sizeof(int) * (ni + 1)));
+    int *d_pos = c->tmp0.as<int>(), *d_flag = c->tmp1.as<int>(), *d_run = c->tmp0.as<int>();
+    const int *order = c->use_item_order ? c->csc.item_order.as<int>() : nullptr;
+    const dim3 gi((unsigned)((n_items + 256) / 256)), gm((unsigned)((m + 256) / 256));
+    hipLaunchKernelGGL(plsa::k_item_positions, gi, dim3(256), 0, c->stream, order, n_items, d_pos);
+    hipLaunchKernelGGL(plsa::k_item_run_flags, gi, dim3(256), 0, c->stream, d_pos, c->csc.item_col.as<int>(),
+                       c->csc.item_first.as<int>(), n_items, gpb, c->partial_runs ? 1 : 0, d_flag);
+    CHK(launch_check(c, "k_item_run_flags"));
+    CHK(exclusive_sum_int(c, d_flag, d_run, n_items + 1));
+    hipLaunchKernelGGL(plsa::k_run_first, gm, dim3(256), 0, c->stream, c->csc.item_first.as<int>(), d_run, (int)m,
+                       c->runs.first.as<int>());
+    if (n_items > 0)
+        hipLaunchKernelGGL(plsa::k_item_records, dim3((unsigned)((n_items + 255) / 256)), dim3(256), 0, c->stream, order,
+                           c->csc.item_col.as<int>(), c->csc.item_start.as<int>(), c->csc.item_end.as<int>(), d_run, n_items,
+                           c->csc.item_rec.as<int4>());
+    CHK(launch_check(c, "k_item_records"));
+    CHK(ensure(c, c->runs.heavy_cols, sizeof(int) * (size_t)(m + 1)));
+    HIPCHK(c, hipMemsetAsync(c->runs.heavy_cols.as<int>() + m, 0, sizeof(int), c->stream));
+    hipLaunchKernelGGL(plsa::k_heavy_list, dim3((unsigned)((m + 255) / 256)), dim3(256), 0, c->stream,
+                       c->runs.first.as<int>(), (int)m, c->heavy_items, c->runs.heavy_cols.as<int>(),
+                       c->runs.heavy_cols.as<int>() + m);
+    CHK(launch_check(c, "k_heavy_list"));
+    int n_runs = 0;
+    HIPCHK(c, hipMemcpyAsync(&n_runs, d_run + n_items, sizeof(int), hipMemcpyDeviceToHost, c->stream));
+    HIPCHK(c, hipMemcpyAsync(&c->runs.n_heavy, c->runs.heavy_cols.as<int>() + m, sizeof(int), hipMemcpyDeviceToHost, c->stream));
+    HIPCHK(c, hipStreamSynchronize(c->stream));
+    c->runs.n = n_runs;
+    c->runs.gpb = gpb;
+    c->runs.valid = true;
     return 0;
 }
 
@@ -847,6 +890,7 @@
     }
     if (lpn != prev_lpn) {
         c->eitems.invalidate();
+        c->runs.invalidate();
         if (!c->seg_override) c->csc.invalidate();
         c->struct_lpn = lpn;
     }
@@ -1080,7 +1124,7 @@
 int run_col_pass(plsa_ctx *c, bool from_p, const float *d_sw, float thresh, int parts = 3) {
     CHK(from_p ? ensure_csc(c) : ensure_packed_csc(c));
     const bool packed = !from_p && c->packed && c->pk_csc.ok;
-    CHK(ensure(c, c->partial, sizeof(float) * (size_t)std::max<i64>(c->csc.n_items, 1) * c->kp));
+    CHK(ensure(c, c->partial, sizeof(float) * (size_t)std::max<i64>(c->runs.n, 1) * c->kp));
     int rc = 0;
     CHK(dispatch_shape_gather(c, table_is_wide(c, c->n), [&](auto S) {
         using Sh = decltype(S);
@@ -1094,7 +1138,7 @@
             c->fit_info.xcd_split = xcd_split;
             rc = ensure(c, c->colsum_rows, sizeof(double) * (size_t)std::max(n_chunks, 1) * c->kp);
             if (rc) return;
-            const size_t smem = sizeof(double) * (size_t)GPB * c->kp;
+            const size_t smem = col_pass_smem(GPB, c->kp);
             auto launch = [&](bool timed) -> int {
                 int grid = col_grid(c, n_chunks, xcd_split != 0);
                 if (c->small_grid > 0 && (double)c->nnz * c->kp < c->overlap_full_limit)
@@ -1135,9 +1179,9 @@
         }
         if (parts & 2) {
             Scope s(c, "k_col_reduce");
-            hipLaunchKernelGGL((plsa::k_col_reduce<Sh>), dim3(grid2 + c->csc.n_heavy), dim3(256),
+            hipLaunchKernelGGL((plsa::k_col_reduce<Sh>), dim3(grid2 + c->runs.n_heavy), dim3(256),
                                (256 / LPN) * c->kp * sizeof(float), c->ls,
-                               c->csc.item_first.as<int>(), (int)c->m, c->heavy_items, c->csc.heavy_cols.as<int>(), c->csc.n_heavy,
+                               c->runs.first.as<int>(), (int)c->m, c->heavy_items, c->runs.heavy_cols.as<int>(), c->runs.n_heavy,
                                c->partial.as<float>(), c->Vacc.as<float>(), c->kp);
         }
     }));
@@ -1208,9 +1252,9 @@
         constexpr int GPB = 256 / Sh::LPN;
         const int grid2 = grid_for(c, c->m, GPB);
         Scope s(c, "k_col_reduce_norm");
-        hipLaunchKernelGGL((plsa::k_col_reduce_norm<Sh>), dim3(grid2 + c->csc.n_heavy), dim3(256),
-                           sizeof(float) * (size_t)(GPB + 1) * c->kp, c->ls, c->csc.item_first.as<int>(), (int)c->m,
-                           c->heavy_items, c->csc.heavy_cols.as<int>(), c->csc.n_heavy, c->partial.as<float>(),
+        hipLaunchKernelGGL((plsa::k_col_reduce_norm<Sh>), dim3(grid2 + c->runs.n_heavy), dim3(256),
+                           sizeof(float) * (size_t)(GPB + 1) * c->kp, c->ls, c->runs.first.as<int>(), (int)c->m,
+                           c->heavy_items, c->runs.heavy_cols.as<int>(), c->runs.n_heavy, c->partial.as<float>(),
                            c->norm_pwz.as<float>(), c->Vt[out_v(c)].as<float>(), c->kp);
     }));
     return launch_check(c, "k_col_reduce_norm");
@@ -1617,6 +1661,7 @@
     if (const char *s = getenv("PLSA_ROW_XCD")) c->row_xcd = atoi(s) != 0;
     if (const char *s = getenv("PLSA_ITEM_ORDER")) c->use_item_order = atoi(s) != 0;
     if (const char *s = getenv("PLSA_XCD_SPLIT")) c->xcd_split = atoi(s) != 0;
+    if (const char *s = getenv("PLSA_PARTIAL_RUNS")) c->partial_runs = atoi(s) != 0;
     if (const char *s = getenv("PLSA_BALANCE")) c->balance = atoi(s);
     if (const char *s = getenv("PLSA_ORDER_BAND")) c->order_band = atoi(s);
     if (const char *s = getenv("PLSA_GRAPH")) c->graph = atoi(s) != 0;
@@ -2679,6 +2724,15 @@
     return 0;
 }
 
+int plsa_partial_info(plsa_ctx *c, int64_t *out) {
+    if (!out) return fail(c, "plsa_partial_info: NULL argument");
+    const bool have = c->csc.valid && c->runs.valid && c->runs.gpb == 256 / std::max(1, c->lpn);
+    out[0] = c->csc.valid ? c->csc.n_items : 0;
+    out[1] = have ? c->runs.n : 0;
+    out[2] = have ? c->runs.n_heavy : 0;
+    return 0;
+}
+
 int plsa_packed_info(plsa_ctx *c, int32_t *csr, int32_t *csc) {
     if (csr) *csr = !c->packed ? 0 : (c->pk_csr.valid ? (c->pk_csr.ok ? 1 : 0) : -1);
     if (csc) *csc = !c->packed ? 0 : (c->csc.valid && c->pk_csc.valid ? (c->pk_csc.ok ? 1 : 0) : -1);
diff --git a/enstop_amd/csrc/plsa_kernels.hpp b/enstop_amd/csrc/plsa_kernels.hpp
--- a/enstop_amd/csrc/plsa_kernels.hpp
+++ b/enstop_amd/csrc/plsa_kernels.hpp
@@ -584,6 +584,7 @@
     const int kp = S::kp(kp_rt);
     const int li = threadIdx.x % LPN;
     const int gid = threadIdx.x / LPN;
+    int *sslot = reinterpret_cast<int *>(scol + GPB * kp);
     const int n_chunks = (int)((n_items + GPB - 1) / GPB);
     const int xcd = xcd_split ? (int)(block & 7) : 0;
     const int nq = xcd_split ? (int)((nblocks + 7 - xcd) / 8) : (int)nblocks;
@@ -595,9 +596,11 @@
         float4 acc[CH];
 #pragma unroll
         for (int j = 0; j < CH; ++j) acc[j] = zero4();
+        if (li == 0) sslot[gid] = -1;
         if (io < n_items) {
             const int4 rec = item_rec[io];
             const int w = rec.x, j0 = rec.y, j1 = rec.z;
+            if (li == 0) sslot[gid] = rec.w;
             float4 vt[CH];
             load_row<S, true, PLSA_NT_STREAMS>(Vt + (i64)w * kp, li, kp, vt);
             int d_n = (j0 + li < j1) ? ldi(csc_row + j0 + li) : 0;
@@ -621,11 +624,25 @@
                 for (; s0 < cnt; s0 += TAIL)
                     col_batch<S, FROM_P, TAIL, TINY>(s0, d_l, x_l, p_l, li, kp, thresh, U, P, vt, acc);
             }
-#pragma unroll
-            for (int j = 0; j < CH; ++j)
-                if (S::ok(li, j, kp)) st4(partial + (i64)rec.w * kp + S::c4(li, j), acc[j]);
         }
         block_colsum<S>(acc, li, gid, kp, scol, chunk_sums + (i64)chunk * kp);
+        const int slot = sslot[gid];
+        if (slot >= 0 && (gid == 0 || sslot[gid - 1] != slot)) {
+            int g_end = gid + 1;
+            while (g_end < GPB && sslot[g_end] == slot) ++g_end;
+#pragma unroll
+            for (int j = 0; j < CH; ++j) {
+                if (S::ok(li, j, kp)) {
+                    const double *p = scol + gid * kp + S::c4(li, j);
+                    double t0 = p[0], t1 = p[1], t2 = p[2], t3 = p[3];
+                    for (int g = gid + 1; g < g_end; ++g) {
+                        p += kp;
+                        t0 += p[0]; t1 += p[1]; t2 += p[2]; t3 += p[3];
+                    }
+                    st4(partial + (i64)slot * kp + S::c4(li, j), make_float4((float)t0, (float)t1, (float)t2, (float)t3));
+                }
+            }
+        }
         __syncthreads();
     }
     if (TIMED && threadIdx.x == 0) t_end[block] = wall_clock64();
@@ -649,20 +666,44 @@
                                           xcd_split, chunk_sums, t_end, scol, blockIdx.x, gridDim.x);
 }
 
+__global__ void k_item_positions(const int *__restrict__ item_order, i64 n_items, int *__restrict__ pos) {
+    const i64 io = (i64)blockIdx.x * blockDim.x + threadIdx.x;
+    if (io < n_items) pos[item_order ? item_order[io] : (int)io] = (int)io;
+}
+
+__global__ void k_item_run_flags(const int *__restrict__ pos, const int *__restrict__ item_col,
+                                 const int *__restrict__ item_first, i64 n_items, int gpb, int merge,
+                                 int *__restrict__ flag) {
+    const i64 it = (i64)blockIdx.x * blockDim.x + threadIdx.x;
+    if (it > n_items) return;
+    int f = 0;
+    if (it < n_items) {
+        const int p = pos[it];
+        f = !merge || it == 0 || item_first[item_col[it]] == (int)it || p % gpb == 0 || pos[it - 1] != p - 1;
+    }
+    flag[it] = f;
+}
+
+__global__ void k_run_first(const int *__restrict__ item_first, const int *__restrict__ run_of_item, int m,
+                            int *__restrict__ run_first) {
+    const i64 c = (i64)blockIdx.x * blockDim.x + threadIdx.x;
+    if (c <= m) run_first[c] = run_of_item[item_first[c]];
+}
+
 __global__ void k_item_records(const int *__restrict__ item_order, const int *__restrict__ item_col,
-                               const int *__restrict__ item_start, const int *__restrict__ item_end, i64 n_items,
-                               int4 *__restrict__ rec) {
+                               const int *__restrict__ item_start, const int *__restrict__ item_end,
+                               const int *__restrict__ run_of_item, i64 n_items, int4 *__restrict__ rec) {
     const i64 io = (i64)blockIdx.x * blockDim.x + threadIdx.x;
     if (io < n_items) {
         const int it = item_order ? item_order[io] : (int)io;
-        rec[io] = make_int4(item_col[it], item_start[it], item_end[it], it);
+        rec[io] = make_int4(item_col[it], item_start[it], item_end[it], run_of_item[it + 1] - 1);
     }
 }
 
 __device__ __forceinline__ float div_pos(float v, float n) { return n > 0.f ? v / n : v; }
 
 template <class S, bool NORMALISE>
-__device__ __forceinline__ void col_reduce_body(const int *__restrict__ item_first, int m, int heavy_items,
+__device__ __forceinline__ void col_reduce_body(const int *__restrict__ run_first, int m, int heavy_items,
                                                 const int *__restrict__ heavy_cols, int n_heavy,
                                                 const float *__restrict__ partial, float *__restrict__ Vt_new,
                                                 int kp, int block, int nblocks, float *sacc ,
@@ -674,7 +715,7 @@
     float4 acc[CH];
     for (int h = block; h < n_heavy; h += nblocks) {
         const int c = heavy_cols[h];
-        const int i0 = item_first[c], i1 = item_first[c + 1];
+        const int i0 = run_first[c], i1 = run_first[c + 1];
 #pragma unroll
         for (int j = 0; j < CH; ++j) acc[j] = zero4();
         constexpr int B = 4;
@@ -709,7 +750,7 @@
         __syncthreads();
     }
     for (i64 c = (i64)block * GPB + gid; c < m; c += (i64)nblocks * GPB) {
-        const int i0 = item_first[c], i1 = item_first[c + 1];
+        const int i0 = run_first[c], i1 = run_first[c + 1];
         if (i1 - i0 > heavy_items) continue;
 #pragma unroll
         for (int j = 0; j < CH; ++j) acc[j] = zero4();
@@ -748,17 +789,17 @@
 }
 
 template <class S>
-__global__ __launch_bounds__(256) void k_col_reduce(const int *__restrict__ item_first, int m,
+__global__ __launch_bounds__(256) void k_col_reduce(const int *__restrict__ run_first, int m,
                                                     int heavy_items, const int *__restrict__ heavy_cols,
                                                     int n_heavy, const float *__restrict__ partial,
                                                     float *__restrict__ Vt_new, int kp_rt) {
     extern __shared__ float sacc[];
-    col_reduce_body<S, false>(item_first, m, heavy_items, heavy_cols, n_heavy, partial, Vt_new, S::kp(kp_rt),
+    col_reduce_body<S, false>(run_first, m, heavy_items, heavy_cols, n_heavy, partial, Vt_new, S::kp(kp_rt),
                               (int)blockIdx.x, (int)gridDim.x, sacc, nullptr);
 }
 
 template <class S>
-__global__ __launch_bounds__(256) void k_col_reduce_norm(const int *__restrict__ item_first, int m,
+__global__ __launch_bounds__(256) void k_col_reduce_norm(const int *__restrict__ run_first, int m,
                                                          int heavy_items, const int *__restrict__ heavy_cols,
                                                          int n_heavy, const float *__restrict__ partial,
                                                          const float *__restrict__ norm_pwz,
@@ -769,14 +810,14 @@
     float *snorm = sdyn + GPB * kp;
     for (int z = threadIdx.x; z < kp; z += 256) snorm[z] = norm_pwz[z];
     __syncthreads();
-    col_reduce_body<S, true>(item_first, m, heavy_items, heavy_cols, n_heavy, partial, Vt_out, kp,
+    col_reduce_body<S, true>(run_first, m, heavy_items, heavy_cols, n_heavy, partial, Vt_out, kp,
                              (int)blockIdx.x, (int)gridDim.x, sdyn, snorm);
 }
 
-__global__ void k_heavy_list(const int *__restrict__ item_first, int m, int heavy_items,
+__global__ void k_heavy_list(const int *__restrict__ run_first, int m, int heavy_items,
                              int *__restrict__ heavy_cols, int *__restrict__ n_heavy) {
     const i64 c = (i64)blockIdx.x * blockDim.x + threadIdx.x;
-    if (c < m && item_first[c + 1] - item_first[c] > heavy_items)
+    if (c < m && run_first[c + 1] - run_first[c] > heavy_items)
         heavy_cols[atomicAdd(n_heavy, 1)] = (int)c;
 }
 
diff --git a/enstop_amd/csrc/plsa_member_kernels.hpp b/enstop_amd/csrc/plsa_member_kernels.hpp
--- a/enstop_amd/csrc/plsa_member_kernels.hpp
+++ b/enstop_amd/csrc/plsa_member_kernels.hpp
@@ -15,7 +15,7 @@
     i64 n_items;
     double *chunk_sums2;
     float *norm_pwz;
-    const int *item_first, *heavy_cols;
+    const int *run_first, *heavy_cols;
     int n_chunks, norm_blocks;
     int m, n_heavy, heavy_items, reduce_grid;
     const int *indptr, *colidx;
@@ -107,7 +107,7 @@
     for (int z = threadIdx.x; z < kp; z += 256) snorm[z] = a.norm_pwz[z];
     __syncthreads();
     const int pv = (int)((cv >> r) & 1ull);
-    col_reduce_body<S, true>(a.item_first, a.m, a.heavy_items, a.heavy_cols, a.n_heavy, a.partial, a.Vt[1 - pv], kp,
+    col_reduce_body<S, true>(a.run_first, a.m, a.heavy_items, a.heavy_cols, a.n_heavy, a.partial, a.Vt[1 - pv], kp,
                              (int)blockIdx.x, a.reduce_grid, sdyn, snorm);
 }
 
diff --git a/enstop_amd/csrc/plsa_members.hpp b/enstop_amd/csrc/plsa_members.hpp
--- a/enstop_amd/csrc/plsa_members.hpp
+++ b/enstop_amd/csrc/plsa_members.hpp
@@ -73,7 +73,7 @@
     const int row_grid = grid_for(c, items ? c->ritems.n : c->n, 256 / c->row_lpn);
     if (items) CHK(ensure(c, c->rpartial, sizeof(float) * (size_t)c->ritems.n * c->kp));
     CHK(ensure(c, c->ll_partials, sizeof(double) * (size_t)row_grid));
-    CHK(ensure(c, c->partial, sizeof(float) * (size_t)std::max<i64>(c->csc.n_items, 1) * c->kp));
+    CHK(ensure(c, c->partial, sizeof(float) * (size_t)std::max<i64>(c->runs.n, 1) * c->kp));
     const int gpb = 256 / c->lpn;
     const int n_chunks = (int)((c->csc.n_items + gpb - 1) / gpb);
     CHK(ensure(c, c->colsum_rows, sizeof(double) * (size_t)std::max(n_chunks, 1) * c->kp));
@@ -93,14 +93,14 @@
     a.n_items = c->csc.n_items;
     a.chunk_sums2 = c->colsum_rows2.as<double>();
     a.norm_pwz = c->norm_pwz.as<float>();
-    a.item_first = c->csc.item_first.as<int>();
-    a.heavy_cols = c->csc.heavy_cols.as<int>();
+    a.run_first = c->runs.first.as<int>();
+    a.heavy_cols = c->runs.heavy_cols.as<int>();
     a.n_chunks = n_chunks;
     a.norm_blocks = norm_blocks;
     a.m = (int)c->m;
-    a.n_heavy = c->csc.n_heavy;
+    a.n_heavy = c->runs.n_heavy;
     a.heavy_items = c->heavy_items;
-    a.reduce_grid = grid_for(c, c->m, gpb) + c->csc.n_heavy;
+    a.reduce_grid = grid_for(c, c->m, gpb) + c->runs.n_heavy;
     a.indptr = c->indptr;
     a.colidx = pk_row ? c->pk_csr.buf.as<int>() : c->col;
     a.vals = c->val;
@@ -117,7 +117,7 @@
     a.row_grid = row_grid;
     a.row_reduce_grid = grid_for(c, c->n, 256 / c->row_lpn);
     for (int i = 0; i < 2; ++i) { a.U[i] = c->U[i].as<float>(); a.Vt[i] = c->Vt[i].as<float>(); }
-    inf.items = items; inf.rseg = c->ritems.seg; inf.n_chunks = n_chunks; inf.n_heavy = c->csc.n_heavy;
+    inf.items = items; inf.rseg = c->ritems.seg; inf.n_chunks = n_chunks; inf.n_heavy = c->runs.n_heavy;
     inf.row_grid = row_grid; inf.norm_blocks = norm_blocks;
     c->colsum_rows_used = n_chunks;
     return 0;
@@ -183,7 +183,7 @@
         CHK(dispatch_shape(c0, [&](auto S) {
             using Sh = decltype(S);
             constexpr int GPB = 256 / Sh::LPN;
-            const size_t smem = sizeof(double) * (size_t)GPB * kp;
+            const size_t smem = col_pass_smem(GPB, kp);
             auto launch = [&](auto SS, auto TN) {
                 hipLaunchKernelGGL((plsa::k_col_pass_members<decltype(SS), decltype(TN)::value>), dim3(chunks_x, G), dim3(256),
                                    smem, col_stream, table, live, cu, cv, kp, thresh);
diff --git a/enstop_amd/engine.py b/enstop_amd/engine.py
--- a/enstop_amd/engine.py
+++ b/enstop_amd/engine.py
@@ -411,6 +411,11 @@
         self._ok(self._L.plsa_packed_info(self._h, C.byref(a), C.byref(b)))
         name = {1: "packed", 0: "arrays", -1: None}
         return dict(csr=name[a.value], csc=name[b.value])
+
+    def partial_info(self):
+        a = np.zeros(3, np.int64)
+        self._ok(self._L.plsa_partial_info(self._h, a))
+        return dict(items=int(a[0]), rows=int(a[1]), heavy_columns=int(a[2]))
 
     def pass_info(self):
         col, row, wide = np.zeros(3, np.int32), np.zeros(3, np.int32), np.zeros(2, np.int32)
diff --git a/include/plsa_hip_diag.h b/include/plsa_hip_diag.h
--- a/include/plsa_hip_diag.h
+++ b/include/plsa_hip_diag.h
@@ -35,6 +35,8 @@
 
 int plsa_packed_info(plsa_ctx *ctx, int32_t *csr, int32_t *csc);
 
+int plsa_partial_info(plsa_ctx *ctx, int64_t *out );
+
 int plsa_pass_info(plsa_ctx *ctx, int32_t *col , int32_t *row , int32_t *wide );
 
 int plsa_fit_info(plsa_ctx *ctx, int32_t *info );
```

Result: no change. 350.2 iter/s, median of 3 (+0.4%).
